# pasqal-io/pulser-diff

Hardware: AMD Instinct MI355X
Metric: time-steps/sec (fwd+grad) (higher is better)
Workload: dtype c128; 1 GPU; c3: 20-qubit register, 1000 time steps, fwd+grad wrt 8 pulse params per parameter set, KRYLOV_SE map, 1 parameter set(s) in the job; n_qubits=20, trajectories_total=1, trajectories_this_rank=1, ranks=1, gathered_parameter_sets=1, parallelism=trajectory-sharded x1 (one replica per rank), kernel_family=chained-tiles, tape=full

## Files before the change

### pulser-diff_amd/_native.py

```python
from __future__ import annotations

import ctypes
import os
import subprocess
import threading
from pathlib import Path

_CSRC = Path(__file__).resolve().parent / "csrc"
_LIB_PATH = Path(os.environ.get("RYDIFF_LIB", _CSRC / "librydiff.so"))

RYDIFF_OK = 0
RYDIFF_EINVAL = -1
RYDIFF_EWORKSPACE = -2
RYDIFF_EHIP = -3
RYDIFF_ENOTIMPL = -4
SOLVER_KRYLOV_SE = 0
SOLVER_DP5_SE = 1
PLAN_SCRATCH_BYTES = 1024
KERNEL_FAMILIES = ("lanes", "persistent", "direct", "chained-tiles")
MAX_QUBITS = 30
MAX_TERMS = 64
MAX_PAULI_STRINGS = 1024
MAX_OVERLAPS = 16
MAX_RDMS = 8
MAX_RDM_QUBITS = 6
MAX_TANGENTS = 8
TANGENT_PAIR_TERMS = 1
TANGENT_DENSITY_MATRIX = 2
TANGENT_RDMS = 4
TANGENT_MOMENTS = 8
MAX_DM_ATOMS = 12
MAX_DM_DIAG = 64
MAX_SHOTS = 1 << 20
SHOT_NONE = 0xFFFFFFFF


class RydProblem(ctypes.Structure):
    _fields_ = [
        ("n_qubits", ctypes.c_int32),
        ("batch", ctypes.c_int32),
        ("coeff_batch", ctypes.c_int32),
        ("n_samples", ctypes.c_int32),
        ("dt", ctypes.c_double),
        ("n_amp_terms", ctypes.c_int32),
        ("n_det_terms", ctypes.c_int32),
        ("amp_masks", ctypes.c_void_p),
        ("det_masks", ctypes.c_void_p),
        ("amp_tables", ctypes.c_void_p),
        ("det_tables", ctypes.c_void_p),
        ("u_pairs", ctypes.c_void_p),
        ("n_tsave", ctypes.c_int32),
        ("tsave", ctypes.c_void_p),
        ("solver", ctypes.c_int32),
        ("tol", ctypes.c_double),
        ("n_obs", ctypes.c_int32),
        ("obs_diag", ctypes.c_void_p),
        ("n_pair_terms", ctypes.c_int32),
        ("pair_qubits", ctypes.c_void_p),
        ("pair_tables", ctypes.c_void_p),
        ("real_amp_grad", ctypes.c_int32),
        ("kernel_variant", ctypes.c_int32),
        ("shard_bits", ctypes.c_int32),
        ("shard_rank_first", ctypes.c_int32),
        ("shard_recv", ctypes.c_void_p),
        ("shard_exchange", ctypes.c_void_p),
        ("shard_user", ctypes.c_void_p),
        ("final_state_only", ctypes.c_int32),
        ("amp_conditioned_terms", ctypes.c_uint64),
        ("det_ones_terms", ctypes.c_uint64),
        ("dp5_piece_refine", ctypes.c_void_p),
        ("dm_moments", ctypes.c_int32),
        ("n_shots", ctypes.c_int32),
        ("n_shot_times", ctypes.c_int32),
        ("shot_times", ctypes.c_void_p),
        ("shot_uniforms", ctypes.c_void_p),
        ("shots_out", ctypes.c_void_p),
        ("bit_moments", ctypes.c_int32),
        ("n_rdms", ctypes.c_int32),
        ("rdm_masks", ctypes.c_void_p),
        ("n_dm_rdms", ctypes.c_int32),
        ("dm_rdm_masks", ctypes.c_void_p),
        ("dm_atoms", ctypes.c_int32),
        ("n_dm_diag", ctypes.c_int32),
        ("dm_diag", ctypes.c_void_p),
        ("n_dm_pauli_obs", ctypes.c_int32),
        ("n_dm_pauli_strings", ctypes.c_int32),
        ("dm_pauli_first", ctypes.c_void_p),
        ("dm_pauli_x", ctypes.c_void_p),
        ("dm_pauli_z", ctypes.c_void_p),
        ("dm_pauli_w", ctypes.c_void_p),
        ("n_dm_fid", ctypes.c_int32),
        ("dm_fid_batch", ctypes.c_int32),
        ("dm_fid_targets", ctypes.c_void_p),
        ("dm_purity", ctypes.c_int32),
        ("dm_shots", ctypes.c_int32),
        ("tape_steps", ctypes.c_int32),
        ("n_overlaps", ctypes.c_int32),
        ("overlap_batch", ctypes.c_int32),
        ("overlap_targets", ctypes.c_void_p),
        ("n_pauli_obs", ctypes.c_int32),
        ("n_pauli_strings", ctypes.c_int32),
        ("pauli_first", ctypes.c_void_p),
        ("pauli_x", ctypes.c_void_p),
        ("pauli_z", ctypes.c_void_p),
        ("pauli_w", ctypes.c_void_p),
    ]


SHARD_EXCHANGE_FN = ctypes.CFUNCTYPE(ctypes.c_int, ctypes.c_void_p, ctypes.c_int, ctypes.c_void_p, ctypes.c_size_t)


class RydPlanInfo(ctypes.Structure):
    _fields_ = [
        ("spectral_lo", ctypes.c_double),
        ("spectral_hi", ctypes.c_double),
        ("rho_design", ctypes.c_double),
        ("degree", ctypes.c_int32),
        ("n_stages", ctypes.c_int32),
        ("max_step_factors", ctypes.c_int32),
        ("flags", ctypes.c_int32),
        ("total_factors", ctypes.c_int64),
        ("workspace_bytes", ctypes.c_size_t),
        ("tape_mode", ctypes.c_int32),
        ("kernel_family", ctypes.c_int32),
        ("kernel_fwd", ctypes.c_char * 80),
        ("kernel_bwd", ctypes.c_char * 80),
    ]


class RydTangent(ctypes.Structure):

    _fields_ = [
        ("n_dir", ctypes.c_int32),
        ("d_amp", ctypes.c_void_p),
        ("d_det", ctypes.c_void_p),
        ("d_u", ctypes.c_void_p),
        ("d_psi0", ctypes.c_void_p),
        ("flags", ctypes.c_int32),
    ]


EXPORTS = (
    "rydiff_plan",
    "rydiff_forward",
    "rydiff_backward",
    "rydiff_apply_hamiltonian",
    "rydiff_apply_factor",
    "rydiff_design_polynomial",
    "rydiff_last_error",
    "rydiff_version",
    "rydiff_sizeof_problem",
    "rydiff_sizeof_plan_info",
    "rydiff_sizeof_tangent",
    "rydiff_tangent_workspace_bytes",
    "rydiff_tangent_workspace_bytes_flags",
    "rydiff_forward_tangent",
    "rydiff_geometry_workspace_bytes",
    "rydiff_geometry_workspace_bytes_flags",
    "rydiff_forward_geometry",
    "rydiff_fisher_workspace_bytes_flags",
    "rydiff_forward_fisher",
)

_lib = None


def build(force: bool = False) -> Path:
    if force or not _LIB_PATH.exists():
        subprocess.run(["make", "-C", str(_CSRC)] + (["-B"] if force else []), check=True)
    return _LIB_PATH


def lib() -> ctypes.CDLL:
    global _lib
    if _lib is not None:
        return _lib
    if not _LIB_PATH.exists():
        raise RuntimeError(
            f"{_LIB_PATH} is missing: the HIP extension has not been built. Run `python -c 'import "
            "__graft_entry__ as g; g.build()'` (or `make -C pulser-diff_amd/csrc`). There is no CPU fallback."
        )
    L = ctypes.CDLL(str(_LIB_PATH))
    vp, i32, dbl = ctypes.c_void_p, ctypes.c_int, ctypes.c_double
    L.rydiff_plan.argtypes = [ctypes.POINTER(RydProblem), i32, i32, vp, vp, ctypes.POINTER(RydPlanInfo)]
    L.rydiff_plan.restype = i32
    L.rydiff_forward.argtypes = [ctypes.POINTER(RydProblem), ctypes.POINTER(RydPlanInfo), vp, vp, vp, vp,
                                 ctypes.c_size_t, i32, vp]
    L.rydiff_forward.restype = i32
    L.rydiff_backward.argtypes = [ctypes.POINTER(RydProblem), ctypes.POINTER(RydPlanInfo), vp, vp, vp, vp, vp, vp,
                                  vp, vp, vp, ctypes.c_size_t, i32, vp]
    L.rydiff_backward.restype = i32
    L.rydiff_apply_hamiltonian.argtypes = [ctypes.POINTER(RydProblem), vp, vp, vp, vp, vp, ctypes.c_size_t, vp]
    L.rydiff_apply_hamiltonian.restype = i32
    L.rydiff_apply_factor.argtypes = [ctypes.POINTER(RydProblem), vp, vp, vp, vp, vp, vp, i32, vp, vp, i32, vp,
                                      ctypes.c_size_t, vp]
    L.rydiff_apply_factor.restype = i32
    L.rydiff_design_polynomial.argtypes = [dbl, dbl, i32, ctypes.POINTER(i32), vp, vp, ctypes.POINTER(dbl)]
    L.rydiff_design_polynomial.restype = i32
    L.rydiff_last_error.restype = ctypes.c_char_p
    L.rydiff_version.restype = ctypes.c_char_p
    L.rydiff_sizeof_problem.restype = ctypes.c_size_t
    L.rydiff_sizeof_plan_info.restype = ctypes.c_size_t
    L.rydiff_sizeof_tangent.restype = ctypes.c_size_t
    L.rydiff_tangent_workspace_bytes.argtypes = [ctypes.POINTER(RydProblem), ctypes.POINTER(RydPlanInfo), i32]
    L.rydiff_tangent_workspace_bytes.restype = ctypes.c_size_t
    L.rydiff_tangent_workspace_bytes_flags.argtypes = [ctypes.POINTER(RydProblem), ctypes.POINTER(RydPlanInfo), i32, i32]
    L.rydiff_tangent_workspace_bytes_flags.restype = ctypes.c_size_t
    L.rydiff_forward_tangent.argtypes = [ctypes.POINTER(RydProblem), ctypes.POINTER(RydPlanInfo), ctypes.POINTER(RydTangent), vp, vp, vp,
                                         vp, ctypes.c_size_t, vp]
    L.rydiff_forward_tangent.restype = i32
    L.rydiff_geometry_workspace_bytes.argtypes = [ctypes.POINTER(RydProblem), ctypes.POINTER(RydPlanInfo), i32]
    L.rydiff_geometry_workspace_bytes.restype = ctypes.c_size_t
    L.rydiff_geometry_workspace_bytes_flags.argtypes = [ctypes.POINTER(RydProblem), ctypes.POINTER(RydPlanInfo), i32, i32]
    L.rydiff_geometry_workspace_bytes_flags.restype = ctypes.c_size_t
    L.rydiff_forward_geometry.argtypes = [ctypes.POINTER(RydProblem), ctypes.POINTER(RydPlanInfo), ctypes.POINTER(RydTangent), vp, vp, vp,
                                          vp, vp, ctypes.c_size_t, vp]
    L.rydiff_forward_geometry.restype = i32
    L.rydiff_fisher_workspace_bytes_flags.argtypes = [ctypes.POINTER(RydProblem), ctypes.POINTER(RydPlanInfo), i32, i32]
    L.rydiff_fisher_workspace_bytes_flags.restype = ctypes.c_size_t
    L.rydiff_forward_fisher.argtypes = [ctypes.POINTER(RydProblem), ctypes.POINTER(RydPlanInfo), ctypes.POINTER(RydTangent), vp, vp, vp,
                                        vp, vp, vp, ctypes.c_size_t, vp]
    L.rydiff_forward_fisher.restype = i32
    if (L.rydiff_sizeof_problem(), L.rydiff_sizeof_plan_info(), L.rydiff_sizeof_tangent()) != (
            ctypes.sizeof(RydProblem), ctypes.sizeof(RydPlanInfo), ctypes.sizeof(RydTangent)):
        raise RuntimeError(f"{_LIB_PATH} was built from another include/rydiff.h than this binding mirrors (struct sizes differ): rebuild it")
    _lib = L
    return L


def last_error() -> str:
    return lib().rydiff_last_error().decode()


def check(rc: int) -> None:
    if rc == RYDIFF_OK:
        return
    msg = last_error()
    if rc == RYDIFF_EINVAL:
        raise ValueError(msg)
    if rc == RYDIFF_ENOTIMPL:
        raise NotImplementedError(msg)
    if rc == RYDIFF_EWORKSPACE:
        raise MemoryError(msg)
    raise RuntimeError(f"rydiff (HIP) error {rc}: {msg}")


def design_polynomial(rho: float, tol: float = 1e-13, max_degree: int = 120):
    import numpy as np

    deg = ctypes.c_int()
    roots = np.zeros(2 * max_degree)
    p0 = np.zeros(2)
    err = ctypes.c_double()
    check(lib().rydiff_design_polynomial(rho, tol, max_degree, ctypes.byref(deg), roots.ctypes.data, p0.ctypes.data,
                                         ctypes.byref(err)))
    m = deg.value
    return roots[: 2 * m].view(np.complex128).copy(), complex(p0[0], p0[1]), err.value


_KNOWN_VARIANTS = (0, 1, 2, 3, 4, 7, 8, 9, 10, 11, 12, 13, 14, 15, 16, 17, 18, 19, 20, 21, 22, 23, 24, 25, 26, 27, 28, 29, 30, 31, 32, 33, 34)
_tls = threading.local()


def set_kernel_variant(variant: int) -> None:
    if int(variant) not in _KNOWN_VARIANTS:
        raise ValueError(f"kernel variant must be one of {_KNOWN_VARIANTS}, got {variant}")
    _tls.variant = int(variant)


def default_kernel_variant() -> int:
    return getattr(_tls, "variant", 0)
```

### pulser-diff_amd/csrc/chain_kernels.hpp

```cpp
#pragma once

constexpr int kSmallTileBits = 10;
constexpr int kTileBits = 12;
constexpr int kWideTileBits = 13;

__device__ __forceinline__ void stream_store(double2* p, const double2& v) {
#ifdef RYDIFF_PLAIN_STORES
    *p = v;
#else
    __builtin_nontemporal_store(v.x, &p->x);
    __builtin_nontemporal_store(v.y, &p->y);
#endif
}

__device__ __forceinline__ void through_store(double2* base, uint32_t n, unsigned i, const double2& v) {
    typedef unsigned u32x4 __attribute__((ext_vector_type(4)));
    const __amdgpu_buffer_rsrc_t dst = __builtin_amdgcn_make_buffer_rsrc(base, 0, int(n * uint32_t(sizeof(double2))), 0x00020000);
    __builtin_amdgcn_raw_buffer_store_b128(__builtin_bit_cast(u32x4, v), dst, int(i * unsigned(sizeof(double2))), 0,  16);
}

template <bool THROUGH>
__device__ __forceinline__ void out_store(double2* base, uint32_t n, unsigned i, const double2& v) {
    if constexpr (THROUGH) through_store(base, n, i, v);
    else stream_store(base + i, v);
}

__device__ __forceinline__ double2 stream_load(const double2* p) {
#ifdef RYDIFF_PLAIN_LOADS
    return *p;
#else
    double2 v;
    v.x = __builtin_nontemporal_load(&p->x);
    v.y = __builtin_nontemporal_load(&p->y);
    return v;
#endif
}

struct ChainArgs {
    const double2* u;
    const double2* p;
    double2* v_out;
    double2* q_out;
    const double* utt;
    const double* vr;
    const double* coef_fin;
    const double* coef_sta;
    long coef_bstride;
    double fb_r, fb_i;
    double fg_r, fg_i;
    int completes;
    double sg_r, sg_i, sb_r, sb_i;
    int lo, hs, hb;
    uint32_t dim;
    int has_p, has_q, write_v;
    int ga, gd;
    uint32_t fin_mask[kMaxGroups];
    uint32_t sta_mask[kMaxGroups];
    uint32_t dmask[kMaxGroups];
    int dcnt[kMaxGroups];
    uint32_t cond;
    int xcd_place;
    int tile_swz;
    int b_first, b_count;
    int resident;
    const double2* x_fin;
    const double2* x_sta;
    double* ge_fin;
    double* ge_sta;
    long ge_bstride, ge_rstride;
    double cb_fin_r, cb_fin_i, cb_sta_r, cb_sta_i;
    double* wtot;
    const double2* inj_gstate;
    const double* inj_gexp;
    const double* inj_obs;
    int inj_n_obs;
    long inj_ostride;
    int sh_bits;
    int sh_nl;
    int sh_rank_first;
    int sh_self;
    const double2* sh_rem[kShardMaxBits];
    int sh_grp[kShardMaxBits];
    long obs_bstride, obs_ostride;
    const double* obs;
    double* expect_slot;
    int n_obs;
    long exp_ostride;
};

template <int NT>
__device__ __forceinline__ void wg_atomic_add(double v, double* dst, double* red ) {
#pragma unroll
    for (int off = 32; off > 0; off >>= 1) v += __shfl_down(v, off, 64);
    __syncthreads();
    if ((threadIdx.x & 63) == 0) red[threadIdx.x >> 6] = v;
    __syncthreads();
    if (threadIdx.x == 0) {
        double s2 = 0.0;
#pragma unroll
        for (int w = 0; w < NT / 64; ++w) s2 += red[w];
        unsafeAtomicAdd(dst, s2);
    }
}

template <int NW>
__device__ __forceinline__ void park2(double v0, double v1, double* red, int slot0, int slot1) {
#pragma unroll
    for (int off = 32; off > 0; off >>= 1) {
        v0 += __shfl_down(v0, off, 64);
        v1 += __shfl_down(v1, off, 64);
    }
    if ((threadIdx.x & 63) == 0) {
        red[slot0 * NW + (threadIdx.x >> 6)] += v0;
        red[slot1 * NW + (threadIdx.x >> 6)] += v1;
    }
}

template <int NW>
__device__ __forceinline__ void park1(double v0, double* red, int slot0) {
#pragma unroll
    for (int off = 32; off > 0; off >>= 1) v0 += __shfl_down(v0, off, 64);
    if ((threadIdx.x & 63) == 0) red[slot0 * NW + (threadIdx.x >> 6)] += v0;
}

template <int LT, int LGT, bool CPLX, bool FULL = false, bool COND = false>
__device__ __forceinline__ void partner_sums(const double2* __restrict__ tile, const double2 (&reg)[1 << (LT - LGT)],
                                             uint32_t mask, unsigned tid, double2 (&ts)[1 << (LT - LGT)],
                                             double2 (&ds)[1 << (LT - LGT)]) {
    constexpr int NT = 1 << LGT, R = 1 << (LT - LGT);
#pragma unroll
    for (int r = 0; r < R; ++r) {
        ts[r] = make_double2(0.0, 0.0);
        ds[r] = make_double2(0.0, 0.0);
    }
#pragma unroll
    for (int b = 0; b < LT; ++b) {
        if (FULL || (mask >> b & 1u)) {
            if (b < LGT) {
                const double sgn = (tid >> b & 1u) ? 1.0 : -1.0;
#pragma unroll
                for (int r = 0; r < R; ++r) {
                    if (COND && !((unsigned(r) * NT + tid) >> (b ^ 1) & 1u)) continue;
                    const double2 q = tile[(unsigned(r) * NT + tid) ^ (1u << b)];
                    ts[r].x += q.x;
                    ts[r].y += q.y;
                    if (CPLX) {
                        ds[r].x = fma(sgn, q.x, ds[r].x);
                        ds[r].y = fma(sgn, q.y, ds[r].y);
                    }
                }
            } else {
#pragma unroll
                for (int r = 0; r < R; ++r) {
                    if (COND && !((unsigned(r) * NT + tid) >> (b ^ 1) & 1u)) continue;
                    const double2 q = reg[r ^ (1 << (b - LGT))];
                    ts[r].x += q.x;
                    ts[r].y += q.y;
                    if (CPLX) {
                        if (r >> (b - LGT) & 1) {
                            ds[r].x += q.x;
                            ds[r].y += q.y;
                        } else {
                            ds[r].x -= q.x;
                            ds[r].y -= q.y;
                        }
                    }
                }
            }
        }
    }
}

template <int CTRL, int BANK>
__device__ __forceinline__ int dpp_mov(int old, int src) {
    return __builtin_amdgcn_update_dpp(old, src, CTRL, 0xF, BANK, false);
}

template <int CTRL, int BANK>
__device__ __forceinline__ int dpp_mov_all(int src) {
    return __builtin_amdgcn_mov_dpp(src, CTRL, 0xF, BANK, true);
}

template <int B>
__device__ __forceinline__ int lane_xor_i32(int w) {
    if constexpr (B == 0) return dpp_mov_all<0xB1, 0xF>(w);
    else if constexpr (B == 1) return dpp_mov_all<0x4E, 0xF>(w);
    else if constexpr (B == 2) {
        const int r = dpp_mov_all<0x124, 0xA>(w);
        return dpp_mov<0x12C, 0x5>(r, w);
    } else if constexpr (B == 3) return dpp_mov_all<0x128, 0xF>(w);
    else return __shfl_xor(w, 1 << B, 64);
}

template <int B>
__device__ __forceinline__ double2 lane_xor(const double2& v) {
    const int a0 = lane_xor_i32<B>(__double2loint(v.x)), a1 = lane_xor_i32<B>(__double2hiint(v.x));
    const int b0 = lane_xor_i32<B>(__double2loint(v.y)), b1 = lane_xor_i32<B>(__double2hiint(v.y));
    return make_double2(__hiloint2double(a1, a0), __hiloint2double(b1, b0));
}

template <int LT, bool CPLX, bool FULL = false, bool COND = false>
__device__ __forceinline__ void partner_sums_lanes(const double2& own, uint32_t mask, unsigned tid, double2& ts, double2& ds) {
    static_assert(LT <= 6, "one amplitude per lane");
    ts = make_double2(0.0, 0.0);
    ds = make_double2(0.0, 0.0);
    auto bit = [&](auto bc) {
        constexpr int b = decltype(bc)::value;
        if constexpr (b < LT) {
            if (FULL || (mask >> b & 1u)) {
                double2 q = lane_xor<b>(own);
                if (COND && !(tid >> (b ^ 1) & 1u)) q = make_double2(0.0, 0.0);
                ts.x += q.x;
                ts.y += q.y;
                if (CPLX) {
                    const double sgn = (tid >> b & 1u) ? 1.0 : -1.0;
                    ds.x = fma(sgn, q.x, ds.x);
                    ds.y = fma(sgn, q.y, ds.y);
                }
            }
        }
    };
    bit(std::integral_constant<int, 0>{});
    bit(std::integral_constant<int, 1>{});
    bit(std::integral_constant<int, 2>{});
    bit(std::integral_constant<int, 3>{});
    bit(std::integral_constant<int, 4>{});
    bit(std::integral_constant<int, 5>{});
}

#ifdef RYDIFF_TIMELINE
__device__ unsigned long long g_timeline[4096 * 11];
#define RYDIFF_TL(slot)                                                                                   \
    do {                                                                                                  \
        if (threadIdx.x == 0 && blockIdx.y == 0 && blockIdx.x < 4096 && a.has_p && a.has_q)               \
            g_timeline[(slot) < 8 ? blockIdx.x * 8 + (slot) : 4096 * (slot) + blockIdx.x] = __builtin_readcyclecounter(); \
    } while (0)
#else
#define RYDIFF_TL(slot)
#endif

constexpr double kRecMinBetaC = 6.0e-5;

template <int LT, int LGT, bool CPLX, bool BWD, bool FAST = false, bool RES = false>
__global__ __launch_bounds__(1 << LGT) void k_chain(ChainArgs a) {
    constexpr int NT = 1 << LGT, R = 1 << (LT - LGT);
    constexpr bool REC = BWD && FAST && !CPLX;
    const int GA = FAST ? 1 : a.ga;
    const int GD = FAST ? (a.gd ? 1 : 0) : a.gd;
    extern __shared__ __attribute__((aligned(16))) double2 tile[];
    double* red = reinterpret_cast<double*>(tile + (size_t(1) << LT));
    constexpr int NW = NT / 64;
    const int n_slots = BWD ? 4 * a.ga + a.gd : 0;
    if (BWD) {
        for (int s = int(threadIdx.x); s < n_slots * NW; s += NT) red[s] = 0.0;
    }
    auto flush_gradients = [&](double* ge_fin_, double* ge_sta_) {
        __syncthreads();
        for (int s = int(threadIdx.x); s < n_slots; s += NT) {
            double sum = 0.0;
#pragma unroll
            for (int w = 0; w < NW; ++w) sum += red[s * NW + w];
            double* dst;
            if (s < 2 * a.ga) dst = ge_fin_ + ((s & 1) ? a.ga : 0) + (s >> 1);
            else if (s < 2 * a.ga + a.gd) dst = (REC ? ge_fin_ : ge_sta_) + 2 * a.ga + (s - 2 * a.ga);
            else dst = ge_sta_ + (((s - 2 * a.ga - a.gd) & 1) ? a.ga : 0) + ((s - 2 * a.ga - a.gd) >> 1);
            if (sum != 0.0) unsafeAtomicAdd(dst, sum);
        }
    };
    const unsigned tid = threadIdx.x;
    unsigned t = a.xcd_place ? (blockIdx.x >> 3) : blockIdx.x;
    if (a.tile_swz) {
        const unsigned w = blockIdx.x, G = 1u << a.tile_swz;
        t = (w & ~(8u * G - 1u)) | ((w & 7u) << a.tile_swz) | ((w >> 3) & (G - 1u));
    }
    const unsigned bl = a.xcd_place ? (blockIdx.y * 8u + (blockIdx.x & 7u)) : blockIdx.y;
    if (bl >= unsigned(a.b_count)) return;
    const unsigned bt = unsigned(a.b_first) + bl;
    const size_t boff = size_t(bt) * a.dim;
    const unsigned rank = unsigned(a.sh_rank_first) + bl;
    const unsigned rank_hi = a.sh_bits ? (rank << a.sh_nl) : 0u;
    const unsigned t_glob = a.sh_bits ? (t + (rank << (a.sh_nl - LT))) : t;
    auto ld = [&](const double2* p) -> double2 {
        if constexpr (RES) return *p;
        else return stream_load(p);
    };
    auto st = [&](double2* p, const double2& v) {
        if constexpr (RES) *p = v;
        else stream_store(p, v);
    };
    const unsigned lomask = (1u << a.lo) - 1u;
    const int midlow = a.hs - a.lo;
    const unsigned xbase = ((t & ((1u << midlow) - 1u)) << a.lo) | ((t >> midlow) << (a.hs + a.hb));

#ifdef RYDIFF_STAGGER
    for (unsigned sl = 0; sl < (blockIdx.x % RYDIFF_STAGGER_PHASES); ++sl) __builtin_amdgcn_s_sleep(RYDIFF_STAGGER);
#endif
    RYDIFF_TL(0);
    double2 uu[R], acc[R];
    unsigned xg[R];
#pragma unroll
    for (int r = 0; r < R; ++r) {
        const unsigned i = unsigned(r) * NT + tid;
        xg[r] = xbase | (i & lomask) | ((i >> a.lo) << a.hs);
        uu[r] = ld(a.u + boff + xg[r]);
    }
#pragma unroll
    for (int r = 0; r < R; ++r) acc[r] = ld(a.p + boff + xg[r]);
    double2 remacc[R];
    if (a.has_p && a.completes && a.sh_bits) {
#pragma unroll
        for (int r = 0; r < R; ++r) remacc[r] = make_double2(0.0, 0.0);
        const double* __restrict__ cfs = a.coef_fin + bt * a.coef_bstride;
        for (int k = 0; k < a.sh_bits; ++k) {
            if (a.sh_grp[k] < 0) continue;
            const double cr = cfs[a.sh_grp[k]], ci = (rank >> k & 1u) ? cfs[a.ga + a.sh_grp[k]] : -cfs[a.ga + a.sh_grp[k]];
            const double kr = a.fb_r * cr - a.fb_i * ci, ki = a.fb_r * ci + a.fb_i * cr;
            const double2* __restrict__ src = a.sh_self ? a.u + size_t(unsigned(a.b_first) + (bl ^ (1u << k))) * a.dim : a.sh_rem[k] + size_t(bl) * a.dim;
#pragma unroll
            for (int r = 0; r < R; ++r) {
                const double2 pv = src[xg[r]];
                remacc[r].x += kr * pv.x - ki * pv.y;
                remacc[r].y += kr * pv.y + ki * pv.x;
            }
        }
    }
    double dg[R];
#pragma unroll
    for (int r = 0; r < R; ++r) dg[r] = a.utt[unsigned(r) * NT + tid];
    double2 xf[R], xs[R];
    constexpr bool XS_EARLY = BWD && !CPLX && !REC;
    bool exact_fin = true, exact_sta = true;
    if constexpr (REC) {
        exact_fin = !(fabs(a.coef_fin[bt * a.coef_bstride]) * sqrt(a.fb_r * a.fb_r + a.fb_i * a.fb_i) >= kRecMinBetaC);
        exact_sta = !(fabs(a.coef_sta[bt * a.coef_bstride]) * sqrt(a.sb_r * a.sb_r + a.sb_i * a.sb_i) >= kRecMinBetaC);
    }
    if (BWD) {
#pragma unroll
        for (int r = 0; r < R; ++r) xf[r] = stream_load(a.x_fin + boff + xg[r]);
    }
    if (XS_EARLY) {
#pragma unroll
        for (int r = 0; r < R; ++r) xs[r] = stream_load(a.x_sta + boff + xg[r]);
    }
#ifndef RYDIFF_ABLATE_SYNC
#pragma unroll
    for (int r = 0; r < R; ++r) tile[unsigned(r) * NT + tid] = uu[r];
    __syncthreads();
#endif
    RYDIFF_TL(1);
    double* ge_fin = nullptr;
    double* ge_sta = nullptr;
    if (BWD) {
        const long goff = bt * a.ge_bstride + (blockIdx.x % kGradReplicas) * a.ge_rstride;
        ge_fin = a.ge_fin + goff;
        ge_sta = a.ge_sta + goff;
    }

    auto interaction_diagonal = [&](double (&du)[R]) {
        double vloc[LT];
        const double* __restrict__ vrow = a.vr + size_t(t_glob) * 16;
#ifdef RYDIFF_ABLATE_COEF
        for (int b2 = 0; b2 < LT; ++b2) vloc[b2] = a.sb_r;
        double dlane = a.sb_i;
        (void)vrow;
#else
#pragma unroll
        for (int b2 = 0; b2 < LT; ++b2) vloc[b2] = vrow[b2];
        double dlane = vrow[LT];
#endif
#pragma unroll
        for (int b2 = 0; b2 < LGT; ++b2)
            if (!(tid >> b2 & 1u)) dlane += vloc[b2];
#pragma unroll
        for (int r = 0; r < R; ++r) {
            double d = dg[r] + dlane;
#pragma unroll
            for (int b2 = LGT; b2 < LT; ++b2)
                if (!(r >> (b2 - LGT) & 1)) d += vloc[b2];
            du[r] = d;
        }
    };
    double du[R];
    if constexpr (REC) interaction_diagonal(du);

    if (a.has_p) {
        const double* __restrict__ cf = a.coef_fin + bt * a.coef_bstride;
        for (int g = 0; g < GA; ++g) {
            const uint32_t mask = a.fin_mask[g];
            if (!mask) continue;
            double2 ts[R], ds[R];
#ifndef RYDIFF_ABLATE_COMPUTE
            if (!FAST && (a.cond >> g & 1u)) partner_sums<LT, LGT, CPLX, false, true>(tile, uu, mask, tid, ts, ds);
            else partner_sums<LT, LGT, CPLX>(tile, uu, mask, tid, ts, ds);
#else
            for (int r = 0; r < R; ++r) { ts[r] = uu[r]; ds[r] = uu[r]; }
#endif
#ifdef RYDIFF_ABLATE_COEF
            const double cr = a.sg_r, ci = a.sg_i;
#else
            const double cr = cf[g], ci = cf[a.ga + g];
#endif
            const double k1r = a.fb_r * cr, k1i = a.fb_i * cr;
            const double k2r = -a.fb_i * ci, k2i = a.fb_r * ci;
#pragma unroll
            for (int r = 0; r < R; ++r) {
                acc[r].x += k1r * ts[r].x - k1i * ts[r].y;
                acc[r].y += k1r * ts[r].y + k1i * ts[r].x;
                if (CPLX) {
                    acc[r].x += k2r * ds[r].x - k2i * ds[r].y;
                    acc[r].y += k2r * ds[r].y + k2i * ds[r].x;
                }
            }
            if (BWD && exact_fin) {
                double z1r = 0.0, z1i = 0.0, z2r = 0.0, z2i = 0.0;
#pragma unroll
                for (int r = 0; r < R; ++r) {
                    z1r += ts[r].x * xf[r].x + ts[r].y * xf[r].y;
                    z1i += ts[r].x * xf[r].y - ts[r].y * xf[r].x;
                    if (CPLX) {
                        z2r += ds[r].x * xf[r].x + ds[r].y * xf[r].y;
                        z2i += ds[r].x * xf[r].y - ds[r].y * xf[r].x;
                    }
                }
                if (CPLX) park2<NW>(a.cb_fin_r * z1r - a.cb_fin_i * z1i, a.cb_fin_r * z2i + a.cb_fin_i * z2r, red, 2 * g, 2 * g + 1);
                else park1<NW>(a.cb_fin_r * z1r - a.cb_fin_i * z1i, red, 2 * g);
            }
        }
        if (a.completes && a.sh_bits) {
#pragma unroll
            for (int r = 0; r < R; ++r) {
                acc[r].x += remacc[r].x;
                acc[r].y += remacc[r].y;
            }
            if (BWD && exact_fin) {
                for (int k = 0; k < a.sh_bits; ++k) {
                    const int g = a.sh_grp[k];
                    if (g < 0) continue;
                    const double2* __restrict__ src = a.sh_self ? a.u + size_t(unsigned(a.b_first) + (bl ^ (1u << k))) * a.dim : a.sh_rem[k] + size_t(bl) * a.dim;
                    const double sgn = (rank >> k & 1u) ? 1.0 : -1.0;
                    double z1r = 0.0, z1i = 0.0;
#pragma unroll
                    for (int r = 0; r < R; ++r) {
                        const double2 pv = src[xg[r]];
                        z1r += pv.x * xf[r].x + pv.y * xf[r].y;
                        z1i += pv.x * xf[r].y - pv.y * xf[r].x;
                    }
                    if (CPLX) park2<NW>(a.cb_fin_r * z1r - a.cb_fin_i * z1i, sgn * (a.cb_fin_r * z1i + a.cb_fin_i * z1r), red, 2 * g, 2 * g + 1);
                    else park1<NW>(a.cb_fin_r * z1r - a.cb_fin_i * z1i, red, 2 * g);
                }
            }
        }
        if constexpr (REC) {
            if (a.completes) {
                double sgd = 0.0, zr = 0.0;
                const double cdet = GD ? cf[2] : 0.0;
#pragma unroll
                for (int r = 0; r < R; ++r) {
                    const double pr = a.cb_fin_r * uu[r].x + a.cb_fin_i * uu[r].y, pi = a.cb_fin_i * uu[r].x - a.cb_fin_r * uu[r].y;
                    const double w = pr * xf[r].x - pi * xf[r].y;
                    if (a.wtot) unsafeAtomicAdd(a.wtot + (a.sh_bits ? boff : 0) + xg[r], w);
                    const double cnt = GD ? double(a.dcnt[0] - popc_i((xg[r] | rank_hi) & a.dmask[0])) : 0.0;
                    sgd += w * cnt;
                    if (!exact_fin) {
                        double d = du[r] + cdet * cnt;
                        for (int g = 1; g < a.gd; ++g) d += cf[2 + g] * double(a.dcnt[g] - popc_i((xg[r] | rank_hi) & a.dmask[g]));
                        const double dr = a.fg_r + a.fb_r * d, di = a.fg_i + a.fb_i * d;
                        const double wx = acc[r].x - (dr * uu[r].x - di * uu[r].y), wy = acc[r].y - (dr * uu[r].y + di * uu[r].x);
                        zr += wx * xf[r].x + wy * xf[r].y;
                    }
                }
                if (GD) park1<NW>(sgd, red, 2 * a.ga);
                for (int g = 1; g < a.gd; ++g) {
                    double sg = 0.0;
#pragma unroll
                    for (int r = 0; r < R; ++r) {
                        const double pr = a.cb_fin_r * uu[r].x + a.cb_fin_i * uu[r].y, pi = a.cb_fin_i * uu[r].x - a.cb_fin_r * uu[r].y;
                        sg += (pr * xf[r].x - pi * xf[r].y) * double(a.dcnt[g] - popc_i((xg[r] | rank_hi) & a.dmask[g]));
                    }
                    park1<NW>(sg, red, 2 * a.ga + g);
                }
                if (!exact_fin) park1<NW>(zr / cf[0], red, 0);
            }
        }
    } else {
#pragma unroll
        for (int r = 0; r < R; ++r) acc[r] = uu[r];
    }
    if (BWD && a.has_p && (a.inj_gexp || a.inj_gstate)) {
        if (a.inj_gexp) {
            bool any = false;
            for (int o = 0; o < a.inj_n_obs; ++o) any |= a.inj_gexp[o * a.inj_ostride + bt] != 0.0;
            if (any) {
#pragma unroll
                for (int r = 0; r < R; ++r) {
                    double wsum = 0.0;
                    for (int o = 0; o < a.inj_n_obs; ++o)
                        wsum += a.inj_gexp[o * a.inj_ostride + bt] * a.inj_obs[size_t(o) * a.obs_ostride + bt * a.obs_bstride + xg[r]];
                    acc[r].x += 2.0 * wsum * xf[r].x;
                    acc[r].y += 2.0 * wsum * xf[r].y;
                }
            }
        }
        if (a.inj_gstate) {
#pragma unroll
            for (int r = 0; r < R; ++r) {
                const double2 gs = stream_load(a.inj_gstate + boff + xg[r]);
                acc[r].x += gs.x;
                acc[r].y += gs.y;
            }
        }
    }
    if (BWD && !XS_EARLY && a.has_q && (!REC || exact_sta)) {
#pragma unroll
        for (int r = 0; r < R; ++r) xs[r] = stream_load(a.x_sta + boff + xg[r]);
    }
    RYDIFF_TL(2);
    if (a.write_v) {
#pragma unroll
        for (int r = 0; r < R; ++r) st(a.v_out + boff + xg[r], acc[r]);
    }
    RYDIFF_TL(3);
    if (!BWD && a.obs) {
        for (int o = 0; o < a.n_obs; ++o) {
            double e = 0.0;
#pragma unroll
            for (int r = 0; r < R; ++r) e += a.obs[size_t(o) * a.obs_ostride + bt * a.obs_bstride + xg[r]] * (acc[r].x * acc[r].x + acc[r].y * acc[r].y);
            wg_atomic_add<NT>(e, a.expect_slot + o * a.exp_ostride + bt, red);
        }
    }
    if (!a.has_q) {
        if (BWD) flush_gradients(ge_fin, ge_sta);
        return;
    }

#ifndef RYDIFF_ABLATE_SYNC
    __syncthreads();
#pragma unroll
    for (int r = 0; r < R; ++r) tile[unsigned(r) * NT + tid] = acc[r];
    __syncthreads();
#endif
    RYDIFF_TL(4);

    const double* __restrict__ cf = a.coef_sta + bt * a.coef_bstride;
    if constexpr (!REC) interaction_diagonal(du);
    double rr[R];
    if (BWD && !REC) {
#pragma unroll
        for (int r = 0; r < R; ++r) {
            const double pr = a.cb_sta_r * acc[r].x + a.cb_sta_i * acc[r].y, pi = a.cb_sta_i * acc[r].x - a.cb_sta_r * acc[r].y;
            rr[r] = pr * xs[r].x - pi * xs[r].y;
            if (a.wtot) unsafeAtomicAdd(a.wtot + (a.sh_bits ? boff : 0) + xg[r], rr[r]);
        }
        for (int g = 0; g < a.gd; ++g) {
            double sgd = 0.0;
#pragma unroll
            for (int r = 0; r < R; ++r) sgd += rr[r] * double(a.dcnt[g] - popc_i((xg[r] | rank_hi) & a.dmask[g]));
            park1<NW>(sgd, red, 2 * a.ga + g);
        }
    }
    double2 q[R];
#pragma unroll
    for (int r = 0; r < R; ++r) {
        double d = du[r];
        if (FAST) {
            if (GD) d += cf[2] * double(a.dcnt[0] - popc_i((xg[r] | rank_hi) & a.dmask[0]));
            for (int g = 1; g < a.gd; ++g) d += cf[2 + g] * double(a.dcnt[g] - popc_i((xg[r] | rank_hi) & a.dmask[g]));
        } else {
            for (int g = 0; g < a.gd; ++g) d += cf[2 * a.ga + g] * double(a.dcnt[g] - popc_i((xg[r] | rank_hi) & a.dmask[g]));
        }
        const double dr = a.sg_r + a.sb_r * d, di = a.sg_i + a.sb_i * d;
        q[r].x = dr * acc[r].x - di * acc[r].y;
        q[r].y = dr * acc[r].y + di * acc[r].x;
    }
    for (int g = 0; g < GA; ++g) {
        const uint32_t mask = a.sta_mask[g];
        if (!FAST && !mask) continue;
        double2 ts[R], ds[R];
#ifndef RYDIFF_ABLATE_COMPUTE
        if (!FAST && (a.cond >> g & 1u)) partner_sums<LT, LGT, CPLX, false, true>(tile, acc, mask, tid, ts, ds);
        else partner_sums<LT, LGT, CPLX, FAST>(tile, acc, mask, tid, ts, ds);
#else
        for (int r = 0; r < R; ++r) { ts[r] = acc[r]; ds[r] = acc[r]; }
#endif
#ifdef RYDIFF_ABLATE_COEF
        const double cr = a.sg_r, ci = a.sg_i;
#else
        const double cr = cf[g], ci = cf[a.ga + g];
#endif
        const double k1r = a.sb_r * cr, k1i = a.sb_i * cr;
        const double k2r = -a.sb_i * ci, k2i = a.sb_r * ci;
#pragma unroll
        for (int r = 0; r < R; ++r) {
            q[r].x += k1r * ts[r].x - k1i * ts[r].y;
            q[r].y += k1r * ts[r].y + k1i * ts[r].x;
            if (CPLX) {
                q[r].x += k2r * ds[r].x - k2i * ds[r].y;
                q[r].y += k2r * ds[r].y + k2i * ds[r].x;
            }
        }
        if (BWD && exact_sta) {
            double z1r = 0.0, z1i = 0.0, z2r = 0.0, z2i = 0.0;
#pragma unroll
            for (int r = 0; r < R; ++r) {
                z1r += ts[r].x * xs[r].x + ts[r].y * xs[r].y;
                z1i += ts[r].x * xs[r].y - ts[r].y * xs[r].x;
                if (CPLX) {
                    z2r += ds[r].x * xs[r].x + ds[r].y * xs[r].y;
                    z2i += ds[r].x * xs[r].y - ds[r].y * xs[r].x;
                }
            }
            if (CPLX) park2<NW>(a.cb_sta_r * z1r - a.cb_sta_i * z1i, a.cb_sta_r * z2i + a.cb_sta_i * z2r, red, 2 * a.ga + a.gd + 2 * g,
                                2 * a.ga + a.gd + 2 * g + 1);
            else park1<NW>(a.cb_sta_r * z1r - a.cb_sta_i * z1i, red, 2 * a.ga + a.gd + 2 * g);
        }
    }
    RYDIFF_TL(5);
#pragma unroll
    for (int r = 0; r < R; ++r) st(a.q_out + boff + xg[r], q[r]);
    if (BWD) flush_gradients(ge_fin, ge_sta);
    RYDIFF_TL(6);
#ifdef RYDIFF_TIMELINE
    __builtin_amdgcn_s_waitcnt(0);
    RYDIFF_TL(7);
#endif
}

template <int I, int N, class F>
__device__ __forceinline__ void static_for(F&& f) {
    if constexpr (I < N) {
        f(std::integral_constant<int, I>{});
        static_for<I + 1, N>(f);
    }
}

template <int LT, bool CPLX, bool BWD, bool FAST, int RH = (1 << (LT - 10)) / 2>
__global__ __launch_bounds__(1024) void k_chain_wide(ChainArgs a) {
    constexpr int LGT = 10, NT = 1 << LGT, R = 1 << (LT - LGT), NP = R / RH, NW = NT / 64;
    static_assert(R >= 2 && RH >= 1 && NP * RH == R, "R amplitudes per thread in NP parts of RH");
    constexpr bool REC = BWD && FAST && !CPLX;
    const int GA = FAST ? 1 : a.ga;
    const int GD = FAST ? (a.gd ? 1 : 0) : a.gd;
    extern __shared__ __attribute__((aligned(16))) double2 tile[];
    double* red = reinterpret_cast<double*>(tile + (size_t(1) << LT));
    const int n_slots = BWD ? 4 * a.ga + a.gd : 0;
    if (BWD) {
        for (int s = int(threadIdx.x); s < n_slots * NW; s += NT) red[s] = 0.0;
    }
    const unsigned tid = threadIdx.x;
    unsigned t = blockIdx.x;
    if (a.tile_swz) {
        const unsigned w = blockIdx.x, G = 1u << a.tile_swz;
        t = (w & ~(8u * G - 1u)) | ((w & 7u) << a.tile_swz) | ((w >> 3) & (G - 1u));
    }
    const unsigned bl = blockIdx.y;
    const unsigned bt = unsigned(a.b_first) + bl;
    const size_t boff = size_t(bt) * a.dim;
    const unsigned rank = unsigned(a.sh_rank_first) + bl;
    const unsigned rank_hi = a.sh_bits ? (rank << a.sh_nl) : 0u;
    const unsigned t_glob = a.sh_bits ? (t + (rank << (a.sh_nl - LT))) : t;
    const unsigned lomask = (1u << a.lo) - 1u;
    const int midlow = a.hs - a.lo;
    const unsigned xbase = ((t & ((1u << midlow) - 1u)) << a.lo) | ((t >> midlow) << (a.hs + a.hb));
    auto xg_of = [&](int r) -> unsigned {
        const unsigned i = unsigned(r) * NT + tid;
        return xbase | (i & lomask) | ((i >> a.lo) << a.hs);
    };
    double* ge_fin = nullptr;
    double* ge_sta = nullptr;
    if (BWD) {
        const long goff = bt * a.ge_bstride + (blockIdx.x % kGradReplicas) * a.ge_rstride;
        ge_fin = a.ge_fin + goff;
        ge_sta = a.ge_sta + goff;
    }
    auto flush_gradients = [&]() {
        __syncthreads();
        for (int s = int(threadIdx.x); s < n_slots; s += NT) {
            double sum = 0.0;
#pragma unroll
            for (int w = 0; w < NW; ++w) sum += red[s * NW + w];
            double* dst;
            if (s < 2 * a.ga) dst = ge_fin + ((s & 1) ? a.ga : 0) + (s >> 1);
            else if (s < 2 * a.ga + a.gd) dst = (REC ? ge_fin : ge_sta) + 2 * a.ga + (s - 2 * a.ga);
            else dst = ge_sta + (((s - 2 * a.ga - a.gd) & 1) ? a.ga : 0) + ((s - 2 * a.ga - a.gd) >> 1);
            if (sum != 0.0) unsafeAtomicAdd(dst, sum);
        }
    };
    const double* __restrict__ vrow = a.vr + size_t(t_glob) * 16;
    auto lane_diag = [&]() -> double {
        double dlane = vrow[LT];
#pragma unroll
        for (int b2 = 0; b2 < LGT; ++b2)
            if (!(tid >> b2 & 1u)) dlane += vrow[b2];
        return dlane;
    };
    auto diag_of = [&](int rf, double dlane) -> double {
        double d = a.utt[unsigned(rf) * NT + tid] + dlane;
#pragma unroll
        for (int b2 = LGT; b2 < LT; ++b2)
            if (!(rf >> (b2 - LGT) & 1)) d += vrow[b2];
        return d;
    };
    bool exact_fin = true, exact_sta = true;
    if constexpr (REC) {
        exact_fin = !(fabs(a.coef_fin[bt * a.coef_bstride]) * sqrt(a.fb_r * a.fb_r + a.fb_i * a.fb_i) >= kRecMinBetaC);
        exact_sta = !(fabs(a.coef_sta[bt * a.coef_bstride]) * sqrt(a.sb_r * a.sb_r + a.sb_i * a.sb_i) >= kRecMinBetaC);
    }

    double2 acc[R];
    {
        double2 uu[RH];
#pragma unroll
        for (int h = 0; h < NP; ++h) {
#pragma unroll
            for (int r = 0; r < RH; ++r) uu[r] = stream_load(a.u + boff + xg_of(h * RH + r));
#pragma unroll
            for (int r = 0; r < RH; ++r) tile[unsigned(h * RH + r) * NT + tid] = uu[r];
        }
    }
#pragma unroll
    for (int r = 0; r < R; ++r) acc[r] = stream_load(a.p + boff + xg_of(r));
    __syncthreads();

    bool inj_any = false;
    if (BWD && a.has_p && a.inj_gexp) {
        for (int o = 0; o < a.inj_n_obs; ++o) inj_any |= a.inj_gexp[o * a.inj_ostride + bt] != 0.0;
    }
    auto finish_half = [&](auto hc) {
        constexpr int h = decltype(hc)::value;
        const double* __restrict__ cf = a.coef_fin + bt * a.coef_bstride;
        double2 xf[RH];
        if (BWD) {
#pragma unroll
            for (int r = 0; r < RH; ++r) xf[r] = stream_load(a.x_fin + boff + xg_of(h * RH + r));
        }
        if (a.has_p) {
            for (int g = 0; g < GA; ++g) {
                const uint32_t mask = a.fin_mask[g];
                if (!mask) continue;
                double2 ts[RH], ds[RH];
#pragma unroll
                for (int r = 0; r < RH; ++r) {
                    ts[r] = make_double2(0.0, 0.0);
                    ds[r] = make_double2(0.0, 0.0);
                }
#pragma unroll
                for (int b = 0; b < LT; ++b) {
                    if (mask >> b & 1u) {
#pragma unroll
                        for (int r = 0; r < RH; ++r) {
                            const unsigned i = unsigned(h * RH + r) * NT + tid;
                            const double2 q = tile[i ^ (1u << b)];
                            ts[r].x += q.x;
                            ts[r].y += q.y;
                            if (CPLX) {
                                const double sgn = (i >> b & 1u) ? 1.0 : -1.0;
                                ds[r].x = fma(sgn, q.x, ds[r].x);
                                ds[r].y = fma(sgn, q.y, ds[r].y);
                            }
                        }
                    }
                }
                const double cr = cf[g], ci = cf[a.ga + g];
                const double k1r = a.fb_r * cr, k1i = a.fb_i * cr;
                const double k2r = -a.fb_i * ci, k2i = a.fb_r * ci;
#pragma unroll
                for (int r = 0; r < RH; ++r) {
                    double2& A = acc[h * RH + r];
                    A.x += k1r * ts[r].x - k1i * ts[r].y;
                    A.y += k1r * ts[r].y + k1i * ts[r].x;
                    if (CPLX) {
                        A.x += k2r * ds[r].x - k2i * ds[r].y;
                        A.y += k2r * ds[r].y + k2i * ds[r].x;
                    }
                }
                if (BWD && exact_fin) {
                    double z1r = 0.0, z1i = 0.0, z2r = 0.0, z2i = 0.0;
#pragma unroll
                    for (int r = 0; r < RH; ++r) {
                        z1r += ts[r].x * xf[r].x + ts[r].y * xf[r].y;
                        z1i += ts[r].x * xf[r].y - ts[r].y * xf[r].x;
                        if (CPLX) {
                            z2r += ds[r].x * xf[r].x + ds[r].y * xf[r].y;
                            z2i += ds[r].x * xf[r].y - ds[r].y * xf[r].x;
                        }
                    }
                    if (CPLX) park2<NW>(a.cb_fin_r * z1r - a.cb_fin_i * z1i, a.cb_fin_r * z2i + a.cb_fin_i * z2r, red, 2 * g, 2 * g + 1);
                    else park1<NW>(a.cb_fin_r * z1r - a.cb_fin_i * z1i, red, 2 * g);
                }
            }
            if (a.completes && a.sh_bits) {
                for (int k = 0; k < a.sh_bits; ++k) {
                    const int g = a.sh_grp[k];
                    if (g < 0) continue;
                    const double cr = cf[g], ci = (rank >> k & 1u) ? cf[a.ga + g] : -cf[a.ga + g];
                    const double kr = a.fb_r * cr - a.fb_i * ci, ki = a.fb_r * ci + a.fb_i * cr;
                    const double2* __restrict__ src = a.sh_self ? a.u + size_t(unsigned(a.b_first) + (bl ^ (1u << k))) * a.dim : a.sh_rem[k] + size_t(bl) * a.dim;
                    const double sgn = (rank >> k & 1u) ? 1.0 : -1.0;
                    double z1r = 0.0, z1i = 0.0;
#pragma unroll
                    for (int r = 0; r < RH; ++r) {
                        const double2 pv = src[xg_of(h * RH + r)];
                        acc[h * RH + r].x += kr * pv.x - ki * pv.y;
                        acc[h * RH + r].y += kr * pv.y + ki * pv.x;
                        if (BWD) {
                            z1r += pv.x * xf[r].x + pv.y * xf[r].y;
                            z1i += pv.x * xf[r].y - pv.y * xf[r].x;
                        }
                    }
                    if (BWD && exact_fin) {
                        if (CPLX) park2<NW>(a.cb_fin_r * z1r - a.cb_fin_i * z1i, sgn * (a.cb_fin_r * z1i + a.cb_fin_i * z1r), red, 2 * g, 2 * g + 1);
                        else park1<NW>(a.cb_fin_r * z1r - a.cb_fin_i * z1i, red, 2 * g);
                    }
                }
            }
            if constexpr (REC) {
                if (a.completes) {
                    double sgd = 0.0, zr = 0.0;
                    const double cdet = GD ? cf[2] : 0.0;
                    const double dlane = exact_fin ? 0.0 : lane_diag();
#pragma unroll
                    for (int r = 0; r < RH; ++r) {
                        const int rf = h * RH + r;
                        const double2 mu = tile[unsigned(rf) * NT + tid];
                        const unsigned x = xg_of(rf);
                        const double pr = a.cb_fin_r * mu.x + a.cb_fin_i * mu.y, pi = a.cb_fin_i * mu.x - a.cb_fin_r * mu.y;
                        const double w = pr * xf[r].x - pi * xf[r].y;
                        if (a.wtot) unsafeAtomicAdd(a.wtot + (a.sh_bits ? boff : 0) + x, w);
                        const double cnt = GD ? double(a.dcnt[0] - popc_i((x | rank_hi) & a.dmask[0])) : 0.0;
                        sgd += w * cnt;
                        if (!exact_fin) {
                            double d = diag_of(rf, dlane) + cdet * cnt;
                            for (int g = 1; g < a.gd; ++g) d += cf[2 + g] * double(a.dcnt[g] - popc_i((x | rank_hi) & a.dmask[g]));
                            const double dr = a.fg_r + a.fb_r * d, di = a.fg_i + a.fb_i * d;
                            const double wx = acc[rf].x - (dr * mu.x - di * mu.y), wy = acc[rf].y - (dr * mu.y + di * mu.x);
                            zr += wx * xf[r].x + wy * xf[r].y;
                        }
                    }
                    if (GD) park1<NW>(sgd, red, 2 * a.ga);
                    for (int g = 1; g < a.gd; ++g) {
                        double sg = 0.0;
#pragma unroll
                        for (int r = 0; r < RH; ++r) {
                            const int rf = h * RH + r;
                            const double2 mu = tile[unsigned(rf) * NT + tid];
                            const double pr = a.cb_fin_r * mu.x + a.cb_fin_i * mu.y, pi = a.cb_fin_i * mu.x - a.cb_fin_r * mu.y;
                            sg += (pr * xf[r].x - pi * xf[r].y) * double(a.dcnt[g] - popc_i((xg_of(rf) | rank_hi) & a.dmask[g]));
                        }
                        park1<NW>(sg, red, 2 * a.ga + g);
                    }
                    if (!exact_fin) park1<NW>(zr / cf[0], red, 0);
                }
            }
        }
        if (BWD && a.has_p && (a.inj_gexp || a.inj_gstate)) {
            if (inj_any) {
#pragma unroll
                for (int r = 0; r < RH; ++r) {
                    double wsum = 0.0;
                    for (int o = 0; o < a.inj_n_obs; ++o)
                        wsum += a.inj_gexp[o * a.inj_ostride + bt] * a.inj_obs[size_t(o) * a.obs_ostride + bt * a.obs_bstride + xg_of(h * RH + r)];
                    acc[h * RH + r].x += 2.0 * wsum * xf[r].x;
                    acc[h * RH + r].y += 2.0 * wsum * xf[r].y;
                }
            }
            if (a.inj_gstate) {
#pragma unroll
                for (int r = 0; r < RH; ++r) {
                    const double2 gs = stream_load(a.inj_gstate + boff + xg_of(h * RH + r));
                    acc[h * RH + r].x += gs.x;
                    acc[h * RH + r].y += gs.y;
                }
            }
        }
        if (a.write_v) {
#pragma unroll
            for (int r = 0; r < RH; ++r) stream_store(a.v_out + boff + xg_of(h * RH + r), acc[h * RH + r]);
        }
    };
    static_for<0, NP>(finish_half);

    if (!BWD && a.obs) {
        for (int o = 0; o < a.n_obs; ++o) {
            double e = 0.0;
#pragma unroll
            for (int r = 0; r < R; ++r) e += a.obs[size_t(o) * a.obs_ostride + bt * a.obs_bstride + xg_of(r)] * (acc[r].x * acc[r].x + acc[r].y * acc[r].y);
            wg_atomic_add<NT>(e, a.expect_slot + o * a.exp_ostride + bt, red);
        }
    }
    if (!a.has_q) {
        if (BWD) flush_gradients();
        return;
    }

    __syncthreads();
#pragma unroll
    for (int r = 0; r < R; ++r) tile[unsigned(r) * NT + tid] = acc[r];
    __syncthreads();

    auto start_half = [&](auto hc) {
        constexpr int h = decltype(hc)::value;
        const double* __restrict__ cf = a.coef_sta + bt * a.coef_bstride;
        const bool need_xs = BWD && (!REC || exact_sta);
        double2 xs[RH];
        if (need_xs) {
#pragma unroll
            for (int r = 0; r < RH; ++r) xs[r] = stream_load(a.x_sta + boff + xg_of(h * RH + r));
        }
        double2 q[RH];
        const double dlane = lane_diag();
#pragma unroll
        for (int r = 0; r < RH; ++r) {
            const int rf = h * RH + r;
            double d = diag_of(rf, dlane);
            const unsigned x = xg_of(rf) | rank_hi;
            if (FAST) {
                if (GD) d += cf[2] * double(a.dcnt[0] - popc_i(x & a.dmask[0]));
                for (int g = 1; g < a.gd; ++g) d += cf[2 + g] * double(a.dcnt[g] - popc_i(x & a.dmask[g]));
            } else {
                for (int g = 0; g < a.gd; ++g) d += cf[2 * a.ga + g] * double(a.dcnt[g] - popc_i(x & a.dmask[g]));
            }
            const double dr = a.sg_r + a.sb_r * d, di = a.sg_i + a.sb_i * d;
            q[r].x = dr * acc[rf].x - di * acc[rf].y;
            q[r].y = dr * acc[rf].y + di * acc[rf].x;
        }
        if (BWD && !REC) {
            double rr[RH];
#pragma unroll
            for (int r = 0; r < RH; ++r) {
                const int rf = h * RH + r;
                const double pr = a.cb_sta_r * acc[rf].x + a.cb_sta_i * acc[rf].y, pi = a.cb_sta_i * acc[rf].x - a.cb_sta_r * acc[rf].y;
                rr[r] = pr * xs[r].x - pi * xs[r].y;
                if (a.wtot) unsafeAtomicAdd(a.wtot + (a.sh_bits ? boff : 0) + xg_of(rf), rr[r]);
            }
            for (int g = 0; g < a.gd; ++g) {
                double sgd = 0.0;
#pragma unroll
                for (int r = 0; r < RH; ++r) sgd += rr[r] * double(a.dcnt[g] - popc_i((xg_of(h * RH + r) | rank_hi) & a.dmask[g]));
                park1<NW>(sgd, red, 2 * a.ga + g);
            }
        }
        for (int g = 0; g < GA; ++g) {
            const uint32_t mask = a.sta_mask[g];
            if (!FAST && !mask) continue;
            double2 ts[RH], ds[RH];
#pragma unroll
            for (int r = 0; r < RH; ++r) {
                ts[r] = make_double2(0.0, 0.0);
                ds[r] = make_double2(0.0, 0.0);
            }
#pragma unroll
            for (int b = 0; b < LT; ++b) {
                if (FAST || (mask >> b & 1u)) {
#pragma unroll
                    for (int r = 0; r < RH; ++r) {
                        const int rf = h * RH + r;
                        const unsigned i = unsigned(rf) * NT + tid;
                        double2 pv;
                        if (b < LGT) pv = tile[i ^ (1u << b)];
                        else pv = acc[rf ^ (1 << (b < LGT ? 0 : b - LGT))];
                        ts[r].x += pv.x;
                        ts[r].y += pv.y;
                        if (CPLX) {
                            const double sgn = (i >> b & 1u) ? 1.0 : -1.0;
                            ds[r].x = fma(sgn, pv.x, ds[r].x);
                            ds[r].y = fma(sgn, pv.y, ds[r].y);
                        }
                    }
                }
            }
            const double cr = cf[g], ci = cf[a.ga + g];
            const double k1r = a.sb_r * cr, k1i = a.sb_i * cr;
            const double k2r = -a.sb_i * ci, k2i = a.sb_r * ci;
#pragma unroll
            for (int r = 0; r < RH; ++r) {
                q[r].x += k1r * ts[r].x - k1i * ts[r].y;
                q[r].y += k1r * ts[r].y + k1i * ts[r].x;
                if (CPLX) {
                    q[r].x += k2r * ds[r].x - k2i * ds[r].y;
                    q[r].y += k2r * ds[r].y + k2i * ds[r].x;
                }
            }
            if (BWD && exact_sta) {
                double z1r = 0.0, z1i = 0.0, z2r = 0.0, z2i = 0.0;
#pragma unroll
                for (int r = 0; r < RH; ++r) {
                    z1r += ts[r].x * xs[r].x + ts[r].y * xs[r].y;
                    z1i += ts[r].x * xs[r].y - ts[r].y * xs[r].x;
                    if (CPLX) {
                        z2r += ds[r].x * xs[r].x + ds[r].y * xs[r].y;
                        z2i += ds[r].x * xs[r].y - ds[r].y * xs[r].x;
                    }
                }
                if (CPLX) park2<NW>(a.cb_sta_r * z1r - a.cb_sta_i * z1i, a.cb_sta_r * z2i + a.cb_sta_i * z2r, red, 2 * a.ga + a.gd + 2 * g,
                                    2 * a.ga + a.gd + 2 * g + 1);
                else park1<NW>(a.cb_sta_r * z1r - a.cb_sta_i * z1i, red, 2 * a.ga + a.gd + 2 * g);
            }
        }
#pragma unroll
        for (int r = 0; r < RH; ++r) stream_store(a.q_out + boff + xg_of(h * RH + r), q[r]);
    };
    static_for<0, NP>(start_half);
    if (BWD) flush_gradients();
}
```

### pulser-diff_amd/csrc/pair_kernels.hpp

```cpp
#pragma once

struct Chain2Args {
    const double2* v;
    const double2* w;
    const double2* t;
    double2* vmid_out;
    double2* y_out;
    double2* w_out;
    double2* t_out;
    const double* utt;
    const double* vr;
    const double* coef_fin;
    const double* coef_sta;
    long coef_bstride;
    double a_r, a_i, b_r, b_i, k_r, k_i;
    double g1_r, g1_i, b1_r, b1_i;
    int lo, hs, hb;
    uint32_t dim;
    int has_p, has_q;
    int gd;
    uint32_t fin_mask;
    uint32_t dmask[kMaxGroups];
    int dcnt[kMaxGroups];
    int b_first, b_count;
    const double* obs;
    double* expect_slot;
    int n_obs;
    long exp_ostride;
};

template <int LT, int LGT, bool ORD = false, int WT = 0, int PACE = 0>
__global__ __launch_bounds__(1 << LGT) void k_chain2(Chain2Args a) {
    constexpr int NT = 1 << LGT, R = 1 << (LT - LGT);
    static_assert(WT >= 0 && WT <= 3);
    static_assert(PACE >= 0 && PACE <= 2 && (!PACE || ORD) && (!PACE || R == 4), "pacing: vector-major kernels with four elements per thread");
    extern __shared__ __attribute__((aligned(16))) double2 tiles[];
    double* red = reinterpret_cast<double*>(tiles + 2 * (size_t(1) << LT));
    const unsigned tid = threadIdx.x;
    const unsigned t = blockIdx.x;
    const unsigned bl = blockIdx.y;
    if (bl >= unsigned(a.b_count)) return;
    const unsigned bt = unsigned(a.b_first) + bl;
    const size_t boff = size_t(bt) * a.dim;
    const unsigned lomask = (1u << a.lo) - 1u;
    const int midlow = a.hs - a.lo;
    const unsigned xbase = ((t & ((1u << midlow) - 1u)) << a.lo) | ((t >> midlow) << (a.hs + a.hb));
    RYDIFF_TL(0);
    const double* __restrict__ vrow = a.vr + size_t(t) * 16;
    [[maybe_unused]] double ut[R], vtop[LT + 1], c_fin = 0.0, c_sta = 0.0, cdet_fin = 0.0, cdet_sta = 0.0;
    if constexpr (ORD) {
#pragma unroll
        for (int b2 = 0; b2 <= LT; ++b2) vtop[b2] = vrow[b2];
#pragma unroll
        for (int r = 0; r < R; ++r) ut[r] = a.utt[unsigned(r) * NT + tid];
        c_fin = a.coef_fin[bt * a.coef_bstride];
        c_sta = a.coef_sta[bt * a.coef_bstride];
        if (a.gd) {
            cdet_fin = a.coef_fin[bt * a.coef_bstride + 2];
            cdet_sta = a.coef_sta[bt * a.coef_bstride + 2];
        }
    }
    double2 uu[R], ww[R], tt[R];
    unsigned xg[R];
#pragma unroll
    for (int r = 0; r < R; ++r) {
        const unsigned i = unsigned(r) * NT + tid;
        xg[r] = xbase | (i & lomask) | ((i >> a.lo) << a.hs);
        uu[r] = stream_load(a.v + boff + xg[r]);
    }
    if constexpr (ORD && !PACE) __builtin_amdgcn_s_barrier();
    if constexpr (PACE) {
        __builtin_amdgcn_sched_barrier(0);
        asm volatile("s_waitcnt vmcnt(2)" ::: "memory");
        __builtin_amdgcn_sched_barrier(0);
    }
#pragma unroll
    for (int r = 0; r < R; ++r) ww[r] = stream_load(a.w + boff + xg[r]);
    if constexpr (ORD && !PACE) __builtin_amdgcn_s_barrier();
    if constexpr (!PACE) {
#pragma unroll
        for (int r = 0; r < R; ++r) tt[r] = stream_load(a.t + boff + xg[r]);
    } else {
        __builtin_amdgcn_sched_barrier(0);
    }
    auto reindex = [&]() {
        if constexpr (ORD) {
            unsigned tid_o = tid;
            asm volatile("" : "+v"(tid_o));
#pragma unroll
            for (int r = 0; r < R; ++r) {
                const unsigned i = unsigned(r) * NT + tid_o;
                xg[r] = xbase | (i & lomask) | ((i >> a.lo) << a.hs);
            }
        }
    };
    reindex();
    double du[R];
    {
        double vloc[LT];
#pragma unroll
        for (int b2 = 0; b2 < LT; ++b2) vloc[b2] = ORD ? vtop[b2] : vrow[b2];
        double dlane = ORD ? vtop[LT] : vrow[LT];
#pragma unroll
        for (int b2 = 0; b2 < LGT; ++b2)
            if (!(tid >> b2 & 1u)) dlane += vloc[b2];
#pragma unroll
        for (int r = 0; r < R; ++r) {
            double d;
            if constexpr (ORD) d = ut[r] + dlane;
            else d = a.utt[unsigned(r) * NT + tid] + dlane;
#pragma unroll
            for (int b2 = LGT; b2 < LT; ++b2)
                if (!(r >> (b2 - LGT) & 1)) d += vloc[b2];
            du[r] = d;
        }
    }
    auto diag = [&](const double* cf, [[maybe_unused]] double cdet, int r) -> double {
        double d = du[r];
        if constexpr (ORD) {
            for (int g = 0; g < a.gd; ++g) d += cdet * double(a.dcnt[g] - popc_i(xg[r] & a.dmask[g]));
        } else {
            for (int g = 0; g < a.gd; ++g) d += cf[2 + g] * double(a.dcnt[g] - popc_i(xg[r] & a.dmask[g]));
        }
        return d;
    };
    int buf = 0;
    auto put = [&](const double2 (&val)[R]) -> const double2* {
        double2* tile = tiles + (size_t(buf) << LT);
#pragma unroll
        for (int r = 0; r < R; ++r) tile[unsigned(r) * NT + tid] = val[r];
        __syncthreads();
        buf ^= 1;
        return tile;
    };
    auto cmul = [](double xr, double xi, const double2& z) { return make_double2(xr * z.x - xi * z.y, xr * z.y + xi * z.x); };
    auto request_t = [&]() {
        __builtin_amdgcn_sched_barrier(0);
        const char* tbase = reinterpret_cast<const char*>(a.t + boff);
#pragma unroll
        for (int r = 0; r < R; ++r) tt[r] = stream_load(reinterpret_cast<const double2*>(tbase + xg[r] * unsigned(sizeof(double2))));
        __builtin_amdgcn_sched_barrier(0);
    };

    double2 y[R];
    if (a.has_p) {
        const double* __restrict__ cf = a.coef_fin + bt * a.coef_bstride;
        double c;
        if constexpr (ORD) c = c_fin;
        else c = cf[0];
        double2 s[R], h1[R], ds[R];
        const double2* vtile;
        if constexpr (PACE == 2) {
            double2* tile = tiles + (size_t(buf) << LT);
#pragma unroll
            for (int r = 0; r < R; ++r) tile[unsigned(r) * NT + tid] = uu[r];
            request_t();
            __syncthreads();
            buf ^= 1;
            vtile = tile;
        } else {
            vtile = put(uu);
        }
        RYDIFF_TL(1);
        partner_sums<LT, LGT, false>(vtile, uu, a.fin_mask, tid, s, ds);
        if constexpr (PACE == 1) {
            __builtin_amdgcn_sched_barrier(0);
            asm volatile("s_waitcnt vmcnt(2)" ::: "memory");
            request_t();
        }
#ifdef RYDIFF_TIMELINE
#pragma unroll
        for (int r = 0; r < R; ++r) asm volatile("" ::"v"(ww[r].x), "v"(ww[r].y));
        RYDIFF_TL(8);
#endif
        double d[R];
#pragma unroll
        for (int r = 0; r < R; ++r) {
            d[r] = diag(cf, cdet_fin, r);
            h1[r].x = d[r] * uu[r].x + c * (ww[r].x + s[r].x);
            h1[r].y = d[r] * uu[r].y + c * (ww[r].y + s[r].y);
            const double2 p = cmul(a.a_r, a.a_i, uu[r]), q = cmul(a.b_r, a.b_i, h1[r]);
            y[r] = make_double2(p.x + q.x, p.y + q.y);
        }
        RYDIFF_TL(2);
        if constexpr (PACE) {
            static_assert(WT >= 1, "pacing: v_mid goes through through_store");
            double2* mid_base = a.vmid_out ? a.vmid_out + boff : nullptr;
            const uint32_t mid_n = a.vmid_out ? a.dim : 0u;
#pragma unroll
            for (int r = 0; r < R; ++r) {
                const double2 p = cmul(a.g1_r, a.g1_i, uu[r]), q = cmul(a.b1_r, a.b1_i, h1[r]);
                through_store(mid_base, mid_n, xg[r], make_double2(p.x + q.x, p.y + q.y));
            }
        } else if (a.vmid_out) {
#pragma unroll
            for (int r = 0; r < R; ++r) {
                const double2 p = cmul(a.g1_r, a.g1_i, uu[r]), q = cmul(a.b1_r, a.b1_i, h1[r]);
                out_store<(WT >= 1)>(a.vmid_out + boff, a.dim, xg[r], make_double2(p.x + q.x, p.y + q.y));
            }
        }
        if (a.k_r != 0.0 || a.k_i != 0.0) {
            double2 e[R], pe[R];
#pragma unroll
            for (int r = 0; r < R; ++r) e[r] = make_double2(h1[r].x + c * ww[r].x, h1[r].y + c * ww[r].y);
            partner_sums<LT, LGT, false>(put(e), e, a.fin_mask, tid, pe, ds);
#ifdef RYDIFF_TIMELINE
#pragma unroll
            for (int r = 0; r < R; ++r) asm volatile("" ::"v"(tt[r].x), "v"(tt[r].y));
            RYDIFF_TL(9);
#endif
#pragma unroll
            for (int r = 0; r < R; ++r) {
                const double2 z = make_double2(d[r] * h1[r].x + c * (tt[r].x + pe[r].x), d[r] * h1[r].y + c * (tt[r].y + pe[r].y));
                const double2 k = cmul(a.k_r, a.k_i, z);
                y[r].x += k.x;
                y[r].y += k.y;
            }
        } else if constexpr (PACE) {
#pragma unroll
            for (int r = 0; r < R; ++r) asm volatile("" ::"v"(tt[r].x), "v"(tt[r].y));
        }
        RYDIFF_TL(3);
#pragma unroll
        for (int r = 0; r < R; ++r) out_store<(WT >= 1)>(a.y_out + boff, a.dim, xg[r], y[r]);
        RYDIFF_TL(4);
        if (a.obs) {
            for (int o = 0; o < a.n_obs; ++o) {
                double ex = 0.0;
#pragma unroll
                for (int r = 0; r < R; ++r) ex += a.obs[size_t(o) * a.dim + xg[r]] * (y[r].x * y[r].x + y[r].y * y[r].y);
                wg_atomic_add<NT>(ex, a.expect_slot + o * a.exp_ostride + bt, red);
            }
        }
    } else {
#pragma unroll
        for (int r = 0; r < R; ++r) y[r] = PACE ? ww[r] : (ORD ? tt[r] : uu[r]);
    }
    if (!a.has_q) return;

    reindex();
    const double* __restrict__ cf = a.coef_sta + bt * a.coef_bstride;
    double c;
    if constexpr (ORD) c = c_sta;
    else c = cf[0];
    double2 w2[R], ds[R];
    partner_sums<LT, LGT, false, true>(put(y), y, ~0u, tid, w2, ds);
#pragma unroll
    for (int r = 0; r < R; ++r) out_store<(WT >= 2)>(a.w_out + boff, a.dim, xg[r], w2[r]);
    RYDIFF_TL(5);
    double2 z[R];
#pragma unroll
    for (int r = 0; r < R; ++r) {
        const double d = diag(cf, cdet_sta, r);
        z[r] = make_double2(d * y[r].x + c * w2[r].x, d * y[r].y + c * w2[r].y);
    }
    double2 t2[R];
    partner_sums<LT, LGT, false, true>(put(z), z, ~0u, tid, t2, ds);
#pragma unroll
    for (int r = 0; r < R; ++r) out_store<(WT >= 3)>(a.t_out + boff, a.dim, xg[r], t2[r]);
    RYDIFF_TL(6);
#ifdef RYDIFF_TIMELINE
    asm volatile("s_waitcnt vmcnt(0)" ::: "memory");
    RYDIFF_TL(7);
#endif
}

struct Chain2BwdArgs {
    const double2* mu;
    const double2* w;
    const double2* t;
    const double2* xa;
    const double2* xb;
    double2* mu_out;
    double2* w_out;
    double2* t_out;
    const double* utt;
    const double* vr;
    const double* coef_fin;
    const double* coef_sta;
    long coef_bstride;
    double gb_r, gb_i, bb_r, bb_i;
    double k_r, k_i;
    double ga_r, ga_i, ba_r, ba_i;
    double cba_r, cba_i, cbb_r, cbb_i;
    int lo, hs, hb;
    uint32_t dim;
    int has_p, has_q;
    int gd;
    uint32_t fin_mask;
    uint32_t dmask;
    int dcnt;
    int b_first, b_count;
    double* ge_fin;
    long ge_bstride, ge_rstride;
    int det_slot;
    double* wtot;
    const double2* inj_gstate;
    const double* inj_gexp;
    const double* inj_obs;
    int inj_n_obs;
    long inj_ostride;
};

__device__ __forceinline__ void stream_load_lds(const double2* g, double2* lds_wave) {
    __builtin_amdgcn_global_load_lds(reinterpret_cast<const __attribute__((address_space(1))) void*>(reinterpret_cast<uintptr_t>(g)),
                                     (__attribute__((address_space(3))) void*)lds_wave, 16, 0,  2);
}

constexpr int kChain2BwdXbLds = 1;

template <int LT, int LGT, bool DMA>
constexpr size_t chain2_bwd_lds_bytes() {
    return 2 * (size_t(1) << LT) * sizeof(double2) + 2 * ((size_t(1) << LGT) / 64) * sizeof(double) +
           (DMA ? size_t(kChain2BwdXbLds) * (size_t(1) << LGT) * sizeof(double2) : 0);
}

template <int LT, int LGT, bool ORD, int WT, bool DMA, int PACE = 0>
__global__ __launch_bounds__(1 << LGT) void k_chain2_bwd(Chain2BwdArgs a) {
    constexpr int NT = 1 << LGT, R = 1 << (LT - LGT), NW = NT / 64;
    static_assert(WT >= 0 && WT <= 3);
    static_assert(PACE >= 0 && PACE <= 1 && (!PACE || (ORD && !DMA && R == 4)), "pacing: the vector-major register-staged kernel, four elements per thread");
    constexpr int XBL = DMA ? kChain2BwdXbLds : 0;
    static_assert(XBL <= R && (2 * NW * sizeof(double)) % sizeof(double2) == 0);
    extern __shared__ __attribute__((aligned(16))) double2 tiles[];
    double* red = reinterpret_cast<double*>(tiles + 2 * (size_t(1) << LT));
    double2* xbs = tiles + 2 * (size_t(1) << LT) + 2 * NW * sizeof(double) / sizeof(double2);
    const unsigned tid = threadIdx.x;
    const unsigned t = blockIdx.x;
    const unsigned bl = blockIdx.y;
    if (bl >= unsigned(a.b_count)) return;
    const unsigned bt = unsigned(a.b_first) + bl;
    const size_t boff = size_t(bt) * a.dim;
    const unsigned lomask = (1u << a.lo) - 1u;
    const int midlow = a.hs - a.lo;
    const unsigned xbase = ((t & ((1u << midlow) - 1u)) << a.lo) | ((t >> midlow) << (a.hs + a.hb));
    if (tid < 2 * NW) red[tid] = 0.0;
    RYDIFF_TL(0);
    double2 uu[R], ww[R], xb[R], tp[R];
    unsigned xg[R];
    auto reindex = [&]() {
        unsigned tid_o = tid;
        asm volatile("" : "+v"(tid_o));
#pragma unroll
        for (int r = 0; r < R; ++r) {
            const unsigned i = unsigned(r) * NT + tid_o;
            xg[r] = xbase | (i & lomask) | ((i >> a.lo) << a.hs);
        }
    };
    double vloc[LT + 1], ut[R];
    {
        const double* __restrict__ vrow = a.vr + size_t(t) * 16;
#pragma unroll
        for (int b2 = 0; b2 <= LT; ++b2) vloc[b2] = vrow[b2];
#pragma unroll
        for (int r = 0; r < R; ++r) ut[r] = a.utt[unsigned(r) * NT + tid];
    }
    double c_fin = a.coef_fin[bt * a.coef_bstride], c_sta = a.coef_sta[bt * a.coef_bstride], cdet_fin = 0.0, cdet_sta = 0.0;
    if (a.gd) {
        cdet_fin = a.coef_fin[bt * a.coef_bstride + 2];
        cdet_sta = a.coef_sta[bt * a.coef_bstride + 2];
    }
#pragma unroll
    for (int r = 0; r < R; ++r) {
        const unsigned i = unsigned(r) * NT + tid;
        xg[r] = xbase | (i & lomask) | ((i >> a.lo) << a.hs);
        uu[r] = stream_load(a.mu + boff + xg[r]);
    }
    if constexpr (ORD && !PACE) __builtin_amdgcn_s_barrier();
    if constexpr (PACE) {
        __builtin_amdgcn_sched_barrier(0);
        asm volatile("s_waitcnt vmcnt(2)" ::: "memory");
        __builtin_amdgcn_sched_barrier(0);
    }
#pragma unroll
    for (int r = 0; r < R; ++r) ww[r] = stream_load(a.w + boff + xg[r]);
    if constexpr (ORD && !PACE) __builtin_amdgcn_s_barrier();
    [[maybe_unused]] double2 xa[R];
    if constexpr (DMA) {
        const unsigned wv = __builtin_amdgcn_readfirstlane(tid & ~63u);
        double2* xat = tiles + (size_t(1) << LT);
#pragma unroll
        for (int r = 0; r < R; ++r) stream_load_lds(a.xa + boff + xg[r], xat + unsigned(r) * NT + wv);
#pragma unroll
        for (int r = 0; r < XBL; ++r) stream_load_lds(a.xb + boff + xg[r], xbs + unsigned(r) * NT + wv);
#pragma unroll
        for (int r = XBL; r < R; ++r) xb[r] = stream_load(a.xb + boff + xg[r]);
    } else {
#pragma unroll
        for (int r = 0; r < R; ++r) xa[r] = stream_load(a.xa + boff + xg[r]);
    }
    __builtin_amdgcn_sched_barrier(0);
    auto uniform = [](double v) {
        return __hiloint2double(__builtin_amdgcn_readfirstlane(__double2hiint(v)), __builtin_amdgcn_readfirstlane(__double2loint(v)));
    };
    c_fin = uniform(c_fin);
    c_sta = uniform(c_sta);
    cdet_fin = uniform(cdet_fin);
    cdet_sta = uniform(cdet_sta);
    double du[R];
    {
        double dlane = vloc[LT];
#pragma unroll
        for (int b2 = 0; b2 < LGT; ++b2) dlane = (tid >> b2 & 1u) ? dlane : dlane + vloc[b2];
#pragma unroll
        for (int r = 0; r < R; ++r) {
            double d = ut[r] + dlane;
#pragma unroll
            for (int b2 = LGT; b2 < LT; ++b2)
                if (!(r >> (b2 - LGT) & 1)) d += vloc[b2];
            du[r] = d;
        }
    }
    auto cnt = [&](int r) -> double { return a.gd ? double(a.dcnt - popc_i(xg[r] & a.dmask)) : 0.0; };
    int buf = 0;
    auto put = [&](const double2 (&val)[R]) -> const double2* {
        double2* tile = tiles + (size_t(buf) << LT);
#pragma unroll
        for (int r = 0; r < R; ++r) tile[unsigned(r) * NT + tid] = val[r];
        __syncthreads();
        buf ^= 1;
        return tile;
    };
    auto cmul = [](double xr, double xi, const double2& z) { return make_double2(xr * z.x - xi * z.y, xr * z.y + xi * z.x); };
    auto cdot = [](const double2& p, const double2& x) { return make_double2(p.x * x.x + p.y * x.y, p.x * x.y - p.y * x.x); };
    auto xbv = [&](int r) -> double2 { return r < XBL ? xbs[unsigned(r) * NT + tid] : xb[r]; };

#ifdef RYDIFF_TIMELINE
#pragma unroll
    for (int r = 0; r < R; ++r) asm volatile("" ::"v"(uu[r].x), "v"(uu[r].y));
    RYDIFF_TL(8);
#endif
#pragma unroll
    for (int r = 0; r < R; ++r) {
        if constexpr (PACE) {
            asm volatile("" ::"v"(uu[r].x), "v"(uu[r].y));
        } else {
            asm volatile("" ::"v"(uu[r].x), "v"(uu[r].y), "v"(ww[r].x), "v"(ww[r].y));
            if constexpr (!DMA) asm volatile("" ::"v"(xa[r].x), "v"(xa[r].y));
            if (DMA && r >= XBL) asm volatile("" ::"v"(xb[r].x), "v"(xb[r].y));
        }
    }
    double2 y[R];
    if (a.has_p) {
        const double c = c_fin, cdet = cdet_fin;
        double2 pm[R], mid[R];
        double wx[R];
        double zc = 0.0;
        const bool two = a.k_r != 0.0 || a.k_i != 0.0;
        {
            double2* etile = tiles + (size_t(buf ^ 1) << LT);
            if constexpr (PACE) {
            } else if constexpr (DMA) {
#ifdef RYDIFF_TIMELINE
                RYDIFF_TL(9);
#endif
                asm volatile("s_waitcnt vmcnt(0)" ::: "memory");
            } else {
#ifdef RYDIFF_TIMELINE
                RYDIFF_TL(9);
#endif
#pragma unroll
                for (int r = 0; r < R; ++r) etile[unsigned(r) * NT + tid] = xa[r];
            }
#ifdef RYDIFF_TIMELINE
            if constexpr (!PACE) RYDIFF_TL(10);
#endif
            double2 s[R], ds[R];
            const double2* mtile = put(uu);
            RYDIFF_TL(1);
            partner_sums<LT, LGT, false>(mtile, uu, a.fin_mask, tid, s, ds);
#ifdef RYDIFF_TIMELINE
            if constexpr (PACE) {
#pragma unroll
                for (int r = 0; r < R; ++r) asm volatile("" ::"v"(ww[r].x), "v"(ww[r].y));
                RYDIFF_TL(9);
#pragma unroll
                for (int r = 0; r < R; ++r) asm volatile("" ::"v"(xa[r].x), "v"(xa[r].y));
                RYDIFF_TL(10);
            }
#endif
#pragma unroll
            for (int r = 0; r < R; ++r) {
                double2 xav;
                if constexpr (PACE) xav = xa[r];
                else xav = etile[unsigned(r) * NT + tid];
                const double d = du[r] + cdet * cnt(r);
                pm[r] = make_double2(ww[r].x + s[r].x, ww[r].y + s[r].y);
                const double2 h1 = make_double2(d * uu[r].x + c * pm[r].x, d * uu[r].y + c * pm[r].y);
                if (two) etile[unsigned(r) * NT + tid] = make_double2(h1.x + c * ww[r].x, h1.y + c * ww[r].y);
                const double2 q1 = cdot(pm[r], xav);
                zc += a.cba_r * q1.x - a.cba_i * q1.y;
                const double2 wa = cdot(uu[r], xav);
                wx[r] = a.cba_r * wa.x - a.cba_i * wa.y;
                const double2 mm = cmul(a.ga_r, a.ga_i, uu[r]), mh = cmul(a.ba_r, a.ba_i, h1);
                mid[r] = make_double2(mm.x + mh.x, mm.y + mh.y);
            }
        }
        park1<NW>(zc, red, 0);
        zc = 0.0;
        RYDIFF_TL(2);
        if constexpr (!DMA) {
#pragma unroll
            for (int r = 0; r < R; ++r) xb[r] = stream_load(a.xb + boff + xg[r]);
        }
#pragma unroll
        for (int r = 0; r < R; ++r) tp[r] = stream_load(a.t + boff + xg[r]);
        reindex();
        double sgd = 0.0;
#pragma unroll
        for (int r = 0; r < R; ++r) {
            const double2 xbr = xbv(r);
            const double2 wb = cdot(mid[r], xbr);
            const double wr = wx[r] + (a.cbb_r * wb.x - a.cbb_i * wb.y);
            if (a.wtot) unsafeAtomicAdd(a.wtot + xg[r], wr);
            sgd += wr * cnt(r);
            const double2 gpm = cmul(a.ga_r, a.ga_i, pm[r]);
            const double2 q = cdot(gpm, xbr);
            zc += a.cbb_r * q.x - a.cbb_i * q.y;
            const double d = du[r] + cdet * cnt(r);
            const double2 y1 = cmul(a.gb_r + a.bb_r * d, a.gb_i + a.bb_i * d, mid[r]), y2 = cmul(a.bb_r * c, a.bb_i * c, gpm);
            y[r] = make_double2(y1.x + y2.x, y1.y + y2.y);
        }
        __builtin_amdgcn_sched_barrier(0);
        RYDIFF_TL(3);
        if (two) {
            __syncthreads();
            buf ^= 1;
        }
        if (two) {
            const double2* tile = tiles + (size_t(buf ^ 1) << LT);
#pragma unroll
            for (int b = 0; b < LT; ++b) {
                if (a.fin_mask >> b & 1u) {
#pragma unroll
                    for (int r = 0; r < R; ++r) {
                        const double2 q = tile[(unsigned(r) * NT + tid) ^ (1u << b)];
                        tp[r].x += q.x;
                        tp[r].y += q.y;
                    }
                }
            }
        }
        const double kc_r = a.k_r * c, kc_i = a.k_i * c;
#pragma unroll
        for (int r = 0; r < R; ++r) {
            const double2 kt = cmul(kc_r, kc_i, tp[r]);
            y[r].x += kt.x;
            y[r].y += kt.y;
            const double2 q = cdot(cmul(a.ba_r, a.ba_i, tp[r]), xbv(r));
            zc += a.cbb_r * q.x - a.cbb_i * q.y;
        }
        RYDIFF_TL(4);
        park2<NW>(zc, sgd, red, 0, 1);
        reindex();
        if (a.inj_gexp || a.inj_gstate) {
            if (a.inj_gexp) {
                bool any = false;
                for (int o = 0; o < a.inj_n_obs; ++o) any |= a.inj_gexp[o * a.inj_ostride + bt] != 0.0;
                if (any) {
#pragma unroll
                    for (int r = 0; r < R; ++r) {
                        double wsum = 0.0;
                        for (int o = 0; o < a.inj_n_obs; ++o) wsum += a.inj_gexp[o * a.inj_ostride + bt] * a.inj_obs[size_t(o) * a.dim + xg[r]];
                        const double2 xbr = xbv(r);
                        y[r].x += 2.0 * wsum * xbr.x;
                        y[r].y += 2.0 * wsum * xbr.y;
                    }
                }
            }
            if (a.inj_gstate) {
#pragma unroll
                for (int r = 0; r < R; ++r) {
                    const double2 gs = stream_load(a.inj_gstate + boff + xg[r]);
                    y[r].x += gs.x;
                    y[r].y += gs.y;
                }
            }
        }
#pragma unroll
        for (int r = 0; r < R; ++r) out_store<(WT >= 1)>(a.mu_out + boff, a.dim, xg[r], y[r]);
        RYDIFF_TL(5);
    } else {
#pragma unroll
        for (int r = 0; r < R; ++r) {
            y[r] = uu[r];
            if constexpr (PACE) asm volatile("" ::"v"(ww[r].x), "v"(ww[r].y), "v"(xa[r].x), "v"(xa[r].y));
        }
    }
    auto flush = [&]() {
        if (a.has_p && tid < 2) {
            double sum = 0.0;
#pragma unroll
            for (int w = 0; w < NW; ++w) sum += red[tid * NW + w];
            double* ge = a.ge_fin + bt * a.ge_bstride + (blockIdx.x % kGradReplicas) * a.ge_rstride;
            if (sum != 0.0) unsafeAtomicAdd(ge + (tid ? a.det_slot : 0), sum);
        }
    };
    if (!a.has_q) {
        __syncthreads();
        flush();
        return;
    }

    const double c = c_sta, cdet = cdet_sta;
    reindex();
    double2 w2[R], ds[R];
    partner_sums<LT, LGT, false, true>(put(y), y, ~0u, tid, w2, ds);
#pragma unroll
    for (int r = 0; r < R; ++r) out_store<(WT >= 2)>(a.w_out + boff, a.dim, xg[r], w2[r]);
    RYDIFF_TL(6);
    double2 z[R];
#pragma unroll
    for (int r = 0; r < R; ++r) {
        const double d = du[r] + cdet * cnt(r);
        z[r] = make_double2(d * y[r].x + c * w2[r].x, d * y[r].y + c * w2[r].y);
    }
    double2 t2[R];
    partner_sums<LT, LGT, false, true>(put(z), z, ~0u, tid, t2, ds);
#pragma unroll
    for (int r = 0; r < R; ++r) out_store<(WT >= 3)>(a.t_out + boff, a.dim, xg[r], t2[r]);
    RYDIFF_TL(7);
    flush();
}
```

### pulser-diff_amd/csrc/pair_launch.hpp

```cpp
#pragma once

namespace {

bool pair_legal(const Runtime& rt) {
    const Plan& pl = rt.pl;
    const uint32_t all = uint32_t(pl.dim) - 1u;
    const ChainGeom g = chain_geom(rt);
    return rt.pair_mode >= 0 && rt.variant == 0 && !rt.force_three && !rt.force_xcd && chain_enabled(rt) && !pl.shard_bits &&
           pl.N > kTileBits && pl.N <= 20 && g.lt == kTileBits && g.layouts == 2 && pl.ga.n == 1 && pl.gd.n <= 1 && !pl.ga.flagged &&
           (pl.ga.amp_index_mask[0] & all) == all && !(rt.flags & 1) && pl.off_pp2 && pl.off_pp3;
}

bool pair_enabled(const Runtime& rt) {
    if (!pair_legal(rt)) return false;
    return rt.pair_mode == 1 || (rt.pl.N == 20 && rt.pl.B == 1);
}

template <class Args>
void fill_chain2(Args& ca, const Runtime& rt, char* ws, const std::vector<ChainItem>& items, const std::vector<std::pair<int, int>>& blk,
                 int j, const double2* cur, const BatchSlice& bs) {
    const Plan& pl = rt.pl;
    double2* wt[2][2] = {{reinterpret_cast<double2*>(ws + pl.off_pp0), reinterpret_cast<double2*>(ws + pl.off_pp1)},
                         {reinterpret_cast<double2*>(ws + pl.off_pp2), reinterpret_cast<double2*>(ws + pl.off_pp3)}};
    const ChainGeom geom{kTileBits, 2};
    const int nb = int(blk.size()), L = j & 1;
    const LayoutDesc Y = chain_layout(pl.NL, L, geom), X = chain_layout(pl.NL, L ^ 1, geom);
    ca.w = j ? wt[(j - 1) & 1][0] : cur;
    ca.t = j ? wt[(j - 1) & 1][1] : cur;
    ca.utt = split_tables(pl, ws, kTileBits) + size_t(L) * rt.per_layout(kTileBits);
    ca.vr = ca.utt + (size_t(1) << kTileBits);
    ca.coef_bstride = rt.coef_bstride();
    ca.coef_fin = rt.coef(ws, j ? items[blk[j - 1].first].stage : 0);
    ca.coef_sta = rt.coef(ws, j < nb ? items[blk[j].first].stage : 0);
    ca.lo = Y.lo;
    ca.hs = Y.hs;
    ca.hb = Y.hb;
    ca.dim = uint32_t(pl.dim);
    ca.has_p = j > 0;
    ca.has_q = j < nb;
    ca.gd = pl.gd.n;
    ca.b_first = bs.first;
    ca.b_count = bs.count;
    if (ca.has_p) ca.fin_mask = to_tile_mask(Y, kTileBits, uint32_t(pl.dim - 1) & ~X.bits);
    if (ca.has_q) {
        ca.w_out = wt[j & 1][0];
        ca.t_out = wt[j & 1][1];
    }
}

constexpr bool kPairVecMajorDefault = true;
constexpr int kPairThroughDefault = 3;
bool pair_vec_major(const Runtime& rt) { return rt.pair_phases >= 0 ? (rt.pair_phases >> 2) != 0 : kPairVecMajorDefault; }
int pair_through(const Runtime& rt) { return rt.pair_phases >= 0 ? (rt.pair_phases & 3) : kPairThroughDefault; }

constexpr int kPairPaceFwdDefault = 0;
constexpr int kPairPaceBwdDefault = 1;
int pair_pace_fwd(const Runtime& rt) {
    if (!pair_vec_major(rt) || pair_through(rt) != 3) return 0;
    return rt.pair_pace_fwd >= 0 ? rt.pair_pace_fwd : kPairPaceFwdDefault;
}

template <class F>
int with_pair_phases(bool ord, int wt, F f) {
    using std::bool_constant;
    using std::integral_constant;
    switch ((ord ? 4 : 0) | wt) {
        case 0: return f(bool_constant<false>{}, integral_constant<int, 0>{});
        case 1: return f(bool_constant<false>{}, integral_constant<int, 1>{});
        case 2: return f(bool_constant<false>{}, integral_constant<int, 2>{});
        case 3: return f(bool_constant<false>{}, integral_constant<int, 3>{});
        case 4: return f(bool_constant<true>{}, integral_constant<int, 0>{});
        case 5: return f(bool_constant<true>{}, integral_constant<int, 1>{});
        case 6: return f(bool_constant<true>{}, integral_constant<int, 2>{});
        case 7: return f(bool_constant<true>{}, integral_constant<int, 3>{});
    }
    return fail(RYDIFF_EINVAL, "internal: no such block kernel");
}

template <int LGT, bool ORD, int WT, int PACE = 0>
int launch_chain2_t(const Chain2Args& ca, unsigned tiles, hipStream_t stream) {
    constexpr int LT = kTileBits;
    const size_t lds = 2 * (size_t(1) << LT) * sizeof(double2) + 256;
    if (int rc = set_max_dynamic_lds_once<&k_chain2<LT, LGT, ORD, WT, PACE>>(lds)) return rc;
    hipLaunchKernelGGL((k_chain2<LT, LGT, ORD, WT, PACE>), dim3(tiles, unsigned(ca.b_count)), dim3(1 << LGT), lds, stream, ca);
    LAUNCH_CHECK();
    return RYDIFF_OK;
}

int launch_chain2(const Runtime& rt, const Chain2Args& ca, unsigned tiles, hipStream_t stream) {
    switch (pair_pace_fwd(rt)) {
        case 1: return launch_chain2_t<10, true, 3, 1>(ca, tiles, stream);
        case 2: return launch_chain2_t<10, true, 3, 2>(ca, tiles, stream);
    }
    return with_pair_phases(pair_vec_major(rt), pair_through(rt), [&](auto ord, auto wt) {
        return launch_chain2_t<10, decltype(ord)::value, decltype(wt)::value>(ca, tiles, stream);
    });
}

template <class DstFn, class DoneFn, class ExpFn>
int run_chain2(const Runtime& rt, char* ws, const std::vector<ChainItem>& items, const double2* start, DstFn dst, bool keep_mid,
               DoneFn on_done, ExpFn exp_slot, const BatchSlice& bs, hipStream_t stream) {
    const Plan& pl = rt.pl;
    const int F = int(items.size());
    if (F <= 0) return RYDIFF_OK;
    std::vector<std::pair<int, int>> blk;
    for (int i = 0; i < F;) {
        if (i + 1 < F && items[i + 1].stage == items[i].stage) {
            blk.push_back({i, i + 1});
            i += 2;
        } else {
            blk.push_back({i, -1});
            ++i;
        }
    }
    const unsigned tiles = unsigned(pl.dim >> kTileBits);
    const int nb = int(blk.size());
    const double2* cur = start;
    for (int j = 0; j <= nb; ++j) {
        Chain2Args ca{};
        fill_chain2(ca, rt, ws, items, blk, j, cur, bs);
        ca.v = cur;
        fill_detuning(ca.dmask, ca.dcnt, pl);
        int f0 = -1, last = -1;
        if (ca.has_p) {
            f0 = blk[j - 1].first;
            const int f1 = blk[j - 1].second;
            last = f1 >= 0 ? f1 : f0;
            const FactorScalars& s1 = items[f0].s;
            const FactorScalars s2 = f1 >= 0 ? items[f1].s : FactorScalars{1.0, 0.0, 0.0, 0.0};
            const std::complex<double> g1(s1.gr, s1.gi), b1(s1.br, s1.bi), g2(s2.gr, s2.gi), b2(s2.br, s2.bi);
            const std::complex<double> qa = g1 * g2, qb = g1 * b2 + b1 * g2, qk = b1 * b2;
            ca.a_r = qa.real();
            ca.a_i = qa.imag();
            ca.b_r = qb.real();
            ca.b_i = qb.imag();
            ca.k_r = qk.real();
            ca.k_i = qk.imag();
            ca.g1_r = s1.gr;
            ca.g1_i = s1.gi;
            ca.b1_r = s1.br;
            ca.b1_i = s1.bi;
            ca.vmid_out = (f1 >= 0 && keep_mid) ? dst(f0) : nullptr;
            ca.y_out = dst(last);
            if (!ca.y_out) return fail(RYDIFF_EINVAL, "internal: chain destination missing");
            ChainStep cs{};
            exp_slot(last, cs);
            ca.obs = cs.obs;
            ca.expect_slot = cs.expect_slot;
            ca.n_obs = cs.n_obs;
            ca.exp_ostride = cs.exp_ostride;
        }
        int rc = launch_chain2(rt, ca, tiles, stream);
        if (rc) return rc;
        if (ca.has_p) {
            if (ca.vmid_out) {
                rc = on_done(f0, ca.vmid_out);
                if (rc) return rc;
            }
            rc = on_done(last, ca.y_out);
            if (rc) return rc;
            cur = ca.y_out;
        }
    }
    return RYDIFF_OK;
}

bool pair_bwd_enabled(const Runtime& rt) {
    const ChainGeom g = chain_geom(rt);
    return !rt.pair_bwd_off && rt.real_amp_grad && pair_enabled(rt) && g.lt == kTileBits && g.layouts == 2;
}

constexpr bool kPairBwdDmaDefault = false;
bool pair_bwd_dma(const Runtime& rt) { return rt.pair_bwd_stage ? rt.pair_bwd_stage > 0 : kPairBwdDmaDefault; }

int pair_pace_bwd(const Runtime& rt) {
    if (!pair_vec_major(rt) || pair_through(rt) != 3 || pair_bwd_dma(rt)) return 0;
    return rt.pair_pace_bwd >= 0 ? rt.pair_pace_bwd : kPairPaceBwdDefault;
}

template <int LGT, bool ORD, int WT, bool DMA, int PACE = 0>
int launch_chain2_bwd_t(const Chain2BwdArgs& ca, unsigned tiles, hipStream_t stream) {
    constexpr int LT = kTileBits;
    constexpr size_t lds = chain2_bwd_lds_bytes<LT, LGT, DMA>();
    static_assert(lds <= 160 * 1024, "k_chain2_bwd: more LDS than a gfx950 workgroup can have");
    if (int rc = set_max_dynamic_lds_once<&k_chain2_bwd<LT, LGT, ORD, WT, DMA, PACE>>(lds)) return rc;
    hipLaunchKernelGGL((k_chain2_bwd<LT, LGT, ORD, WT, DMA, PACE>), dim3(tiles, unsigned(ca.b_count)), dim3(1 << LGT), lds, stream, ca);
    LAUNCH_CHECK();
    return RYDIFF_OK;
}

int launch_chain2_bwd(const Runtime& rt, const Chain2BwdArgs& ca, unsigned tiles, hipStream_t stream) {
    const bool ord = pair_vec_major(rt);
    if (pair_pace_bwd(rt)) return launch_chain2_bwd_t<10, true, 3, false, 1>(ca, tiles, stream);
    if (pair_bwd_dma(rt)) {
        if (ord && pair_through(rt) == 3) return launch_chain2_bwd_t<10, true, 3, true>(ca, tiles, stream);
        if (ord && pair_through(rt) == 0) return launch_chain2_bwd_t<10, true, 0, true>(ca, tiles, stream);
        return fail(RYDIFF_EINVAL, "internal: no such block kernel");
    }
    return with_pair_phases(ord, pair_through(rt), [&](auto o, auto wt) {
        return launch_chain2_bwd_t<10, decltype(o)::value, decltype(wt)::value, false>(ca, tiles, stream);
    });
}

template <class StageEndFn>
int run_chain2_bwd(const Runtime& rt, char* ws, const std::vector<ChainItem>& items, const std::vector<const double2*>& xs,
                   const std::vector<int>& save_k, const double2* lam_in, double2* lam_bufs[2], int& cl, double* wtot,
                   StageEndFn on_stage_end, const BatchSlice& bs, const InjectSource& inj, hipStream_t stream) {
    const Plan& pl = rt.pl;
    const int M = int(items.size());
    if (M <= 0) return RYDIFF_OK;
    std::vector<std::pair<int, int>> blk;
    for (int f = M - 1; f >= 0;) {
        if (f >= 1 && items[f - 1].stage == items[f].stage) {
            blk.push_back({f - 1, f});
            f -= 2;
        } else {
            blk.push_back({f, -1});
            --f;
        }
    }
    const unsigned tiles = unsigned(pl.dim >> kTileBits);
    const int nb = int(blk.size());
    const double2* cur = lam_in;
    int rc = on_stage_end(items[M - 1].stage, cur, xs[M]);
    if (rc) return rc;
    for (int j = 0; j <= nb; ++j) {
        Chain2BwdArgs ca{};
        fill_chain2(ca, rt, ws, items, blk, j, cur, bs);
        ca.mu = cur;
        ca.xa = ca.xb = cur;
        if (pl.gd.n) {
            ca.dmask = pl.gd.amp_index_mask[0];
            ca.dcnt = pl.gd.count[0];
        }
        ca.ge_fin = rt.ge(ws, 0);
        ca.ge_bstride = rt.ge_bstride();
        ca.ge_rstride = pl.NC + 1;
        ca.det_slot = 2 * pl.ga.n;
        ca.wtot = wtot;
        int fb = -1;
        if (ca.has_p) {
            fb = blk[j - 1].first;
            const int fa = blk[j - 1].second;
            const FactorScalars& sb = items[fb].s;
            const FactorScalars sa = fa >= 0 ? items[fa].s : FactorScalars{1.0, 0.0, 0.0, 0.0};
            const std::complex<double> gb(sb.gr, -sb.gi), bb(sb.br, -sb.bi), ga(sa.gr, -sa.gi), ba(sa.br, -sa.bi);
            const std::complex<double> qk = ba * bb;
            ca.gb_r = gb.real();
            ca.gb_i = gb.imag();
            ca.bb_r = bb.real();
            ca.bb_i = bb.imag();
            ca.k_r = qk.real();
            ca.k_i = qk.imag();
            ca.ga_r = ga.real();
            ca.ga_i = ga.imag();
            ca.ba_r = ba.real();
            ca.ba_i = ba.imag();
            ca.cba_r = sa.br;
            ca.cba_i = sa.bi;
            ca.cbb_r = sb.br;
            ca.cbb_i = sb.bi;
            ca.xb = xs[fb];
            ca.xa = fa >= 0 ? xs[fa] : xs[fb];
            ca.ge_fin = rt.ge(ws, items[fb].stage);
            cl ^= 1;
            ca.mu_out = lam_bufs[cl];
            if (ca.mu_out == cur) return fail(RYDIFF_EINVAL, "internal: cotangent ping-pong clash");
            fill_inject(ca, inj, save_k[fb], pl);
        }
        rc = launch_chain2_bwd(rt, ca, tiles, stream);
        if (rc) return rc;
        if (ca.has_p) {
            cur = ca.mu_out;
            if (fb >= 1 && items[fb].stage != items[fb - 1].stage) {
                rc = on_stage_end(items[fb - 1].stage, cur, xs[fb]);
                if (rc) return rc;
            }
        }
    }
    return RYDIFF_OK;
}

}
```

### pulser-diff_amd/csrc/runtime.hpp

```cpp
#pragma once

struct LayoutDesc {
    int lo, hs, hb;
    uint32_t bits;
};

struct ChainGeom {
    int lt;
    int layouts;
};

double* split_tables(const Plan& pl, char* ws, int lt) {
    return reinterpret_cast<double*>(ws + pl.off_split) + pl.split_off_doubles[lt - kSmallTileBits];
}

LayoutDesc chain_layout(int N, int which, const ChainGeom& g) {
    LayoutDesc d{};
    const bool three = g.layouts == 3;
    if (which == 0) {
        d.lo = g.lt;
        d.hs = g.lt;
        d.hb = 0;
    } else if (which == 1) {
        d.hs = g.lt;
        d.hb = three ? 8 : N - g.lt;
        d.lo = g.lt - d.hb;
    } else {
        d.hs = g.lt + 8;
        d.hb = N - d.hs;
        d.lo = g.lt - d.hb;
    }
    d.bits = ((1u << d.lo) - 1u) | (((1u << d.hb) - 1u) << d.hs);
    return d;
}

namespace {

struct Runtime {
    Plan pl;
    PolyDesign poly;
    double sigma = 0.0, width = 1.0, rho_design = 1.0;
    int64_t total_factors = 0;
    int max_step_factors = 0;
    int flags = 0;
    bool real_amp_grad = false;
    bool prefer_direct = false;
    bool small_tiles = false;
    int variant = 0;
    bool generic_direct = false;
    bool plain_tile_order = false;
    int force_three = 0;
    int tile_mode = 0;
    bool force_xcd = false;
    int pair_mode = 0;
    bool pair_bwd_off = false;
    int pair_bwd_stage = 0;
    int pair_phases = -1;
    int pair_pace_fwd = -1;
    int pair_pace_bwd = -1;
    int chain_lgt = 9;
    void* const* shard_recv = nullptr;
    int (*shard_exchange)(void*, int, const void*, size_t) = nullptr;
    void* shard_user = nullptr;
    GroupArgs garg{};
    PairArgs parg{};

    long coef_bstride() const { return pl.Bc > 1 ? long(pl.stages.size()) * pl.NC : 0; }
    long ge_rec() const { return long(kGradReplicas) * (pl.NC + 1); }
    long ge_bstride() const { return pl.Bc > 1 ? long(pl.stages.size()) * ge_rec() : 0; }
    long obs_bstride() const { return pl.shard_bits ? long(pl.dim) : 0; }
    long obs_ostride() const { return pl.shard_bits ? long(pl.B) * long(pl.dim) : long(pl.dim); }
    size_t per_layout(int lt) const { return (size_t(1) << lt) + size_t((size_t(1) << pl.N) >> lt) * 16; }
    const double* coef(const char* ws, int stage) const { return reinterpret_cast<const double*>(ws + pl.off_coef) + size_t(stage) * pl.NC; }
    double* ge(char* ws, int stage) const { return reinterpret_cast<double*>(ws + pl.off_ge) + size_t(stage) * ge_rec(); }
};

int decode_variant(const RydProblem* p, Runtime& rt) {
    int v = p->kernel_variant;
    if (v < 0 || v > 34 || v == 5 || v == 6) return fail(RYDIFF_EINVAL, "kernel_variant must be 0..4 or 7..34");
    rt.pair_mode = (v == 17 || v >= 20) ? 1 : (v == 18 ? -1 : 0);
    rt.pair_bwd_off = v == 19;
    rt.pair_bwd_stage = (v == 21 || v == 29) ? 1 : (v >= 20 ? -1 : 0);
    static constexpr int kPhases[9] = {4, 1, 2, 3, 5, 6, 7, 4, 0};
    rt.pair_phases = (v >= 22 && v <= 30) ? kPhases[v - 22] : -1;
    const bool pair_forced = v == 17 || v >= 20;
    rt.pair_pace_fwd = (v == 31 || v == 33) ? 1 : (v == 34 ? 2 : (pair_forced ? 0 : -1));
    rt.pair_pace_bwd = (v == 32 || v == 33) ? 1 : (pair_forced ? 0 : -1);
    if (v >= 17) v = 0;
    rt.generic_direct = v == 9;
    if (v == 9) v = 1;
    rt.force_three = v == 7 ? 1 : (v == 11 ? 2 : 0);
    rt.plain_tile_order = v == 12;
    rt.tile_mode = v == 13 ? 12 : (v == 14 ? 13 : (v == 15 ? 11 : (v == 16 ? 10 : 0)));
    if (v == 7 || v == 11 || v >= 12) v = 0;
    rt.force_xcd = v == 10;
    if (v == 10) v = 0;
    rt.variant = v;
    rt.chain_lgt = v == 3 ? 8 : (v == 4 ? 10 : 9);
    rt.shard_recv = p->shard_recv;
    rt.shard_exchange = p->shard_exchange;
    rt.shard_user = p->shard_user;
    return RYDIFF_OK;
}

ChainGeom chain_geom(const Runtime& rt) {
    const int N = rt.pl.NL;
    int lt = kTileBits;
    if (rt.pl.ga.flagged) lt = kTileBits;
    else if (rt.tile_mode == 13) lt = N > kWideTileBits ? kWideTileBits : kTileBits;
    else if (rt.tile_mode == 10 || rt.tile_mode == 11) lt = (N > rt.tile_mode && N <= 2 * rt.tile_mode - 2) ? rt.tile_mode : kTileBits;
    else if (rt.small_tiles) lt = 11;
    else if (rt.tile_mode == 0 && rt.variant == 0 && !rt.force_three && !rt.force_xcd && ((N >= 21 && N <= 24) || N >= 29))
        lt = kWideTileBits;
    ChainGeom g{lt, 2};
    if (lt == kWideTileBits) g.layouts = N <= 24 ? 2 : 3;
    else if (rt.force_three == 2 && N <= 24) g.layouts = 2;
    else if (N >= 23 || (rt.force_three == 1 && N >= 21)) g.layouts = 3;
    return g;
}

int upload_words(hipStream_t stream, void* dst, const void* src, size_t bytes) {
    const size_t nwords = (bytes + 7) / 8;
    const unsigned char* sp = static_cast<const unsigned char*>(src);
    unsigned long long* dp = static_cast<unsigned long long*>(dst);
    for (size_t w0 = 0; w0 < nwords; w0 += kUploadWords) {
        const int n = int(std::min<size_t>(kUploadWords, nwords - w0));
        UploadChunk c;
        const size_t have = std::min<size_t>(size_t(n) * 8, bytes - w0 * 8);
        memcpy(c.w, sp + w0 * 8, have);
        if (have < size_t(n) * 8) memset(reinterpret_cast<unsigned char*>(c.w) + have, 0, size_t(n) * 8 - have);
        hipLaunchKernelGGL(k_upload, dim3(1), dim3(256), 0, stream, dp + w0, c, n);
        LAUNCH_CHECK();
    }
    return RYDIFF_OK;
}

struct Runtime;
void assign_pauli_layouts(Runtime& rt);
int upload_pauli_tables(const Plan& pl, char* ws, hipStream_t stream);
int upload_dm_tables(const Plan& pl, char* ws, hipStream_t stream);

std::mutex g_poly_mutex;
std::vector<PolyDesign> g_poly_cache;

PolyDesign cached_design(double rho, double tol) {
    std::lock_guard<std::mutex> lk(g_poly_mutex);
    for (const auto& d : g_poly_cache)
        if (d.rho == rho && d.tol == tol) return d;
    PolyDesign d = design_polynomial(rho, tol);
    if (g_poly_cache.size() > 64) g_poly_cache.clear();
    g_poly_cache.push_back(d);
    return d;
}

template <class Masks, class Counts>
void fill_detuning(Masks& dmask, Counts& dcnt, const Plan& pl) {
    for (int g = 0; g < pl.gd.n; ++g) {
        dmask[g] = pl.gd.amp_index_mask[g];
        dcnt[g] = pl.gd.count[g];
    }
}

void fill_group_args(const Plan& pl, GroupArgs& g) {
    g.ga = pl.ga.n;
    g.gd = pl.gd.n;
    for (int q = 0; q < pl.ga.n; ++q) g.amask[q] = pl.ga.amp_index_mask[q];
    fill_detuning(g.dmask, g.dcnt, pl);
    g.cond = pl.ga.flagged;
}

double generator_half_width(const Plan& pl, double lo, double hi) { return std::max(0.5 * (hi - lo), 1e-9) + pl.pair_radius; }

int64_t step_factor_count(const Runtime& rt, int k) {
    int64_t f = 0;
    for (int e = rt.pl.step_begin[k]; e < rt.pl.step_begin[k + 1]; ++e) f += int64_t(rt.pl.stages[e].nsub) * rt.poly.degree;
    return f;
}

int finish_runtime(Runtime& rt, double lo, double hi) {
    Plan& pl = rt.pl;
    if (!(hi >= lo) || !std::isfinite(hi) || !std::isfinite(lo)) return fail(RYDIFF_EINVAL, "non-finite spectral bounds (NaN/Inf in the coefficient tables?)");
    lo -= pl.pair_radius;
    hi += pl.pair_radius;
    rt.sigma = 0.5 * (hi + lo);
    rt.width = std::max(0.5 * (hi - lo), 1e-9);
    double rho_d = 1e-6;
    for (auto& s : pl.stages) {
        const double rho = s.tau * rt.width;
        s.nsub = std::max(1, int(std::ceil(rho / kRhoCap)));
        rho_d = std::max(rho_d, rho / s.nsub);
    }
    const double q = std::pow(2.0, std::ceil(std::log2(rho_d) * 16.0) / 16.0);
    rt.rho_design = q;
    rt.poly = cached_design(rt.rho_design, pl.tol);
    if (rt.poly.degree < 1 || rt.poly.roots.empty()) return fail(RYDIFF_EINVAL, "polynomial design failed");
    rt.total_factors = 0;
    rt.max_step_factors = 0;
    for (int k = 0; k < pl.T; ++k) {
        const int f = int(step_factor_count(rt, k));
        rt.total_factors += f;
        rt.max_step_factors = std::max(rt.max_step_factors, f);
    }
    fill_group_args(pl, rt.garg);
    if (pl.ga.flagged) {
        rt.generic_direct = true;
    }
    rt.parg.n = pl.n_pair;
    for (int t = 0; t < pl.n_pair; ++t) {
        rt.parg.ma[t] = pl.pair_ma[t];
        rt.parg.mb[t] = pl.pair_mb[t];
        unsigned dm = 0;
        for (int w = 0; w < 2; ++w)
            for (int own = 0; own < 4; ++own)
                for (int s = 0; s < 4; ++s) {
                    const double* e = pl.pair_tab.data() + size_t(t) * 64 + size_t(w) * 32 + size_t(own * 4 + s) * 2;
                    if (e[0] != 0.0 || e[1] != 0.0) dm |= 1u << (own ^ s);
                }
        rt.parg.dl[t] = uint8_t(dm);
    }
    return RYDIFF_OK;
}

int run_stats(const RydProblem* p, const Plan& pl, void* scratch, hipStream_t stream, double& lo, double& hi, int& flags) {
    StatsArgs sa{};
    sa.amp = static_cast<const double2*>(p->amp_tables);
    sa.det = p->det_tables;
    sa.u_pairs = p->u_pairs;
    sa.n_samples = pl.n_samples;
    sa.Ka = pl.Ka;
    sa.Kd = pl.Kd;
    sa.n_pairs = pl.N * (pl.N - 1) / 2;
    sa.Bc = pl.Bc;
    sa.ga = pl.ga.n;
    sa.gd = pl.gd.n;
    for (int g = 0; g < pl.ga.n; ++g) {
        sa.amem[g] = pl.ga.members[g];
        sa.acnt[g] = pl.ga.count[g];
    }
    for (int g = 0; g < pl.gd.n; ++g) {
        sa.dmem[g] = pl.gd.members[g];
        sa.dcnt[g] = pl.gd.nq[g];
    }
    sa.dones = pl.gd.flagged;
    HIP_TRY(hipMemsetAsync(scratch, 0, 8 * sizeof(double), stream));
    const int ns = std::max(pl.n_samples, 1);
    dim3 grid((ns + 127) / 128, pl.Bc);
    hipLaunchKernelGGL(k_table_stats, grid, dim3(128), 0, stream, static_cast<unsigned long long*>(scratch), sa);
    LAUNCH_CHECK();
    double host[6] = {0, 0, 0, 0, 0, 0};
    HIP_TRY(hipMemcpyAsync(host, scratch, sizeof(host), hipMemcpyDeviceToHost, stream));
    HIP_TRY(hipStreamSynchronize(stream));
    double wsum = 1.0;
    for (const auto& s : pl.stages) {
        double a = 0.0;
        for (int q = 0; q < 4; ++q) a += std::fabs(s.w[q]);
        wsum = std::max(wsum, a);
    }
    hi = host[3] + wsum * (host[1] + host[0]);
    lo = -host[5] - wsum * (host[2] + host[0]);
    flags = (host[4] != 0.0) ? 1 : 0;
    return RYDIFF_OK;
}

bool small_tiles_win(const Runtime& rt, bool with_gradients) {
    const Plan& pl = rt.pl;
    if (rt.pair_mode == 1 || rt.variant != 0 || rt.force_three || rt.force_xcd || rt.tile_mode != 0 || pl.shard_bits || pl.n_pair || pl.ga.flagged) return false;
    if (pl.N < 13 || pl.N > 19) return false;
    const size_t amps = size_t(pl.B) << pl.N;
    if (amps > (size_t(1) << 19)) return false;
    return with_gradients ? (amps >= (size_t(7) << 16) && pl.N >= 14) : amps > (size_t(1) << 18);
}

bool few_tiles(const Runtime& rt, bool with_gradients) {
    const Plan& pl = rt.pl;
    if (rt.small_tiles) return false;
    if (rt.pair_mode == 1 || rt.variant != 0 || rt.force_three || rt.force_xcd || (rt.tile_mode != 0 && rt.tile_mode != kTileBits) || pl.shard_bits) return false;
    return (size_t(pl.B) << pl.N) <= (size_t(1) << (with_gradients ? 19 : 18));
}

bool full_tape_possible(const Plan& pl) {
    if (pl.shard_bits) return false;
    if (pl.N <= kPersistBwdMaxQubits) return pl.ga.n <= kPersistGroups && pl.gd.n <= kPersistGroups;
    return pl.n_pair == 0;
}

bool partial_tape_possible(const Runtime& rt) {
    return full_tape_possible(rt.pl) && rt.pl.N > kTileBits;
}

struct TapeMap {
    int k0 = 0;
    std::vector<int64_t> bprefix;
    int64_t entries = 0;
};

TapeMap partial_tape_map(const Runtime& rt, int tape_steps) {
    const Plan& pl = rt.pl;
    TapeMap m;
    m.k0 = std::max(0, pl.T - std::max(tape_steps, 0));
    m.bprefix.assign(pl.T + 1, 0);
    for (int k = 0; k < pl.T; ++k) m.bprefix[k + 1] = m.bprefix[k] + (k >= m.k0 ? std::max<int64_t>(step_factor_count(rt, k) - 1, 0) : 0);
    m.entries = int64_t(pl.T + 1) + m.bprefix[pl.T];
    return m;
}

int plan_runtime(const RydProblem* p, const RydPlanInfo* info, void* scratch, size_t scratch_bytes, int& need_tape, bool need_backward,
                 hipStream_t stream, Runtime& rt, double& lo, double& hi, size_t& need) {
    std::string err;
    if (!p) return fail(RYDIFF_EINVAL, "null problem");
    int rc = decode_variant(p, rt);
    if (rc) return rc;
    if (!build_plan(p, rt.pl, err)) return fail(err.find("not implemented") != std::string::npos ? RYDIFF_ENOTIMPL : RYDIFF_EINVAL, err);
    if (!scratch) return fail(RYDIFF_EINVAL, "null workspace");
    if (info) {
        lo = info->spectral_lo;
        hi = info->spectral_hi;
        rt.flags = info->flags;
    } else {
        if (scratch_bytes < RYDIFF_PLAN_SCRATCH_BYTES) return fail(RYDIFF_EWORKSPACE, "workspace too small");
        rc = run_stats(p, rt.pl, scratch, stream, lo, hi, rt.flags);
        if (rc) return rc;
    }
    rt.real_amp_grad = p->real_amp_grad != 0;
    if (!build_plan(p, rt.pl, err, generator_half_width(rt.pl, lo, hi))) return fail(RYDIFF_EINVAL, err);
    rc = finish_runtime(rt, lo, hi);
    if (rc) return rc;
    if (need_tape == 2 && !full_tape_possible(rt.pl)) need_tape = 1;
    if (need_tape == 3 && (!partial_tape_possible(rt) || p->tape_steps < 1)) need_tape = 1;
    rt.small_tiles = small_tiles_win(rt, need_backward || need_tape != 0);
    rt.prefer_direct = few_tiles(rt, need_backward || need_tape != 0);
    need = carve(rt.pl, need_tape, need_backward, std::max(rt.max_step_factors - 1, 1), rt.total_factors,
                 need_tape == 3 ? partial_tape_map(rt, p->tape_steps).entries : 0);
    return RYDIFF_OK;
}

int launch_expand(const Plan& pl, char* ws, const double2* amp, const double* det, double* coef, hipStream_t stream) {
    const size_t E = pl.stages.size();
    ExpandArgs ea{};
    ea.amp = amp;
    ea.det = det;
    ea.st = reinterpret_cast<const StageDev*>(ws + pl.off_meta_idx);
    ea.coef = coef;
    ea.E = int(E);
    ea.n_samples = pl.n_samples;
    ea.Ka = amp ? pl.Ka : 0;
    ea.Kd = det ? pl.Kd : 0;
    ea.NC = pl.NC;
    ea.ga = pl.ga.n;
    ea.gd = pl.gd.n;
    for (int g = 0; g < pl.ga.n; ++g) ea.amem[g] = pl.ga.members[g];
    for (int g = 0; g < pl.gd.n; ++g) ea.dmem[g] = pl.gd.members[g];
    hipLaunchKernelGGL(k_expand_coeffs, dim3((unsigned(E) + 127) / 128, pl.Bc), dim3(128), 0, stream, ea);
    LAUNCH_CHECK();
    return RYDIFF_OK;
}

int prepare(const RydProblem* p, const RydPlanInfo* info, void* workspace, size_t workspace_bytes, int need_tape,
            bool need_backward, hipStream_t stream, Runtime& rt) {
    double lo, hi;
    size_t need;
    int rc = plan_runtime(p, info, workspace, workspace_bytes, need_tape, need_backward, stream, rt, lo, hi, need);
    if (rc) return rc;
    Plan& pl = rt.pl;
    if (pl.shard_bits && pl.n_pair)
        return fail(RYDIFF_ENOTIMPL, "state-sharded runs do not take dense pair terms");
    if (pl.shard_bits) rt.generic_direct = true;
    if (workspace_bytes < need)
        return fail(RYDIFF_EWORKSPACE, "workspace too small: need " + std::to_string(need) + " bytes, got " + std::to_string(workspace_bytes));
    char* ws = static_cast<char*>(workspace);
    const size_t E = pl.stages.size();
    {
        std::vector<StageDev> sd(E);
        for (size_t e = 0; e < E; ++e) sd[e] = {pl.stages[e].w[0], pl.stages[e].w[1], pl.stages[e].idx[0], pl.stages[e].idx[1]};
        rc = upload_words(stream, ws + pl.off_meta_idx, sd.data(), E * sizeof(StageDev));
        if (rc) return rc;
    }
    if (pl.n_pair) {
        rc = upload_words(stream, ws + pl.off_pair, pl.pair_tab.data(), pl.pair_tab.size() * sizeof(double));
        if (rc) return rc;
        rt.parg.tab = reinterpret_cast<const double2*>(ws + pl.off_pair);
    }
    if (pl.n_pobs) {
        assign_pauli_layouts(rt);
        rc = upload_pauli_tables(pl, ws, stream);
        if (rc) return rc;
    }
    if (pl.dm_n) {
        rc = upload_dm_tables(pl, ws, stream);
        if (rc) return rc;
    }
    if (pl.NC > 0) {
        const int rc2 = launch_expand(pl, ws, static_cast<const double2*>(p->amp_tables), p->det_tables,
                                      reinterpret_cast<double*>(ws + pl.off_coef), stream);
        if (rc2) return rc2;
    }
    double* udiag = reinterpret_cast<double*>(ws + pl.off_udiag);
    if (pl.N > 1) {
        if (pl.shard_bits)
            hipLaunchKernelGGL(k_build_udiag, dim3((pl.dim + 255) / 256, pl.B), dim3(256), 0, stream, udiag, p->u_pairs, pl.N, uint32_t(pl.dim),
                               pl.NL, pl.rank_first);
        else
            hipLaunchKernelGGL(k_build_udiag, dim3((pl.dim + 255) / 256), dim3(256), 0, stream, udiag, p->u_pairs, pl.N, uint32_t(pl.dim));
        LAUNCH_CHECK();
    } else {
        HIP_TRY(hipMemsetAsync(udiag, 0, pl.dim * sizeof(double), stream));
    }
    if (pl.NL > kTileBits && pl.NL <= 30) {
        const ChainGeom g = chain_geom(rt);
        const unsigned tiles = unsigned((size_t(1) << pl.N) >> g.lt);
        const size_t tile_amps = size_t(1) << g.lt;
        double* split = split_tables(pl, ws, g.lt);
        for (int l = 0; l < g.layouts; ++l) {
            const LayoutDesc d = chain_layout(pl.NL, l, g);
            double* utt = split + l * rt.per_layout(g.lt);
            hipLaunchKernelGGL(k_build_split, dim3(unsigned((tile_amps + tiles + 255) / 256)), dim3(256), 0, stream, utt, utt + tile_amps,
                               p->u_pairs, pl.N, d.lo, d.hs, d.hb, tiles, g.lt);
            LAUNCH_CHECK();
        }
    }
    return RYDIFF_OK;
}

struct FactorScalars {
    double gr, gi, br, bi;
};

int shard_signal(const Runtime& rt, int phase, const void* src) {
    if (!rt.pl.shard_bits || rt.pl.shard_self) return RYDIFF_OK;
    if (rt.shard_exchange(rt.shard_user, phase, src, rt.pl.dim * sizeof(double2)) != 0)
        return fail(RYDIFF_EHIP, phase == 0 ? "shard_exchange failed to post the slab exchange" : "shard_exchange failed to wait for the partner slabs");
    return RYDIFF_OK;
}

FactorScalars factor_scalars(const Runtime& rt, double tau_sub, int f) {
    using cd = std::complex<double>;
    const cd z = rt.poly.roots[f];
    const cd denom = rt.rho_design * z;
    cd beta = -tau_sub / denom;
    cd gamma = cd(1.0, 0.0) + tau_sub * rt.sigma / denom;
    if (f == rt.poly.degree - 1) {
        const cd kappa = std::exp(cd(0.0, -tau_sub * rt.sigma)) * rt.poly.p0;
        beta *= kappa;
        gamma *= kappa;
    }
    return {gamma.real(), gamma.imag(), beta.real(), beta.imag()};
}

struct ChainItem {
    int stage;
    FactorScalars s;
};

void build_step_chain(const Runtime& rt, int k, std::vector<ChainItem>& chain) {
    chain.clear();
    const Plan& pl = rt.pl;
    for (int e = pl.step_begin[k]; e < pl.step_begin[k + 1]; ++e) {
        const Stage& st = pl.stages[e];
        const double tau_sub = st.tau / st.nsub;
        for (int s = 0; s < st.nsub; ++s)
            for (int f = 0; f < rt.poly.degree; ++f) chain.push_back({e, factor_scalars(rt, tau_sub, f)});
    }
}

void shard_groups(const Plan& pl, int (&grp)[kShardMaxBits]) {
    for (int k = 0; k < kShardMaxBits; ++k) {
        grp[k] = -1;
        if (k >= pl.shard_bits) continue;
        for (int g = 0; g < pl.ga.n; ++g)
            if (pl.ga.amp_index_mask[g] >> (pl.NL + k) & 1u) grp[k] = g;
    }
}

struct PauliInject {
    const Runtime* rt = nullptr;
    char* ws = nullptr;
    hipStream_t stream = nullptr;
    const double2* gstate = nullptr;
    const double* gexp = nullptr;
    const double* ov_gexp = nullptr;
    const double2* ov_targets = nullptr;
    const double* rdm_gexp = nullptr;
    const double* moments_gexp = nullptr;
    const double* dm_gexp = nullptr;
    const double* dm_diag = nullptr;
    const double2* dm_phi = nullptr;
    double2* buf = nullptr;
    std::function<const double2*(int)> state_at;
};
const double2* observable_cotangent(const PauliInject& pi, int k);

struct InjectSource {
    const double2* gstate = nullptr;
    const double* gexp = nullptr;
    const double* obs = nullptr;
    int n_obs = 0;
    const PauliInject* pauli = nullptr;
    bool any() const { return gstate || gexp || pauli; }
};

template <class Args>
void fill_inject(Args& a, const InjectSource& inj, int k, const Plan& pl) {
    if (k < 0 || !inj.any()) return;
    if (inj.pauli) a.inj_gstate = observable_cotangent(*inj.pauli, k);
    else a.inj_gstate = inj.gstate ? inj.gstate + size_t(k) * pl.B * pl.dim : nullptr;
    a.inj_gexp = inj.gexp ? inj.gexp + size_t(k) * pl.B : nullptr;
    a.inj_obs = inj.obs;
    a.inj_n_obs = inj.n_obs;
    a.inj_ostride = long(pl.T + 1) * pl.B;
}

template <class Args>
void fill_shard(Args& a, const Runtime& rt) {
    const Plan& pl = rt.pl;
    if (!pl.shard_bits) return;
    a.sh_bits = pl.shard_bits;
    a.sh_nl = pl.NL;
    a.sh_rank_first = pl.rank_first;
    a.sh_self = pl.shard_self ? 1 : 0;
    for (int k = 0; k < pl.shard_bits; ++k) a.sh_rem[k] = pl.shard_self ? nullptr : static_cast<const double2*>(rt.shard_recv[k]);
    shard_groups(pl, a.sh_grp);
}

template <auto Kernel>
int set_max_dynamic_lds_once(size_t bytes) {
    static std::atomic<bool> attr_set{false};
    if (!attr_set.load(std::memory_order_acquire)) {
        HIP_TRY(hipFuncSetAttribute(reinterpret_cast<const void*>(Kernel), hipFuncAttributeMaxDynamicSharedMemorySize, int(bytes)));
        attr_set.store(true, std::memory_order_release);
    }
    return RYDIFF_OK;
}

struct BatchSlice {
    int first = 0, count = 0;
    bool xcd = false;
};

struct SweepCtx {
    const Runtime& rt;
    const RydProblem* p;
    char* ws;
    hipStream_t stream;
    size_t sv;
    TapeMap tmap;
    bool full_tape() const { return rt.pl.tape_mode == 2; }
    bool partial_tape() const { return rt.pl.tape_mode == 3; }
};

struct ForwardCtx : SweepCtx {
    const double2* psi0 = nullptr;
    const double2* start = nullptr;
    double2* buf[2] = {};
    double2* tape = nullptr;
    double2* tape_b = nullptr;
    double2* copy_out = nullptr;
    double2* final_dst = nullptr;
    const double* obs = nullptr;
    double* expect_out = nullptr;
    bool want_exp = false;
    double* pauli_out = nullptr;
    double* overlap_out = nullptr;
    double* rdm_out = nullptr;
    double* moments_out = nullptr;
    double* moments_drec = nullptr;
    double* dm_out = nullptr;
    const double* shot_u = nullptr;
    uint32_t* shots_out = nullptr;
};

struct BackwardCtx : SweepCtx {
    const double2* tape = nullptr;
    const double2* tape_b = nullptr;
    std::vector<int64_t> fprefix;
    double2* lam[2] = {};
    double2* chainbuf = nullptr;
    double* ge = nullptr;
    double* wtot = nullptr;
    bool want_tau = false;
    InjectSource inj;
    PauliInject pauli;
    bool taped(int k) const { return full_tape() || (partial_tape() && k >= tmap.k0); }
    const double2* state_at(int k) const { return tape + size_t(full_tape() ? fprefix[k] : k) * sv; }
};

}
```

### pulser-diff_amd/csrc/rydiff.hip

```cpp
#include <hip/hip_runtime.h>

#include <algorithm>
#include <atomic>
#include <complex>
#include <cstdio>
#include <cstdlib>
#include <cstring>
#include <functional>
#include <mutex>
#include <type_traits>
#include <string>
#include <vector>

#include "../../include/rydiff.h"
#include "plan.hpp"
#include "poly.hpp"

using namespace rydiff;

#include "common.hpp"
#include "direct_kernels.hpp"
#include "chain_kernels.hpp"
#include "pair_kernels.hpp"
#include "persist_kernels.hpp"
#include "lane_kernels.hpp"
#include "pauli_kernels.hpp"
#include "overlap_kernels.hpp"
#include "rdm_kernels.hpp"
#include "moments_kernels.hpp"
#include "shots_kernels.hpp"
#include "dm_kernels.hpp"
#include "tangent_kernels.hpp"
#include "gram_kernels.hpp"
#include "fisher_kernels.hpp"
static_assert(sizeof(PersistFactor) == 48, "plan.hpp sizes the factor table with 48 bytes per entry");

#include "runtime.hpp"
#include "pauli_launch.hpp"
#include "direct_launch.hpp"
#include "chain_launch.hpp"
#include "pair_launch.hpp"
#include "shots_launch.hpp"
#include "rdm_launch.hpp"
#include "moments_launch.hpp"
#include "dm_launch.hpp"
#include "overlap_launch.hpp"
#include "tangent_launch.hpp"
#include "gram_launch.hpp"
#include "fisher_launch.hpp"
#include "persist_launch.hpp"

namespace {

void describe_kernels(const Runtime& rt, const RydProblem* p, bool backward, RydPlanInfo* info) {
    const Plan& pl = rt.pl;
    auto b = [](bool v) { return v ? "true" : "false"; };
    info->kernel_fwd[0] = info->kernel_bwd[0] = 0;
    if (info->kernel_family == 3) {
        const bool pairs = pl.tape_mode != 3 && xcd_group_size(rt, false) == 0 && pair_enabled(rt);
        const bool pairs_bwd = xcd_group_size(rt, true) == 0 && pair_bwd_enabled(rt);
        const bool fast = pl.ga.n == 1 && (pl.ga.amp_index_mask[0] & ((1u << pl.NL) - 1u)) == (1u << pl.NL) - 1u && !pl.ga.flagged;
        for (int bwd = 0; bwd <= (backward ? 1 : 0); ++bwd) {
            const bool cplx = (rt.flags & 1) != 0 || (bwd && !p->real_amp_grad);
            const int lgt = rt.variant == 0 ? ((bwd && cplx) ? 9 : 10) : rt.chain_lgt;
            const bool res = xcd_group_size(rt, bwd != 0) > 0;
            if (!bwd && pairs && pair_pace_fwd(rt))
                std::snprintf(info->kernel_fwd, sizeof(info->kernel_fwd), "k_chain2<%d,10,true,3,%d>", kTileBits, pair_pace_fwd(rt));
            else if (!bwd && pairs)
                std::snprintf(info->kernel_fwd, sizeof(info->kernel_fwd), "k_chain2<%d,10,%s,%d>", kTileBits, b(pair_vec_major(rt)), pair_through(rt));
            else if (bwd && pairs_bwd && pair_pace_bwd(rt))
                std::snprintf(info->kernel_bwd, sizeof(info->kernel_bwd), "k_chain2_bwd<%d,10,true,3,false,%d>", kTileBits, pair_pace_bwd(rt));
            else if (bwd && pairs_bwd)
                std::snprintf(info->kernel_bwd, sizeof(info->kernel_bwd), "k_chain2_bwd<%d,10,%s,%d,%s>", kTileBits, b(pair_vec_major(rt)),
                              pair_through(rt), b(pair_bwd_dma(rt)));
            else if (chain_geom(rt).lt == kWideTileBits)
                std::snprintf(bwd ? info->kernel_bwd : info->kernel_fwd, sizeof(info->kernel_fwd), "k_chain_wide<%d,%s,%s,%s>", kWideTileBits,
                              b(cplx), b(bwd != 0), b(fast));
            else
                std::snprintf(bwd ? info->kernel_bwd : info->kernel_fwd, sizeof(info->kernel_fwd), "k_chain<%d,%d,%s,%s,%s,%s>", chain_geom(rt).lt,
                              chain_geom(rt).lt == kTileBits ? lgt : 10, b(cplx), b(bwd != 0), b(fast), b(res));
        }
    } else if (info->kernel_family == 2) {
        if (direct_global_ok(rt)) {
            std::snprintf(info->kernel_fwd, sizeof(info->kernel_fwd), "k_factor_direct_global<%d,%s>", pl.N, b(pl.N <= 13));
            if (backward) std::snprintf(info->kernel_bwd, sizeof(info->kernel_bwd), "k_factor_bwd_direct_global<%d,%s>", pl.N, b(pl.N <= 13));
        } else {
            std::snprintf(info->kernel_fwd, sizeof(info->kernel_fwd), "k_factor_direct");
            if (backward) std::snprintf(info->kernel_bwd, sizeof(info->kernel_bwd), "k_factor_bwd_direct");
        }
    } else {
        std::snprintf(info->kernel_fwd, sizeof(info->kernel_fwd), info->kernel_family == 0 ? "k_lanes_fwd (N=%d)" : "k_persist<%d,...>", pl.N);
        if (backward && persist_bwd_enabled(rt))
            std::snprintf(info->kernel_bwd, sizeof(info->kernel_bwd), info->kernel_family == 0 ? "k_lanes_bwd (N=%d)" : "k_persist_bwd<%d,...>", pl.N);
        else if (backward && direct_global_ok(rt))
            std::snprintf(info->kernel_bwd, sizeof(info->kernel_bwd), "k_factor_bwd_direct_global<%d,%s>", pl.N, b(pl.N <= 13));
        else if (backward)
            std::snprintf(info->kernel_bwd, sizeof(info->kernel_bwd), "k_factor_bwd_direct");
    }
}

int launch_expect(const ForwardCtx& c, const double2* psi, int k) {
    const Plan& pl = c.rt.pl;
    const unsigned red_blocks = unsigned(std::min<size_t>((pl.dim + 255) / 256, 1024));
    hipLaunchKernelGGL(k_expect_diag, dim3(red_blocks, pl.B), dim3(256), 0, c.stream, psi, c.obs, c.expect_out, pl.n_obs, pl.T + 1, k, pl.B,
                       uint32_t(pl.dim), c.rt.obs_bstride());
    LAUNCH_CHECK();
    return RYDIFF_OK;
}

int bind_expect_rows(ForwardCtx& c, double* expect_out) {
    const Plan& pl = c.rt.pl;
    const ExpectRows rows(pl);
    c.obs = c.p->obs_diag;
    c.expect_out = expect_out;
    c.want_exp = expect_out && pl.n_obs > 0;
    c.pauli_out = rows.at(expect_out, ExpectRows::Pauli);
    c.overlap_out = rows.at(expect_out, ExpectRows::Overlap);
    c.rdm_out = rows.at(expect_out, ExpectRows::Rdm);
    c.moments_out = rows.at(expect_out, ExpectRows::Moments);
    c.dm_out = rows.at(expect_out, ExpectRows::DmTrace, ExpectRows::End);
    if (expect_out && rows.total()) HIP_TRY(hipMemsetAsync(expect_out, 0, rows.size() * sizeof(double), c.stream));
    return RYDIFF_OK;
}

int forward_chained(const ForwardCtx& c) {
    const Runtime& rt = c.rt;
    const Plan& pl = rt.pl;
    const size_t sv = c.sv;
    hipStream_t stream = c.stream;
    std::vector<ChainItem> all, chain;
    std::vector<int> step_of_end;
    std::vector<int64_t> b_entry;
    for (int k = 0; k < pl.T; ++k) {
        build_step_chain(rt, k, chain);
        for (size_t i = 0; i < chain.size(); ++i) {
            all.push_back(chain[i]);
            step_of_end.push_back(i + 1 == chain.size() ? k + 1 : 0);
            if (c.partial_tape()) b_entry.push_back((k >= c.tmap.k0 && i + 1 < chain.size()) ? c.tmap.bprefix[k] + int64_t(i) : -1);
        }
    }
    const int grp = xcd_group_size(rt, false);
    for (int b0 = 0; b0 < pl.B; b0 += (grp ? grp : pl.B)) {
        const BatchSlice bs{b0, std::min(grp ? grp : pl.B, pl.B - b0), grp > 0};
        int flip = 0;
        auto dst = [&](int i) -> double2* {
            if (c.full_tape()) return c.tape + size_t(i + 1) * sv;
            if (step_of_end[i] && c.tape) return c.tape + size_t(step_of_end[i]) * sv;
            if (c.partial_tape() && b_entry[i] >= 0) return c.tape_b + size_t(b_entry[i]) * sv;
            if (bs.xcd) return c.buf[0];
            flip ^= 1;
            return c.buf[flip];
        };
        auto done = [&](int i, const double2* out) -> int {
            if (c.final_dst && step_of_end[i] == pl.T)
                HIP_TRY(hipMemcpyAsync(c.final_dst + size_t(bs.first) * pl.dim, out + size_t(bs.first) * pl.dim,
                                       size_t(bs.count) * pl.dim * sizeof(double2), hipMemcpyDeviceToDevice, stream));
            if (c.copy_out && step_of_end[i])
                HIP_TRY(hipMemcpyAsync(c.copy_out + size_t(step_of_end[i]) * sv + size_t(bs.first) * pl.dim, out + size_t(bs.first) * pl.dim,
                                       size_t(bs.count) * pl.dim * sizeof(double2), hipMemcpyDeviceToDevice, stream));
            if (step_of_end[i]) return launch_observables_expect(c, out, 0, step_of_end[i], 1, bs);
            return RYDIFF_OK;
        };
        auto exp_slot = [&](int i, ChainStep& cs) {
            if (c.want_exp && step_of_end[i]) {
                cs.obs = c.obs;
                cs.n_obs = pl.n_obs;
                cs.exp_ostride = long(pl.T + 1) * pl.B;
                cs.expect_slot = c.expect_out + size_t(step_of_end[i]) * pl.B;
            }
        };
        const int rc = (!c.partial_tape() && !bs.xcd && pair_enabled(rt))
                           ? run_chain2(rt, c.ws, all, c.start, dst, c.full_tape(), done, exp_slot, bs, stream)
                           : run_chain(rt, c.ws, all, c.start, dst, done, exp_slot, false, bs, stream);
        if (rc) return rc;
    }
    return RYDIFF_OK;
}

int forward_direct(const ForwardCtx& c) {
    const Runtime& rt = c.rt;
    const Plan& pl = rt.pl;
    const size_t sv = c.sv;
    std::vector<ChainItem> chain;
    const double2* cur = c.start;
    int pp = 0;
    bool exp_fused = false;
    size_t gfac = 0;
    for (int k = 0; k < pl.T; ++k) {
        build_step_chain(rt, k, chain);
        for (size_t i = 0; i < chain.size(); ++i, ++gfac) {
            const bool last = (i + 1 == chain.size());
            double2* dst;
            if (c.full_tape() && c.tape) dst = c.tape + (gfac + 1) * sv;
            else if (last && c.tape) dst = c.tape + size_t(k + 1) * sv;
            else if (c.partial_tape() && k >= c.tmap.k0) dst = c.tape_b + size_t(c.tmap.bprefix[k] + int64_t(i)) * sv;
            else {
                dst = c.buf[pp];
                if (dst == cur) dst = c.buf[pp ^ 1];
                pp ^= 1;
            }
            const bool want_here = c.want_exp && last;
            int rc = shard_signal(rt, 0, cur);
            if (!rc) rc = shard_signal(rt, 1, nullptr);
            if (rc) return rc;
            rc = launch_factor(rt, c.ws, cur, dst, chain[i].stage, chain[i].s, c.stream, want_here ? c.obs : nullptr,
                               want_here ? c.expect_out + size_t(k + 1) * pl.B : nullptr, &exp_fused);
            if (rc) return rc;
            cur = dst;
        }
        if (c.copy_out) HIP_TRY(hipMemcpyAsync(c.copy_out + size_t(k + 1) * sv, cur, pl.state_bytes, hipMemcpyDeviceToDevice, c.stream));
        if (c.want_exp && !exp_fused) {
            const int rc = launch_expect(c, cur, k + 1);
            if (rc) return rc;
        }
        if (const int rc = launch_observables_expect(c, cur, 0, k + 1, 1, BatchSlice{0, pl.B, false})) return rc;
    }
    if (c.final_dst) HIP_TRY(hipMemcpyAsync(c.final_dst, cur, pl.state_bytes, hipMemcpyDeviceToDevice, c.stream));
    return RYDIFF_OK;
}

int gather_factor_inputs(const BackwardCtx& c, const BatchSlice& bs, int k, int k_hi, const std::vector<ChainItem>& chain,
                         std::vector<const double2*>& xs) {
    const Runtime& rt = c.rt;
    const int M = int(chain.size());
    const size_t sv = c.sv;
    xs.assign(M + 1, nullptr);
    xs[0] = c.state_at(k);
    xs[M] = c.state_at(k_hi + 1);
    if (c.full_tape()) {
        for (int i = 1; i < M; ++i) xs[i] = c.tape + size_t(c.fprefix[k] + i) * sv;
    } else if (c.taped(k_hi)) {
        int i = 0;
        for (int kk = k; kk <= k_hi; ++kk) {
            const int mk = int(c.fprefix[kk + 1] - c.fprefix[kk]);
            for (int j = 0; j < mk; ++j, ++i) xs[i] = j == 0 ? c.state_at(kk) : c.tape_b + size_t(c.tmap.bprefix[kk] + j - 1) * sv;
        }
    } else if (M - 1 > rt.pl.chain_slots) {
        return fail(RYDIFF_EWORKSPACE, "internal: chain buffers too small");
    } else if (chain_enabled(rt) && M > 1) {
        for (int i = 1; i < M; ++i) xs[i] = c.chainbuf + size_t(i - 1) * sv;
        auto dst = [&](int i) -> double2* { return c.chainbuf + size_t(i) * sv; };
        auto done = [&](int, const double2*) -> int { return RYDIFF_OK; };
        auto no_exp = [&](int, ChainStep&) {};
        return run_chain(rt, c.ws, chain, xs[0], dst, done, no_exp, true, bs, c.stream);
    } else {
        for (int i = 1; i < M; ++i) {
            double2* dst = c.chainbuf + size_t(i - 1) * sv;
            int rc = shard_signal(rt, 0, xs[i - 1]);
            if (!rc) rc = shard_signal(rt, 1, nullptr);
            if (rc) return rc;
            rc = launch_factor(rt, c.ws, xs[i - 1], dst, chain[i - 1].stage, chain[i - 1].s, c.stream);
            if (rc) return rc;
            xs[i] = dst;
        }
    }
    return RYDIFF_OK;
}

int adjoint_chained(const BackwardCtx& c, const BatchSlice& bs, const std::vector<ChainItem>& chain, const std::vector<const double2*>& xs,
                    const std::vector<int>& save_k, int& cl) {
    const Runtime& rt = c.rt;
    double2* lam[2] = {c.lam[0], c.lam[1]};
    auto dot_h = [&](int stage, const double2* g, const double2* xout) -> int {
        return c.want_tau ? launch_dot_h(rt, c.ws, stage, g, xout, bs, c.stream) : RYDIFF_OK;
    };
    return (!bs.xcd && pair_bwd_enabled(rt)) ? run_chain2_bwd(rt, c.ws, chain, xs, save_k, lam[cl], lam, cl, c.wtot, dot_h, bs, c.inj, c.stream)
                                             : run_chain_bwd(rt, c.ws, chain, xs, save_k, lam[cl], lam, cl, c.wtot, dot_h, c.want_tau, bs, c.inj, c.stream);
}

int adjoint_direct(const BackwardCtx& c, const BatchSlice& bs, const std::vector<ChainItem>& chain, const std::vector<const double2*>& xs,
                   const std::vector<int>& save_k, int& cl) {
    const Runtime& rt = c.rt;
    const int M = int(chain.size());
    for (int i = M; i >= 1; --i) {
        const ChainItem& it = chain[i - 1];
        int rc = shard_signal(rt, 0, c.lam[cl]);
        if (!rc) rc = shard_signal(rt, 1, nullptr);
        if (rc) return rc;
        if (c.want_tau && (i == M || chain[i].stage != it.stage)) {
            rc = launch_dot_h(rt, c.ws, it.stage, c.lam[cl], xs[i], bs, c.stream);
            if (rc) return rc;
        }
        rc = launch_factor_bwd(rt, c.ws, c.lam[cl], xs[i - 1], c.lam[cl ^ 1], it.stage, it.s, c.wtot, c.inj, save_k[i - 1], c.stream);
        if (rc) return rc;
        cl ^= 1;
    }
    return RYDIFF_OK;
}

int adjoint_sweep(const BackwardCtx& c, const BatchSlice& bs, int& cl) {
    const Runtime& rt = c.rt;
    const Plan& pl = rt.pl;
    const bool chained = chain_enabled(rt);
    std::vector<ChainItem> chain, part;
    std::vector<const double2*> xs;
    std::vector<int> save_k;
    cl = 0;
    for (int k = pl.T - 1; k >= 0; --k) {
        const int k_hi = k;
        if (c.taped(k_hi) && chained) {
            while (k > 0 && c.taped(k - 1) && c.fprefix[k_hi + 1] - c.fprefix[k - 1] < (int64_t(1) << 16)) --k;
        }
        chain.clear();
        save_k.clear();
        for (int kk = k; kk <= k_hi; ++kk) {
            build_step_chain(rt, kk, part);
            for (size_t i = 0; i < part.size(); ++i) save_k.push_back(i == 0 ? kk : -1);
            chain.insert(chain.end(), part.begin(), part.end());
        }
        int rc = gather_factor_inputs(c, bs, k, k_hi, chain, xs);
        if (!rc) rc = chained ? adjoint_chained(c, bs, chain, xs, save_k, cl) : adjoint_direct(c, bs, chain, xs, save_k, cl);
        if (rc) return rc;
    }
    return RYDIFF_OK;
}

int scatter_gradients(const BackwardCtx& c, void* g_amp, double* g_det, double* g_u, double* g_tsave) {
    const Plan& pl = c.rt.pl;
    hipStream_t stream = c.stream;
    const size_t E = pl.stages.size();
    if (g_amp) HIP_TRY(hipMemsetAsync(g_amp, 0, size_t(pl.Bc) * pl.Ka * pl.n_samples * 16, stream));
    if (g_det) HIP_TRY(hipMemsetAsync(g_det, 0, size_t(pl.Bc) * pl.Kd * pl.n_samples * 8, stream));
    if (g_tsave) HIP_TRY(hipMemsetAsync(g_tsave, 0, size_t(pl.T + 1) * 8, stream));
    if ((g_amp && pl.Ka) || (g_det && pl.Kd) || g_tsave) {
        char* m = c.ws + pl.off_meta2;
        if (g_tsave) {
            std::vector<StageBwdDev> sb(E);
            for (size_t e = 0; e < E; ++e) {
                const Stage& st = pl.stages[e];
                sb[e] = {st.tau_scale, st.tnw[0], st.tnw[1], st.tn[0], st.tn[1], st.t_hi, st.t_lo};
            }
            const int rc = upload_words(stream, m, sb.data(), E * sizeof(StageBwdDev));
            if (rc) return rc;
        }
        ScatterArgs sa{};
        sa.ge = c.ge;
        sa.st = reinterpret_cast<const StageDev*>(c.ws + pl.off_meta_idx);
        sa.sb = reinterpret_cast<const StageBwdDev*>(m);
        sa.inv_dt = pl.dt > 0.0 ? 1.0 / pl.dt : 0.0;
        sa.amp = static_cast<const double2*>(c.p->amp_tables);
        sa.det = c.p->det_tables;
        sa.g_amp = static_cast<double2*>(g_amp);
        sa.g_det = g_det;
        sa.g_tsave = g_tsave;
        sa.E = int(E);
        sa.n_samples = pl.n_samples;
        sa.Ka = pl.Ka;
        sa.Kd = pl.Kd;
        sa.NC = pl.NC;
        sa.ga = pl.ga.n;
        sa.gd = pl.gd.n;
        for (int g = 0; g < pl.ga.n; ++g) sa.amem[g] = pl.ga.members[g];
        for (int g = 0; g < pl.gd.n; ++g) sa.dmem[g] = pl.gd.members[g];
        hipLaunchKernelGGL(k_scatter_grads, dim3((unsigned(E) + 63) / 64, pl.Bc), dim3(64), 0, stream, sa);
        LAUNCH_CHECK();
    }
    const int npairs = pl.N * (pl.N - 1) / 2;
    if (g_u && npairs > 0) {
        HIP_TRY(hipMemsetAsync(g_u, 0, size_t(npairs) * 8, stream));
        const unsigned nb = unsigned(std::min<size_t>((pl.dim + 255) / 256, 256));
        hipLaunchKernelGGL(k_ugrad, dim3(nb, npairs), dim3(256), 0, stream, g_u, c.wtot, pl.N, uint32_t(pl.dim), pl.shard_bits ? pl.B : 0, pl.NL,
                           pl.rank_first);
        LAUNCH_CHECK();
    }
    return RYDIFF_OK;
}

}

extern "C" {

const char* rydiff_last_error(void) { return g_last_error.c_str(); }
const char* rydiff_version(void) { return "rydiff 0.4 (gfx950)"; }
size_t rydiff_sizeof_problem(void) { return sizeof(RydProblem); }
size_t rydiff_sizeof_plan_info(void) { return sizeof(RydPlanInfo); }
size_t rydiff_sizeof_tangent(void) { return sizeof(RydTangent); }

#ifdef RYDIFF_TIMELINE
int rydiff_debug_timeline(unsigned long long* host_buf, int n_entries) {
    return hipMemcpyFromSymbol(host_buf, HIP_SYMBOL(g_timeline), size_t(n_entries) * sizeof(unsigned long long)) == hipSuccess ? 0 : -3;
}
#endif

int rydiff_design_polynomial(double rho, double tol, int max_degree, int* degree, double* roots_reim, double* p0_reim, double* max_err) {
    if (!(rho > 0.0) || !degree || !roots_reim || max_degree < 1) return fail(RYDIFF_EINVAL, "bad arguments");
    PolyDesign d = design_polynomial(rho, tol, max_degree);
    if (d.degree < 1) return fail(RYDIFF_EINVAL, "polynomial design failed");
    *degree = d.degree;
    for (int i = 0; i < d.degree; ++i) {
        roots_reim[2 * i] = d.roots[i].real();
        roots_reim[2 * i + 1] = d.roots[i].imag();
    }
    if (p0_reim) {
        p0_reim[0] = d.p0.real();
        p0_reim[1] = d.p0.imag();
    }
    if (max_err) *max_err = d.max_err;
    return RYDIFF_OK;
}

int rydiff_plan(const RydProblem* p, int need_tape, int need_backward, void* scratch, void* stream_, RydPlanInfo* info) {
    if (!p) return fail(RYDIFF_EINVAL, "null problem");
    if (!info || !scratch) return fail(RYDIFF_EINVAL, "null info or scratch");
    if (need_tape < 0 || need_tape > 3) return fail(RYDIFF_EINVAL, "need_tape must be 0..3");
    Runtime rt;
    double lo, hi;
    size_t ws;
    const int rc = plan_runtime(p, nullptr, scratch, RYDIFF_PLAN_SCRATCH_BYTES, need_tape, need_backward != 0, static_cast<hipStream_t>(stream_),
                                rt, lo, hi, ws);
    if (rc) return rc;
    info->spectral_lo = lo;
    info->spectral_hi = hi;
    info->rho_design = rt.rho_design;
    info->degree = rt.poly.degree;
    info->n_stages = int(rt.pl.stages.size());
    info->max_step_factors = rt.max_step_factors;
    info->flags = rt.flags;
    info->total_factors = rt.total_factors;
    info->workspace_bytes = ws;
    info->tape_mode = need_tape;
    if (persist_enabled(rt)) info->kernel_family = lanes_enabled(rt) ? 0 : 1;
    else info->kernel_family = chain_enabled(rt) ? 3 : 2;
    describe_kernels(rt, p, need_backward != 0, info);
    return RYDIFF_OK;
}

int rydiff_forward(const RydProblem* p, const RydPlanInfo* info, const void* psi0, void* states_out, double* expect_out,
                   void* workspace, size_t workspace_bytes, int need_tape, void* stream_) {
    hipStream_t stream = static_cast<hipStream_t>(stream_);
    if (!psi0) return fail(RYDIFF_EINVAL, "null psi0");
    Runtime rt;
    int rc = prepare(p, info, workspace, workspace_bytes, need_tape >= 2 ? need_tape : (states_out ? 0 : need_tape), false, stream, rt);
    if (rc) return rc;
    const Plan& pl = rt.pl;
    ForwardCtx c{{rt, p, static_cast<char*>(workspace), stream, size_t(pl.B) * pl.dim}};
    c.psi0 = c.start = static_cast<const double2*>(psi0);
    c.buf[0] = reinterpret_cast<double2*>(c.ws + pl.off_buf0);
    c.buf[1] = reinterpret_cast<double2*>(c.ws + pl.off_buf1);
    if (c.partial_tape()) c.tmap = partial_tape_map(rt, p->tape_steps);
    const bool ws_tape = c.full_tape() || c.partial_tape();
    double2* sout = static_cast<double2*>(states_out);
    if (p->final_state_only && sout) {
        if (need_tape || persist_enabled(rt))
            return fail(RYDIFF_EINVAL, "final_state_only needs the launch-per-factor kernels (more than 12 qubits or a sharded run) and no tape");
        c.final_dst = sout;
        sout = nullptr;
    }
    c.tape = (sout && !ws_tape) ? sout : (pl.tape_mode ? reinterpret_cast<double2*>(c.ws + pl.off_tape) : nullptr);
    c.copy_out = ws_tape ? sout : nullptr;
    c.tape_b = c.partial_tape() ? c.tape + size_t(pl.T + 1) * c.sv : nullptr;
    if (c.tape) {
        HIP_TRY(hipMemcpyAsync(c.tape, psi0, pl.state_bytes, hipMemcpyDeviceToDevice, stream));
        c.start = c.tape;
    }
    if (c.copy_out) HIP_TRY(hipMemcpyAsync(c.copy_out, psi0, pl.state_bytes, hipMemcpyDeviceToDevice, stream));
    if (pl.n_shots) {
        c.shot_u = p->shot_uniforms;
        c.shots_out = p->shots_out;
    }
    rc = bind_expect_rows(c, expect_out);
    if (rc) return rc;
    if (c.want_exp) {
        rc = launch_expect(c, c.start, 0);
        if (rc) return rc;
    }
    if (persist_enabled(rt)) return forward_persist(c);
    rc = launch_observables_expect(c, c.start, 0, 0, 1, BatchSlice{0, pl.B, false});
    if (rc) return rc;
    return chain_enabled(rt) ? forward_chained(c) : forward_direct(c);
}

int rydiff_backward(const RydProblem* p, const RydPlanInfo* info, const void* states, const void* grad_states,
                    const double* grad_expect, void* g_amp, double* g_det, double* g_u, double* g_tsave, void* g_psi0,
                    void* workspace, size_t workspace_bytes, int need_tape, void* stream_) {
    hipStream_t stream = static_cast<hipStream_t>(stream_);
    if (!states && !need_tape) return fail(RYDIFF_EINVAL, "backward needs the trajectory: pass states or use the workspace tape");
    Runtime rt;
    int rc = prepare(p, info, workspace, workspace_bytes, need_tape >= 2 ? need_tape : (states ? 0 : need_tape), true, stream, rt);
    if (rc) return rc;
    const Plan& pl = rt.pl;
    if (!states && !pl.tape_mode) return fail(RYDIFF_EINVAL, "backward needs the trajectory: pass states or use the workspace tape");
    BackwardCtx c{{rt, p, static_cast<char*>(workspace), stream, size_t(pl.B) * pl.dim}};
    c.tape = (pl.tape_mode >= 2 || !states) ? reinterpret_cast<const double2*>(c.ws + pl.off_tape) : static_cast<const double2*>(states);
    if (c.partial_tape()) {
        c.tmap = partial_tape_map(rt, p->tape_steps);
        c.tape_b = c.tape + size_t(pl.T + 1) * c.sv;
    }
    c.fprefix.assign(pl.T + 1, 0);
    for (int k = 0; k < pl.T; ++k) c.fprefix[k + 1] = c.fprefix[k] + step_factor_count(rt, k);
    c.lam[0] = reinterpret_cast<double2*>(c.ws + pl.off_buf0);
    c.lam[1] = reinterpret_cast<double2*>(c.ws + pl.off_buf1);
    c.chainbuf = reinterpret_cast<double2*>(c.ws + pl.off_chain);
    c.ge = rt.ge(c.ws, 0);
    c.wtot = g_u ? reinterpret_cast<double*>(c.ws + pl.off_wtot) : nullptr;
    c.want_tau = g_tsave != nullptr;
    const bool have_gexp = grad_expect && pl.n_obs > 0;
    c.inj.gstate = static_cast<const double2*>(grad_states);
    c.inj.gexp = have_gexp ? grad_expect : nullptr;
    c.inj.obs = p->obs_diag;
    c.inj.n_obs = have_gexp ? pl.n_obs : 0;
    const ExpectRows rows(pl);
    if (grad_expect && rows.total() > rows.count(ExpectRows::Diag)) {
        c.pauli.rt = &rt;
        c.pauli.ws = c.ws;
        c.pauli.stream = stream;
        c.pauli.gstate = c.inj.gstate;
        c.pauli.gexp = rows.at(grad_expect, ExpectRows::Pauli);
        c.pauli.ov_gexp = rows.at(grad_expect, ExpectRows::Overlap);
        c.pauli.ov_targets = static_cast<const double2*>(p->overlap_targets);
        c.pauli.rdm_gexp = rows.at(grad_expect, ExpectRows::Rdm);
        c.pauli.moments_gexp = rows.at(grad_expect, ExpectRows::Moments);
        c.pauli.dm_gexp = rows.at(grad_expect, ExpectRows::DmTrace, ExpectRows::End);
        c.pauli.dm_diag = p->dm_diag;
        c.pauli.dm_phi = static_cast<const double2*>(p->dm_fid_targets);
        if (pl.n_rdm && (rc = rdm_apply_prepare())) return rc;
        c.pauli.buf = reinterpret_cast<double2*>(c.ws + pl.off_pauli_cot);
        c.pauli.state_at = [&c](int k) { return c.state_at(k); };
        c.inj.pauli = &c.pauli;
    }

    HIP_TRY(hipMemsetAsync(c.ge, 0, size_t(pl.Bc) * pl.stages.size() * rt.ge_rec() * sizeof(double), stream));
    if (c.wtot) HIP_TRY(hipMemsetAsync(c.wtot, 0, pl.dim * (pl.shard_bits ? size_t(pl.B) : 1) * sizeof(double), stream));
    int cl = 0;
    if (persist_bwd_enabled(rt)) {
        rc = backward_persist(c);
        if (rc) return rc;
    } else {
        hipLaunchKernelGGL(k_inject, dim3(unsigned((pl.dim + 255) / 256), pl.B), dim3(256), 0, stream, c.lam[0],
                           c.inj.pauli ? observable_cotangent(c.pauli, pl.T) : (c.inj.gstate ? c.inj.gstate + size_t(pl.T) * c.sv : nullptr), c.state_at(pl.T), c.inj.obs, c.inj.gexp, pl.n_obs,
                           pl.T + 1, pl.T, pl.B, uint32_t(pl.dim), 1, rt.obs_ostride(), rt.obs_bstride());
        LAUNCH_CHECK();
        const int grp = chain_enabled(rt) ? xcd_group_size(rt, true) : 0;
        for (int b0 = 0; b0 < pl.B; b0 += (grp ? grp : pl.B)) {
            rc = adjoint_sweep(c, BatchSlice{b0, std::min(grp ? grp : pl.B, pl.B - b0), grp > 0}, cl);
            if (rc) return rc;
        }
    }
    if (g_psi0) HIP_TRY(hipMemcpyAsync(g_psi0, c.lam[cl], pl.state_bytes, hipMemcpyDeviceToDevice, stream));
    return scatter_gradients(c, g_amp, g_det, g_u, g_tsave);
}

size_t rydiff_tangent_workspace_bytes_flags(const RydProblem* p, const RydPlanInfo* info, int n_dir, int flags) {
    Runtime rt;
    TangentLayout lay;
    return tangent_plan(p, info, n_dir, flags, rt, lay) ? 0 : lay.total;
}

size_t rydiff_tangent_workspace_bytes(const RydProblem* p, const RydPlanInfo* info, int n_dir) {
    return rydiff_tangent_workspace_bytes_flags(p, info, n_dir, 0);
}

size_t rydiff_geometry_workspace_bytes_flags(const RydProblem* p, const RydPlanInfo* info, int n_dir, int flags) {
    Runtime rt;
    TangentLayout lay;
    if (tangent_plan(p, info, n_dir, flags, rt, lay)) return 0;
    if (geometry_validate(p)) return 0;
    return geometry_layout(rt.pl, lay, n_dir).total;
}

size_t rydiff_geometry_workspace_bytes(const RydProblem* p, const RydPlanInfo* info, int n_dir) {
    return rydiff_geometry_workspace_bytes_flags(p, info, n_dir, 0);
}

size_t rydiff_fisher_workspace_bytes_flags(const RydProblem* p, const RydPlanInfo* info, int n_dir, int flags) {
    Runtime rt;
    TangentLayout lay;
    if (tangent_plan(p, info, n_dir, flags, rt, lay)) return 0;
    if (geometry_validate(p)) return 0;
    return fisher_layout(rt.pl, geometry_layout(rt.pl, lay, n_dir), n_dir).total;
}

}

namespace {

int tangent_sweep(const RydProblem* p, const RydPlanInfo* info, const RydTangent* tg, const void* psi0, double* expect_out,
                  double* dexpect_out, bool geometry, void* gram_out, bool fisher, double* cgram_out, void* workspace, size_t workspace_bytes,
                  hipStream_t stream) {
    if (!p) return fail(RYDIFF_EINVAL, "null problem");
    if (!tg) return fail(RYDIFF_EINVAL, "null tangent");
    int rc = tangent_validate(p, info, tg->n_dir, tg->flags);
    if (rc) return rc;
    if (geometry && (rc = geometry_validate(p))) return rc;
    if (!tg->d_amp && !tg->d_det && !tg->d_u && !tg->d_psi0)
        return fail(RYDIFF_EINVAL, "tangent: all of d_amp, d_det, d_u, d_psi0 are NULL (nothing to differentiate)");
    if (!geometry && !dexpect_out) return fail(RYDIFF_EINVAL, "null dexpect_out");
    if (geometry && !fisher && !gram_out) return fail(RYDIFF_EINVAL, "null gram_out");
    if (fisher && !cgram_out) return fail(RYDIFF_EINVAL, "null cgram_out");
    if (!psi0) return fail(RYDIFF_EINVAL, "null psi0");
    Runtime rt0;
    TangentLayout lay;
    rc = tangent_plan(p, info, tg->n_dir, tg->flags, rt0, lay);
    if (rc) return rc;
    GeometryLayout glay;
    if (geometry) glay = geometry_layout(rt0.pl, lay, tg->n_dir);
    FisherLayout flay;
    if (fisher) flay = fisher_layout(rt0.pl, glay, tg->n_dir);
    const size_t need = fisher ? flay.total : (geometry ? glay.total : lay.total);
    if (!workspace) return fail(RYDIFF_EINVAL, "null workspace");
    if (workspace_bytes < need)
        return fail(RYDIFF_EWORKSPACE, std::string(fisher ? "fisher" : (geometry ? "geometry" : "tangent")) + " workspace too small: need " + std::to_string(need) +
                                           " bytes, got " + std::to_string(workspace_bytes));
    RydProblem q = *p;
    q.kernel_variant = 0;
    Runtime rt;
    rc = prepare(&q, info, workspace, workspace_bytes, 0, false, stream, rt);
    if (rc) return rc;
    const Plan& pl = rt.pl;
    const int D = tg->n_dir;
    char* ws = static_cast<char*>(workspace);
    rc = tangent_tables(rt, &q, tg, ws, lay, stream);
    if (rc) return rc;
    const size_t sv = size_t(pl.B) * pl.dim;
    double2* vec[2] = {reinterpret_cast<double2*>(ws + lay.off_vec[0]), reinterpret_cast<double2*>(ws + lay.off_vec[1])};
    HIP_TRY(hipMemcpyAsync(vec[0], psi0, pl.state_bytes, hipMemcpyDeviceToDevice, stream));
    const int Dp = tangent_padded(D);
    if (tg->d_psi0) {
        HIP_TRY(hipMemcpyAsync(vec[0] + sv, tg->d_psi0, size_t(D) * pl.state_bytes, hipMemcpyDeviceToDevice, stream));
        if (Dp > D) HIP_TRY(hipMemsetAsync(vec[0] + size_t(1 + D) * sv, 0, size_t(Dp - D) * pl.state_bytes, stream));
    } else {
        HIP_TRY(hipMemsetAsync(vec[0] + sv, 0, size_t(Dp) * pl.state_bytes, stream));
    }
    const ExpectRows rows(pl);
    if (rows.total() && dexpect_out) HIP_TRY(hipMemsetAsync(dexpect_out, 0, size_t(D) * rows.size() * sizeof(double), stream));
    ForwardCtx c{{rt, &q, ws, stream, sv}};
    c.psi0 = c.start = vec[0];
    rc = bind_expect_rows(c, expect_out);
    if (rc) return rc;
    if (pl.moments && pl.moment_tiles() > 1) c.moments_drec = reinterpret_cast<double*>(ws + lay.off_dmoments);
    auto save_point = [&](const double2* v, int k) -> int {
        if (c.want_exp)
            if (const int r = launch_expect(c, v, k)) return r;
        if (const int r = launch_observables_expect(c, v, 0, k, 1, BatchSlice{0, pl.B, false})) return r;
        if (dexpect_out)
            if (const int r = launch_expect_tangent(c, v, D, k, dexpect_out)) return r;
        if (geometry && gram_out)
            if (const int r = launch_gram(rt, ws, glay, v, D, k, static_cast<double2*>(gram_out), stream)) return r;
        return fisher ? launch_cfi(rt, ws, flay, v, D, k, cgram_out, stream) : RYDIFF_OK;
    };
    rc = save_point(vec[0], 0);
    if (rc) return rc;
    TangentFactorArgs fa{};
    fill_tangent_factor(fa, rt, ws, lay, tg->d_u != nullptr);
    std::vector<ChainItem> chain;
    int cur = 0;
    for (int k = 0; k < pl.T; ++k) {
        build_step_chain(rt, k, chain);
        for (const ChainItem& it : chain) {
            rc = launch_factor_tangent(fa, rt, ws, lay, D, vec[cur], vec[cur ^ 1], it.stage, it.s, stream);
            if (rc) return rc;
            cur ^= 1;
        }
        rc = save_point(vec[cur], k + 1);
        if (rc) return rc;
    }
    return RYDIFF_OK;
}

}

extern "C" {

int rydiff_forward_tangent(const RydProblem* p, const RydPlanInfo* info, const RydTangent* tg, const void* psi0, double* expect_out,
                           double* dexpect_out, void* workspace, size_t workspace_bytes, void* stream_) {
    return tangent_sweep(p, info, tg, psi0, expect_out, dexpect_out, false, nullptr, false, nullptr, workspace, workspace_bytes,
                         static_cast<hipStream_t>(stream_));
}

int rydiff_forward_geometry(const RydProblem* p, const RydPlanInfo* info, const RydTangent* tg, const void* psi0, double* expect_out,
                            double* dexpect_out, void* gram_out, void* workspace, size_t workspace_bytes, void* stream_) {
    return tangent_sweep(p, info, tg, psi0, expect_out, dexpect_out, true, gram_out, false, nullptr, workspace, workspace_bytes,
                         static_cast<hipStream_t>(stream_));
}

int rydiff_forward_fisher(const RydProblem* p, const RydPlanInfo* info, const RydTangent* tg, const void* psi0, double* expect_out,
                          double* dexpect_out, void* gram_out, double* cgram_out, void* workspace, size_t workspace_bytes, void* stream_) {
    return tangent_sweep(p, info, tg, psi0, expect_out, dexpect_out, true, gram_out, true, cgram_out, workspace, workspace_bytes,
                         static_cast<hipStream_t>(stream_));
}

int rydiff_apply_factor(const RydProblem* p, const double* c_amp_reim, const double* c_det, const double* gamma_reim,
                        const double* beta_reim, const void* x, void* y, int n_remote, const void* const* remote,
                        const double* remote_coef_reim, int reuse_diag, void* workspace, size_t workspace_bytes, void* stream_) {
    hipStream_t stream = static_cast<hipStream_t>(stream_);
    if (!p) return fail(RYDIFF_EINVAL, "null problem");
    if (!x || !y || !workspace || !gamma_reim || !beta_reim) return fail(RYDIFF_EINVAL, "null buffer");
    if ((p->n_amp_terms > 0 && !c_amp_reim) || (p->n_det_terms > 0 && !c_det))
        return fail(RYDIFF_EINVAL, "missing coefficient values (c_amp_reim / c_det) for the problem's terms");
    if (n_remote < 0 || n_remote > kMaxRemote || (n_remote > 0 && (!remote || !remote_coef_reim)))
        return fail(RYDIFF_EINVAL, "bad remote vector list");
    RydProblem q = *p;
    double dummy_t[2] = {0.0, 1.0};
    if (q.n_tsave < 2 || !q.tsave) {
        q.n_tsave = 2;
        q.tsave = dummy_t;
    }
    q.solver = RYDIFF_SOLVER_KRYLOV_SE;
    Runtime rt;
    std::string err;
    if (!build_plan(&q, rt.pl, err)) return fail(RYDIFF_EINVAL, err);
    Plan& pl = rt.pl;
    if (pl.n_pair) return fail(RYDIFF_ENOTIMPL, "rydiff_apply_factor does not take pair terms");
    fill_group_args(pl, rt.garg);
    const size_t need = align_up(pl.dim * sizeof(double));
    if (workspace_bytes < need) return fail(RYDIFF_EWORKSPACE, "workspace too small: need " + std::to_string(need));
    FactorArgs fa{};
    fa.use_inline = 1;
    for (int g = 0; g < pl.ga.n; ++g)
        for (int k = 0; k < pl.Ka; ++k)
            if (pl.ga.members[g] >> k & 1ull) {
                fa.coef_inline[g] += c_amp_reim[2 * k];
                fa.coef_inline[pl.ga.n + g] += c_amp_reim[2 * k + 1];
            }
    for (int g = 0; g < pl.gd.n; ++g)
        for (int k = 0; k < pl.Kd; ++k)
            if (pl.gd.members[g] >> k & 1ull) fa.coef_inline[2 * pl.ga.n + g] += 2.0 * c_det[k];
    double* udiag = static_cast<double*>(workspace);
    if (!reuse_diag) {
        if (pl.N > 1) {
            hipLaunchKernelGGL(k_build_udiag, dim3((pl.dim + 255) / 256), dim3(256), 0, stream, udiag, p->u_pairs, pl.N, uint32_t(pl.dim));
            LAUNCH_CHECK();
        } else {
            HIP_TRY(hipMemsetAsync(udiag, 0, pl.dim * sizeof(double), stream));
        }
    }
    fa.xin = static_cast<const double2*>(x);
    fa.xout = static_cast<double2*>(y);
    fa.udiag = udiag;
    fa.coef = nullptr;
    fa.coef_bstride = 0;
    fa.dim = uint32_t(pl.dim);
    fa.gr = gamma_reim[0];
    fa.gi = gamma_reim[1];
    fa.br = beta_reim[0];
    fa.bi = beta_reim[1];
    fa.g = rt.garg;
    fa.n_remote = n_remote;
    for (int k = 0; k < n_remote; ++k) {
        fa.remote[k] = static_cast<const double2*>(remote[k]);
        fa.rc[2 * k] = remote_coef_reim[2 * k];
        fa.rc[2 * k + 1] = remote_coef_reim[2 * k + 1];
    }
    hipLaunchKernelGGL(k_factor_direct, dim3(unsigned((pl.dim + 255) / 256), pl.B), dim3(256), 0, stream, fa);
    LAUNCH_CHECK();
    return RYDIFF_OK;
}

int rydiff_apply_hamiltonian(const RydProblem* p, const double* c_amp_reim, const double* c_det, const void* x, void* y,
                             void* workspace, size_t workspace_bytes, void* stream_) {
    const double zero[2] = {0.0, 0.0}, one[2] = {1.0, 0.0};
    return rydiff_apply_factor(p, c_amp_reim, c_det, zero, one, x, y, 0, nullptr, nullptr, 0, workspace, workspace_bytes, stream_);
}

}
```

Measured before the change: 4479 time-steps/s.

## Store P_X v on the full tape in place of mid-block states for the block adjoint

Result: faster. 4595 time-steps/s, median of 6 (+2.6%).

```diff
diff --git a/pulser-diff_amd/_native.py b/pulser-diff_amd/_native.py
--- a/pulser-diff_amd/_native.py
+++ b/pulser-diff_amd/_native.py
@@ -258,7 +258,7 @@
     return roots[: 2 * m].view(np.complex128).copy(), complex(p0[0], p0[1]), err.value
 
 
-_KNOWN_VARIANTS = (0, 1, 2, 3, 4, 7, 8, 9, 10, 11, 12, 13, 14, 15, 16, 17, 18, 19, 20, 21, 22, 23, 24, 25, 26, 27, 28, 29, 30, 31, 32, 33, 34)
+_KNOWN_VARIANTS = (0, 1, 2, 3, 4, 7, 8, 9, 10, 11, 12, 13, 14, 15, 16, 17, 18, 19, 20, 21, 22, 23, 24, 25, 26, 27, 28, 29, 30, 31, 32, 33, 34, 35)
 _tls = threading.local()
 
 
diff --git a/pulser-diff_amd/csrc/chain_kernels.hpp b/pulser-diff_amd/csrc/chain_kernels.hpp
--- a/pulser-diff_amd/csrc/chain_kernels.hpp
+++ b/pulser-diff_amd/csrc/chain_kernels.hpp
@@ -229,7 +229,7 @@
 }
 
 #ifdef RYDIFF_TIMELINE
-__device__ unsigned long long g_timeline[4096 * 11];
+__device__ unsigned long long g_timeline[4096 * 12];
 #define RYDIFF_TL(slot)                                                                                   \
     do {                                                                                                  \
         if (threadIdx.x == 0 && blockIdx.y == 0 && blockIdx.x < 4096 && a.has_p && a.has_q)               \
diff --git a/pulser-diff_amd/csrc/pair_kernels.hpp b/pulser-diff_amd/csrc/pair_kernels.hpp
--- a/pulser-diff_amd/csrc/pair_kernels.hpp
+++ b/pulser-diff_amd/csrc/pair_kernels.hpp
@@ -283,6 +283,7 @@
     double k_r, k_i;
     double ga_r, ga_i, ba_r, ba_i;
     double cba_r, cba_i, cbb_r, cbb_i;
+    double cgb_r, cgb_i;
     int lo, hs, hb;
     uint32_t dim;
     int has_p, has_q;
@@ -315,10 +316,11 @@
            (DMA ? size_t(kChain2BwdXbLds) * (size_t(1) << LGT) * sizeof(double2) : 0);
 }
 
-template <int LT, int LGT, bool ORD, int WT, bool DMA, int PACE = 0>
+template <int LT, int LGT, bool ORD, int WT, bool DMA, int PACE = 0, bool XW = false>
 __global__ __launch_bounds__(1 << LGT) void k_chain2_bwd(Chain2BwdArgs a) {
     constexpr int NT = 1 << LGT, R = 1 << (LT - LGT), NW = NT / 64;
     static_assert(WT >= 0 && WT <= 3);
+    static_assert(!XW || (ORD && WT == 3 && !DMA && !PACE && R == 4), "P_X x_b on the tape: one instantiation");
     static_assert(PACE >= 0 && PACE <= 1 && (!PACE || (ORD && !DMA && R == 4)), "pacing: the vector-major register-staged kernel, four elements per thread");
     constexpr int XBL = DMA ? kChain2BwdXbLds : 0;
     static_assert(XBL <= R && (2 * NW * sizeof(double)) % sizeof(double2) == 0);
@@ -360,23 +362,31 @@
         cdet_fin = a.coef_fin[bt * a.coef_bstride + 2];
         cdet_sta = a.coef_sta[bt * a.coef_bstride + 2];
     }
+    [[maybe_unused]] double2 xa[R];
 #pragma unroll
     for (int r = 0; r < R; ++r) {
         const unsigned i = unsigned(r) * NT + tid;
         xg[r] = xbase | (i & lomask) | ((i >> a.lo) << a.hs);
-        uu[r] = stream_load(a.mu + boff + xg[r]);
-    }
-    if constexpr (ORD && !PACE) __builtin_amdgcn_s_barrier();
-    if constexpr (PACE) {
+        if constexpr (XW) xb[r] = stream_load(a.xb + boff + xg[r]);
+        else uu[r] = stream_load(a.mu + boff + xg[r]);
+    }
+    if constexpr (ORD && !PACE && !XW) __builtin_amdgcn_s_barrier();
+    if constexpr (PACE || XW) {
         __builtin_amdgcn_sched_barrier(0);
         asm volatile("s_waitcnt vmcnt(2)" ::: "memory");
         __builtin_amdgcn_sched_barrier(0);
     }
-#pragma unroll
-    for (int r = 0; r < R; ++r) ww[r] = stream_load(a.w + boff + xg[r]);
-    if constexpr (ORD && !PACE) __builtin_amdgcn_s_barrier();
-    [[maybe_unused]] double2 xa[R];
-    if constexpr (DMA) {
+    if constexpr (!XW) {
+#pragma unroll
+        for (int r = 0; r < R; ++r) ww[r] = stream_load(a.w + boff + xg[r]);
+    }
+    if constexpr (ORD && !PACE && !XW) __builtin_amdgcn_s_barrier();
+    if constexpr (XW) {
+#pragma unroll
+        for (int r = 0; r < R; ++r) xa[r] = stream_load(a.xa + boff + xg[r]);
+#pragma unroll
+        for (int r = 0; r < R; ++r) uu[r] = stream_load(a.mu + boff + xg[r]);
+    } else if constexpr (DMA) {
         const unsigned wv = __builtin_amdgcn_readfirstlane(tid & ~63u);
         double2* xat = tiles + (size_t(1) << LT);
 #pragma unroll
@@ -432,7 +442,9 @@
 #endif
 #pragma unroll
     for (int r = 0; r < R; ++r) {
-        if constexpr (PACE) {
+        if constexpr (XW) {
+            asm volatile("" ::"v"(xb[r].x), "v"(xb[r].y));
+        } else if constexpr (PACE) {
             asm volatile("" ::"v"(uu[r].x), "v"(uu[r].y));
         } else {
             asm volatile("" ::"v"(uu[r].x), "v"(uu[r].y), "v"(ww[r].x), "v"(ww[r].y));
@@ -449,7 +461,39 @@
         const bool two = a.k_r != 0.0 || a.k_i != 0.0;
         {
             double2* etile = tiles + (size_t(buf ^ 1) << LT);
-            if constexpr (PACE) {
+            if constexpr (XW) {
+                __builtin_amdgcn_sched_barrier(0);
+                {
+                    const char* wbase = reinterpret_cast<const char*>(a.w + boff);
+#pragma unroll
+                    for (int r = 0; r < R; ++r) ww[r] = stream_load(reinterpret_cast<const double2*>(wbase + xg[r] * unsigned(sizeof(double2))));
+                }
+                __builtin_amdgcn_sched_barrier(0);
+#pragma unroll
+                for (int r = 0; r < R; ++r) etile[unsigned(r) * NT + tid] = xb[r];
+                if (two) {
+                    __syncthreads();
+                    RYDIFF_TL(11);
+                    double2 sx[R], dsx[R];
+                    partner_sums<LT, LGT, false>(etile, xb, a.fin_mask, tid, sx, dsx);
+#pragma unroll
+                    for (int r = 0; r < R; ++r) {
+                        double d = du[r];
+                        if (a.gd) d += cdet * double(a.dcnt - popc_i(xg[r] & a.dmask));
+                        double2 h1;
+                        h1.x = d * xb[r].x + c * (xa[r].x + sx[r].x);
+                        h1.y = d * xb[r].y + c * (xa[r].y + sx[r].y);
+                        const double2 p = cmul(a.cgb_r, a.cgb_i, xb[r]), q = cmul(a.cbb_r, a.cbb_i, h1);
+                        xa[r] = make_double2(p.x + q.x, p.y + q.y);
+                    }
+                } else {
+#pragma unroll
+                    for (int r = 0; r < R; ++r) {
+                        asm volatile("" ::"v"(xa[r].x), "v"(xa[r].y));
+                        xa[r] = xb[r];
+                    }
+                }
+            } else if constexpr (PACE) {
             } else if constexpr (DMA) {
 #ifdef RYDIFF_TIMELINE
                 RYDIFF_TL(9);
@@ -463,14 +507,14 @@
                 for (int r = 0; r < R; ++r) etile[unsigned(r) * NT + tid] = xa[r];
             }
 #ifdef RYDIFF_TIMELINE
-            if constexpr (!PACE) RYDIFF_TL(10);
+            if constexpr (!PACE && !XW) RYDIFF_TL(10);
 #endif
             double2 s[R], ds[R];
             const double2* mtile = put(uu);
             RYDIFF_TL(1);
             partner_sums<LT, LGT, false>(mtile, uu, a.fin_mask, tid, s, ds);
 #ifdef RYDIFF_TIMELINE
-            if constexpr (PACE) {
+            if constexpr (PACE || XW) {
 #pragma unroll
                 for (int r = 0; r < R; ++r) asm volatile("" ::"v"(ww[r].x), "v"(ww[r].y));
                 RYDIFF_TL(9);
@@ -482,8 +526,9 @@
 #pragma unroll
             for (int r = 0; r < R; ++r) {
                 double2 xav;
-                if constexpr (PACE) xav = xa[r];
+                if constexpr (PACE || XW) xav = xa[r];
                 else xav = etile[unsigned(r) * NT + tid];
+                if constexpr (XW) xb[r] = etile[unsigned(r) * NT + tid];
                 const double d = du[r] + cdet * cnt(r);
                 pm[r] = make_double2(ww[r].x + s[r].x, ww[r].y + s[r].y);
                 const double2 h1 = make_double2(d * uu[r].x + c * pm[r].x, d * uu[r].y + c * pm[r].y);
@@ -499,7 +544,7 @@
         park1<NW>(zc, red, 0);
         zc = 0.0;
         RYDIFF_TL(2);
-        if constexpr (!DMA) {
+        if constexpr (!DMA && !XW) {
 #pragma unroll
             for (int r = 0; r < R; ++r) xb[r] = stream_load(a.xb + boff + xg[r]);
         }
@@ -585,6 +630,7 @@
         for (int r = 0; r < R; ++r) {
             y[r] = uu[r];
             if constexpr (PACE) asm volatile("" ::"v"(ww[r].x), "v"(ww[r].y), "v"(xa[r].x), "v"(xa[r].y));
+            if constexpr (XW) asm volatile("" ::"v"(xa[r].x), "v"(xa[r].y));
         }
     }
     auto flush = [&]() {
diff --git a/pulser-diff_amd/csrc/pair_launch.hpp b/pulser-diff_amd/csrc/pair_launch.hpp
--- a/pulser-diff_amd/csrc/pair_launch.hpp
+++ b/pulser-diff_amd/csrc/pair_launch.hpp
@@ -16,17 +16,38 @@
     return rt.pair_mode == 1 || (rt.pl.N == 20 && rt.pl.B == 1);
 }
 
+std::vector<std::pair<int, int>> forward_blocks(const std::vector<ChainItem>& items) {
+    std::vector<std::pair<int, int>> blk;
+    const int F = int(items.size());
+    for (int i = 0; i < F;) {
+        if (i + 1 < F && items[i + 1].stage == items[i].stage) {
+            blk.push_back({i, i + 1});
+            i += 2;
+        } else {
+            blk.push_back({i, -1});
+            ++i;
+        }
+    }
+    return blk;
+}
+
+int64_t step_block_count(const Runtime& rt, int k) {
+    int64_t b = 0;
+    for (int e = rt.pl.step_begin[k]; e < rt.pl.step_begin[k + 1]; ++e) b += (int64_t(rt.pl.stages[e].nsub) * rt.poly.degree + 1) / 2;
+    return b;
+}
+
 template <class Args>
 void fill_chain2(Args& ca, const Runtime& rt, char* ws, const std::vector<ChainItem>& items, const std::vector<std::pair<int, int>>& blk,
-                 int j, const double2* cur, const BatchSlice& bs) {
+                 int j, const double2* cur, const BatchSlice& bs, int par = 0) {
     const Plan& pl = rt.pl;
     double2* wt[2][2] = {{reinterpret_cast<double2*>(ws + pl.off_pp0), reinterpret_cast<double2*>(ws + pl.off_pp1)},
                          {reinterpret_cast<double2*>(ws + pl.off_pp2), reinterpret_cast<double2*>(ws + pl.off_pp3)}};
     const ChainGeom geom{kTileBits, 2};
-    const int nb = int(blk.size()), L = j & 1;
+    const int nb = int(blk.size()), jp = j + (par & 1), L = jp & 1;
     const LayoutDesc Y = chain_layout(pl.NL, L, geom), X = chain_layout(pl.NL, L ^ 1, geom);
-    ca.w = j ? wt[(j - 1) & 1][0] : cur;
-    ca.t = j ? wt[(j - 1) & 1][1] : cur;
+    ca.w = j ? wt[(jp - 1) & 1][0] : cur;
+    ca.t = j ? wt[(jp - 1) & 1][1] : cur;
     ca.utt = split_tables(pl, ws, kTileBits) + size_t(L) * rt.per_layout(kTileBits);
     ca.vr = ca.utt + (size_t(1) << kTileBits);
     ca.coef_bstride = rt.coef_bstride();
@@ -43,8 +64,8 @@
     ca.b_count = bs.count;
     if (ca.has_p) ca.fin_mask = to_tile_mask(Y, kTileBits, uint32_t(pl.dim - 1) & ~X.bits);
     if (ca.has_q) {
-        ca.w_out = wt[j & 1][0];
-        ca.t_out = wt[j & 1][1];
+        ca.w_out = wt[jp & 1][0];
+        ca.t_out = wt[jp & 1][1];
     }
 }
 
@@ -99,20 +120,12 @@
 
 template <class DstFn, class DoneFn, class ExpFn>
 int run_chain2(const Runtime& rt, char* ws, const std::vector<ChainItem>& items, const double2* start, DstFn dst, bool keep_mid,
-               DoneFn on_done, ExpFn exp_slot, const BatchSlice& bs, hipStream_t stream) {
+               bool wtape, DoneFn on_done, ExpFn exp_slot, const BatchSlice& bs, hipStream_t stream) {
     const Plan& pl = rt.pl;
     const int F = int(items.size());
     if (F <= 0) return RYDIFF_OK;
-    std::vector<std::pair<int, int>> blk;
-    for (int i = 0; i < F;) {
-        if (i + 1 < F && items[i + 1].stage == items[i].stage) {
-            blk.push_back({i, i + 1});
-            i += 2;
-        } else {
-            blk.push_back({i, -1});
-            ++i;
-        }
-    }
+    if (wtape && !keep_mid) return fail(RYDIFF_EINVAL, "internal: P_X v is taped with the full tape only");
+    const std::vector<std::pair<int, int>> blk = forward_blocks(items);
     const unsigned tiles = unsigned(pl.dim >> kTileBits);
     const int nb = int(blk.size());
     const double2* cur = start;
@@ -140,7 +153,8 @@
             ca.g1_i = s1.gi;
             ca.b1_r = s1.br;
             ca.b1_i = s1.bi;
-            ca.vmid_out = (f1 >= 0 && keep_mid) ? dst(f0) : nullptr;
+            ca.vmid_out = (f1 >= 0 && keep_mid && !wtape) ? dst(f0) : nullptr;
+            if (f1 >= 0 && wtape) ca.w = dst(f0);
             ca.y_out = dst(last);
             if (!ca.y_out) return fail(RYDIFF_EINVAL, "internal: chain destination missing");
             ChainStep cs{};
@@ -149,6 +163,10 @@
             ca.expect_slot = cs.expect_slot;
             ca.n_obs = cs.n_obs;
             ca.exp_ostride = cs.exp_ostride;
+        }
+        if (wtape && ca.has_q && blk[j].second >= 0) {
+            ca.w_out = dst(blk[j].first);
+            if (!ca.w_out) return fail(RYDIFF_EINVAL, "internal: chain destination missing");
         }
         int rc = launch_chain2(rt, ca, tiles, stream);
         if (rc) return rc;
@@ -170,6 +188,12 @@
     return !rt.pair_bwd_off && rt.real_amp_grad && pair_enabled(rt) && g.lt == kTileBits && g.layouts == 2;
 }
 
+constexpr bool kPairWtapeDefault = true;
+bool pair_wtape(const Runtime& rt) {
+    const bool sel = rt.pair_wtape ? rt.pair_wtape > 0 : kPairWtapeDefault;
+    return sel && rt.pl.tape_mode == 2 && pair_bwd_enabled(rt) && xcd_group_size(rt, false) == 0 && xcd_group_size(rt, true) == 0;
+}
+
 constexpr bool kPairBwdDmaDefault = false;
 bool pair_bwd_dma(const Runtime& rt) { return rt.pair_bwd_stage ? rt.pair_bwd_stage > 0 : kPairBwdDmaDefault; }
 
@@ -178,19 +202,23 @@
     return rt.pair_pace_bwd >= 0 ? rt.pair_pace_bwd : kPairPaceBwdDefault;
 }
 
-template <int LGT, bool ORD, int WT, bool DMA, int PACE = 0>
+template <int LGT, bool ORD, int WT, bool DMA, int PACE = 0, bool XW = false>
 int launch_chain2_bwd_t(const Chain2BwdArgs& ca, unsigned tiles, hipStream_t stream) {
     constexpr int LT = kTileBits;
     constexpr size_t lds = chain2_bwd_lds_bytes<LT, LGT, DMA>();
     static_assert(lds <= 160 * 1024, "k_chain2_bwd: more LDS than a gfx950 workgroup can have");
-    if (int rc = set_max_dynamic_lds_once<&k_chain2_bwd<LT, LGT, ORD, WT, DMA, PACE>>(lds)) return rc;
-    hipLaunchKernelGGL((k_chain2_bwd<LT, LGT, ORD, WT, DMA, PACE>), dim3(tiles, unsigned(ca.b_count)), dim3(1 << LGT), lds, stream, ca);
+    if (int rc = set_max_dynamic_lds_once<&k_chain2_bwd<LT, LGT, ORD, WT, DMA, PACE, XW>>(lds)) return rc;
+    hipLaunchKernelGGL((k_chain2_bwd<LT, LGT, ORD, WT, DMA, PACE, XW>), dim3(tiles, unsigned(ca.b_count)), dim3(1 << LGT), lds, stream, ca);
     LAUNCH_CHECK();
     return RYDIFF_OK;
 }
 
-int launch_chain2_bwd(const Runtime& rt, const Chain2BwdArgs& ca, unsigned tiles, hipStream_t stream) {
+int launch_chain2_bwd(const Runtime& rt, const Chain2BwdArgs& ca, unsigned tiles, bool wtape, hipStream_t stream) {
     const bool ord = pair_vec_major(rt);
+    if (wtape) {
+        if (!ord || pair_through(rt) != 3 || pair_bwd_dma(rt)) return fail(RYDIFF_EINVAL, "internal: no such block kernel");
+        return launch_chain2_bwd_t<10, true, 3, false, 0, true>(ca, tiles, stream);
+    }
     if (pair_pace_bwd(rt)) return launch_chain2_bwd_t<10, true, 3, false, 1>(ca, tiles, stream);
     if (pair_bwd_dma(rt)) {
         if (ord && pair_through(rt) == 3) return launch_chain2_bwd_t<10, true, 3, true>(ca, tiles, stream);
@@ -205,12 +233,16 @@
 template <class StageEndFn>
 int run_chain2_bwd(const Runtime& rt, char* ws, const std::vector<ChainItem>& items, const std::vector<const double2*>& xs,
                    const std::vector<int>& save_k, const double2* lam_in, double2* lam_bufs[2], int& cl, double* wtot,
-                   StageEndFn on_stage_end, const BatchSlice& bs, const InjectSource& inj, hipStream_t stream) {
+                   StageEndFn on_stage_end, const BatchSlice& bs, const InjectSource& inj, bool wtape, int64_t g_hi, hipStream_t stream) {
     const Plan& pl = rt.pl;
     const int M = int(items.size());
     if (M <= 0) return RYDIFF_OK;
     std::vector<std::pair<int, int>> blk;
-    for (int f = M - 1; f >= 0;) {
+    if (wtape) {
+        blk = forward_blocks(items);
+        std::reverse(blk.begin(), blk.end());
+    }
+    for (int f = wtape ? -1 : M - 1; f >= 0;) {
         if (f >= 1 && items[f - 1].stage == items[f].stage) {
             blk.push_back({f - 1, f});
             f -= 2;
@@ -221,12 +253,13 @@
     }
     const unsigned tiles = unsigned(pl.dim >> kTileBits);
     const int nb = int(blk.size());
+    const int par = wtape ? int(g_hi & 1) : 0;
     const double2* cur = lam_in;
     int rc = on_stage_end(items[M - 1].stage, cur, xs[M]);
     if (rc) return rc;
     for (int j = 0; j <= nb; ++j) {
         Chain2BwdArgs ca{};
-        fill_chain2(ca, rt, ws, items, blk, j, cur, bs);
+        fill_chain2(ca, rt, ws, items, blk, j, cur, bs, par);
         ca.mu = cur;
         ca.xa = ca.xb = cur;
         if (pl.gd.n) {
@@ -260,6 +293,8 @@
             ca.cba_i = sa.bi;
             ca.cbb_r = sb.br;
             ca.cbb_i = sb.bi;
+            ca.cgb_r = sb.gr;
+            ca.cgb_i = sb.gi;
             ca.xb = xs[fb];
             ca.xa = fa >= 0 ? xs[fa] : xs[fb];
             ca.ge_fin = rt.ge(ws, items[fb].stage);
@@ -268,7 +303,7 @@
             if (ca.mu_out == cur) return fail(RYDIFF_EINVAL, "internal: cotangent ping-pong clash");
             fill_inject(ca, inj, save_k[fb], pl);
         }
-        rc = launch_chain2_bwd(rt, ca, tiles, stream);
+        rc = launch_chain2_bwd(rt, ca, tiles, wtape, stream);
         if (rc) return rc;
         if (ca.has_p) {
             cur = ca.mu_out;
diff --git a/pulser-diff_amd/csrc/runtime.hpp b/pulser-diff_amd/csrc/runtime.hpp
--- a/pulser-diff_amd/csrc/runtime.hpp
+++ b/pulser-diff_amd/csrc/runtime.hpp
@@ -58,6 +58,7 @@
     int pair_phases = -1;
     int pair_pace_fwd = -1;
     int pair_pace_bwd = -1;
+    int pair_wtape = 0;
     int chain_lgt = 9;
     void* const* shard_recv = nullptr;
     int (*shard_exchange)(void*, int, const void*, size_t) = nullptr;
@@ -77,7 +78,7 @@
 
 int decode_variant(const RydProblem* p, Runtime& rt) {
     int v = p->kernel_variant;
-    if (v < 0 || v > 34 || v == 5 || v == 6) return fail(RYDIFF_EINVAL, "kernel_variant must be 0..4 or 7..34");
+    if (v < 0 || v > 35 || v == 5 || v == 6) return fail(RYDIFF_EINVAL, "kernel_variant must be 0..4 or 7..35");
     rt.pair_mode = (v == 17 || v >= 20) ? 1 : (v == 18 ? -1 : 0);
     rt.pair_bwd_off = v == 19;
     rt.pair_bwd_stage = (v == 21 || v == 29) ? 1 : (v >= 20 ? -1 : 0);
@@ -86,6 +87,7 @@
     const bool pair_forced = v == 17 || v >= 20;
     rt.pair_pace_fwd = (v == 31 || v == 33) ? 1 : (v == 34 ? 2 : (pair_forced ? 0 : -1));
     rt.pair_pace_bwd = (v == 32 || v == 33) ? 1 : (pair_forced ? 0 : -1);
+    rt.pair_wtape = v == 35 ? 1 : ((pair_forced || v == 19) ? -1 : 0);
     if (v >= 17) v = 0;
     rt.generic_direct = v == 9;
     if (v == 9) v = 1;
@@ -543,6 +545,7 @@
     hipStream_t stream;
     size_t sv;
     TapeMap tmap;
+    bool wtape = false;
     bool full_tape() const { return rt.pl.tape_mode == 2; }
     bool partial_tape() const { return rt.pl.tape_mode == 3; }
 };
diff --git a/pulser-diff_amd/csrc/rydiff.hip b/pulser-diff_amd/csrc/rydiff.hip
--- a/pulser-diff_amd/csrc/rydiff.hip
+++ b/pulser-diff_amd/csrc/rydiff.hip
@@ -68,6 +68,8 @@
                 std::snprintf(info->kernel_fwd, sizeof(info->kernel_fwd), "k_chain2<%d,10,true,3,%d>", kTileBits, pair_pace_fwd(rt));
             else if (!bwd && pairs)
                 std::snprintf(info->kernel_fwd, sizeof(info->kernel_fwd), "k_chain2<%d,10,%s,%d>", kTileBits, b(pair_vec_major(rt)), pair_through(rt));
+            else if (bwd && pairs_bwd && pair_wtape(rt))
+                std::snprintf(info->kernel_bwd, sizeof(info->kernel_bwd), "k_chain2_bwd<%d,10,true,3,false,0,true>", kTileBits);
             else if (bwd && pairs_bwd && pair_pace_bwd(rt))
                 std::snprintf(info->kernel_bwd, sizeof(info->kernel_bwd), "k_chain2_bwd<%d,10,true,3,false,%d>", kTileBits, pair_pace_bwd(rt));
             else if (bwd && pairs_bwd)
@@ -97,6 +99,21 @@
         else if (backward)
             std::snprintf(info->kernel_bwd, sizeof(info->kernel_bwd), "k_factor_bwd_direct");
     }
+}
+
+std::mutex g_tape_format_mutex;
+std::vector<const void*> g_wtape_workspaces;
+
+void tape_format_record(const void* workspace, bool wtape) {
+    std::lock_guard<std::mutex> lk(g_tape_format_mutex);
+    auto it = std::find(g_wtape_workspaces.begin(), g_wtape_workspaces.end(), workspace);
+    if (wtape && it == g_wtape_workspaces.end()) g_wtape_workspaces.push_back(workspace);
+    else if (!wtape && it != g_wtape_workspaces.end()) g_wtape_workspaces.erase(it);
+}
+
+bool tape_format_wtape(const void* workspace) {
+    std::lock_guard<std::mutex> lk(g_tape_format_mutex);
+    return std::find(g_wtape_workspaces.begin(), g_wtape_workspaces.end(), workspace) != g_wtape_workspaces.end();
 }
 
 int launch_expect(const ForwardCtx& c, const double2* psi, int k) {
@@ -170,7 +187,7 @@
             }
         };
         const int rc = (!c.partial_tape() && !bs.xcd && pair_enabled(rt))
-                           ? run_chain2(rt, c.ws, all, c.start, dst, c.full_tape(), done, exp_slot, bs, stream)
+                           ? run_chain2(rt, c.ws, all, c.start, dst, c.full_tape(), c.wtape, done, exp_slot, bs, stream)
                            : run_chain(rt, c.ws, all, c.start, dst, done, exp_slot, false, bs, stream);
         if (rc) return rc;
     }
@@ -258,13 +275,14 @@
 }
 
 int adjoint_chained(const BackwardCtx& c, const BatchSlice& bs, const std::vector<ChainItem>& chain, const std::vector<const double2*>& xs,
-                    const std::vector<int>& save_k, int& cl) {
+                    const std::vector<int>& save_k, int64_t g_hi, int& cl) {
     const Runtime& rt = c.rt;
     double2* lam[2] = {c.lam[0], c.lam[1]};
     auto dot_h = [&](int stage, const double2* g, const double2* xout) -> int {
         return c.want_tau ? launch_dot_h(rt, c.ws, stage, g, xout, bs, c.stream) : RYDIFF_OK;
     };
-    return (!bs.xcd && pair_bwd_enabled(rt)) ? run_chain2_bwd(rt, c.ws, chain, xs, save_k, lam[cl], lam, cl, c.wtot, dot_h, bs, c.inj, c.stream)
+    if (c.wtape && (bs.xcd || !pair_bwd_enabled(rt))) return fail(RYDIFF_EINVAL, "internal: P_X v on the tape without the block adjoint");
+    return (!bs.xcd && pair_bwd_enabled(rt)) ? run_chain2_bwd(rt, c.ws, chain, xs, save_k, lam[cl], lam, cl, c.wtot, dot_h, bs, c.inj, c.wtape, g_hi, c.stream)
                                              : run_chain_bwd(rt, c.ws, chain, xs, save_k, lam[cl], lam, cl, c.wtot, dot_h, c.want_tau, bs, c.inj, c.stream);
 }
 
@@ -295,6 +313,9 @@
     std::vector<ChainItem> chain, part;
     std::vector<const double2*> xs;
     std::vector<int> save_k;
+    std::vector<int64_t> bprefix(pl.T + 1, 0);
+    if (c.wtape)
+        for (int k = 0; k < pl.T; ++k) bprefix[k + 1] = bprefix[k] + step_block_count(rt, k);
     cl = 0;
     for (int k = pl.T - 1; k >= 0; --k) {
         const int k_hi = k;
@@ -309,7 +330,7 @@
             chain.insert(chain.end(), part.begin(), part.end());
         }
         int rc = gather_factor_inputs(c, bs, k, k_hi, chain, xs);
-        if (!rc) rc = chained ? adjoint_chained(c, bs, chain, xs, save_k, cl) : adjoint_direct(c, bs, chain, xs, save_k, cl);
+        if (!rc) rc = chained ? adjoint_chained(c, bs, chain, xs, save_k, bprefix[k_hi + 1] - 1, cl) : adjoint_direct(c, bs, chain, xs, save_k, cl);
         if (rc) return rc;
     }
     return RYDIFF_OK;
@@ -439,6 +460,10 @@
     c.buf[1] = reinterpret_cast<double2*>(c.ws + pl.off_buf1);
     if (c.partial_tape()) c.tmap = partial_tape_map(rt, p->tape_steps);
     const bool ws_tape = c.full_tape() || c.partial_tape();
+    if (c.full_tape()) {
+        c.wtape = pair_wtape(rt);
+        tape_format_record(workspace, c.wtape);
+    }
     double2* sout = static_cast<double2*>(states_out);
     if (p->final_state_only && sout) {
         if (need_tape || persist_enabled(rt))
@@ -486,6 +511,12 @@
         c.tmap = partial_tape_map(rt, p->tape_steps);
         c.tape_b = c.tape + size_t(pl.T + 1) * c.sv;
     }
+    c.wtape = c.full_tape() && tape_format_wtape(workspace);
+    if (c.full_tape() && c.wtape != pair_wtape(rt))
+        return fail(RYDIFF_EINVAL, c.wtape ? "the full tape in this workspace holds P_X v between the factors of a block (written by a forward call with the "
+                                             "block adjoint in view), and this backward call would read it as the mid-block state: use the forward call's kernel_variant and real_amp_grad"
+                                           : "the full tape in this workspace holds the mid-block state between the factors of a block, and this backward call "
+                                             "expects P_X v there: use the forward call's kernel_variant and real_amp_grad");
     c.fprefix.assign(pl.T + 1, 0);
     for (int k = 0; k < pl.T; ++k) c.fprefix[k + 1] = c.fprefix[k] + step_factor_count(rt, k);
     c.lam[0] = reinterpret_cast<double2*>(c.ws + pl.off_buf0);
```
